# nubot-nudt/RDMNet

Measured on AMD Instinct MI355X. Metric: scan-pairs/sec (whole node), higher is better.
Workload: dtype f32

## Files before the change

### rdmnet_amd/csrc/engine.hip

```cpp
#include <algorithm>
#include <cmath>
#include <cstring>
#include <atomic>
#include <chrono>
#include <functional>
#include <map>
#include <memory>
#include <string>
#include <vector>

#include "../../include/rdmnet_hip.h"
#include <ctime>

#include "common.h"
#include "internal.h"
#include "lockstep.h"

namespace {

using namespace rdm;

struct Mat {
  float* p = nullptr;
  int64_t rows = 0, cols = 0, ld = 0;
  Mat cols_from(int64_t c0, int64_t n) const { return Mat{p + c0, rows, n, ld}; }
  Mat rows_from(int64_t r0, int64_t n) const { return Mat{p + r0 * ld, n, cols, ld}; }
};

struct HostParam {
  std::vector<int64_t> shape;
  std::vector<float> data;
};

struct Linear {
  float* b = nullptr;
  float* wt = nullptr;
  float* bias = nullptr;
  float* packed = nullptr;
  int64_t in = 0, out = 0, kpad = 0, ldb = 0;
};

inline int64_t pad4(int64_t n) { return (n + 3) / 4 * 4; }

struct ParamSet {
  std::map<std::string, Linear> lin;
  std::map<std::string, float*> vec;
  std::vector<void*> owned;
  int device = -1;
  ParamSet() = default;
  ParamSet(const ParamSet&) = delete;
  ParamSet& operator=(const ParamSet&) = delete;
  ~ParamSet() {
    for (void* p : owned) (void)hipFree(p);
  }
};

struct Level {
  float* pts = nullptr;
  int64_t n = 0;
  int64_t* lengths = nullptr;
  int64_t n_ref = 0;
};
struct Table {
  int64_t* idx = nullptr;
  bool i32 = false;
  int64_t rows = 0, width = 0;
  int64_t ld = 0;
// ... 9 lines not shown
struct PairPyramid {
  Level lv[5];
  Table nb[5], sub[4], up[4];
  Grid grids[5];
  int32_t* flags = nullptr;
  int calls = 0;
};

}

struct rdm_engine {
  rdm_engine_config cfg;
  int device = -1;
  std::map<std::string, HostParam> host;
  std::shared_ptr<ParamSet> params = std::make_shared<ParamSet>();
  char* arena = nullptr;
  size_t arena_cap = 0, arena_off = 0;
  bool arena_exhausted = false, arena_fixed = false;
  void* pinned = nullptr;
  void* pinned_dev = nullptr;
  int64_t host_corr_cap = 0;
  int wait_sleep_us = 0;
  bool finalized = false;
  std::map<std::string, rdm_tensor_view> taps;
  bool keep_taps = false;
  bool collate_only = false;
  std::vector<double> topk_fracs;
  bool has_fm = false;
  rdm_fine_matching_options fm{1, 0, 1, 0, 0.f, 0};
  int pairs_in_flight = 1;
  int overlap_mode = 1;
  hipStream_t side = nullptr;
  std::map<hipStream_t, bool> side_ok;
  std::vector<PairPyramid> batch;
  std::vector<int64_t> batch_n_ref, batch_n_src;
  size_t arena_base = 0;
  bool profile = false;
  bool profile_shapes_only = false;
  std::vector<hipEvent_t> events;
  std::vector<rdm_kpconv_profile> prof;
  int prof_layers = 0;
  struct GtInputs {
    bool valid = false;
    const float* nodes[2] = {nullptr, nullptr};
    int64_t m[2] = {0, 0};
    const float* pf[2] = {nullptr, nullptr};
    int64_t nf[2] = {0, 0};
    const int64_t* knn[2] = {nullptr, nullptr};
    const uint8_t* km[2] = {nullptr, nullptr};
    const uint8_t* nm[2] = {nullptr, nullptr};
    int k = 0;
  } gt;

  template <typename T>
  T* alloc(size_t count) {
    size_t bytes = align_up(count * sizeof(T) + 16);
    if (arena_off + bytes > arena_cap) return nullptr;
    T* r = reinterpret_cast<T*>(arena + arena_off);
    arena_off += bytes;
    return r;
  }
  Mat mat(int64_t rows, int64_t cols) {
    Mat m;
    m.rows = rows; m.cols = cols; m.ld = pad4(cols);
    m.p = alloc<float>(static_cast<size_t>(rows > 0 ? rows : 1) * m.ld);
    return m;
  }
};

namespace {

#define ENG_CHECK(...)             \
  do {                             \
    int _rc = (__VA_ARGS__);       \
    if (_rc != 0) return _rc;      \
  } while (0)
#define ENG_ALLOC(ptr)                                             \
  do {                                                             \
    if ((ptr) == nullptr) {                                        \
      set_error("rdm_engine: activation arena exhausted (%zu B)", e->arena_cap); \
      e->arena_exhausted = true;                                   \
      return RDM_ERR_WORKSPACE;                                    \
    }                                                              \
  } while (0)

struct Run {
  rdm_engine* e;
  hipStream_t st;
  void* ws;
  size_t ws_bytes;
  int groups;
};

void tap(Run& r, const char* name, const void* p, int64_t rows, int64_t cols, int64_t ld, int dtype) {
  if (!r.e->keep_taps) return;
  rdm_tensor_view v;
  v.data = const_cast<void*>(p); v.rows = rows; v.cols = cols; v.ld = ld; v.dtype = dtype;
  r.e->taps[name] = v;
}
void tap(Run& r, const char* name, const Mat& m) { tap(r, name, m.p, m.rows, m.cols, m.ld, 0); }

const Linear* lin_param(Run& r, const std::string& name) {
  auto it = r.e->params->lin.find(name);
  if (it != r.e->params->lin.end()) return &it->second;
  set_error("rdm_engine: missing parameter %s", name.c_str());
  return nullptr;
}

float* vecp(Run& r, const std::string& name) {
  auto it = r.e->params->vec.find(name);
  return it == r.e->params->vec.end() ? nullptr : it->second;
}

int norm_params(Run& r, const std::string& prefix, float** g, float** b) {
  *g = vecp(r, prefix + ".weight");
  *b = vecp(r, prefix + ".bias");
  if (*g && *b) return RDM_OK;
  set_error("rdm_engine: missing parameter %s.*", prefix.c_str());
  return RDM_ERR_ARG;
}

int linear(Run& r, const std::string& name, const Mat& x, Mat& y, int act = 0, bool alloc_out = true) {
  lockstep_align();
  rdm_engine* e = r.e;
  const Linear* Lp = lin_param(r, name);
  if (!Lp) return RDM_ERR_ARG;
  const Linear& L = *Lp;
  if (alloc_out) {
    y = e->mat(x.rows, L.out);
    ENG_ALLOC(y.p);
  }
  return rdm_gemm(x.p, x.ld, 0, L.b, L.ldb, 0, 0, y.p, y.ld, 0, x.rows, L.out, L.kpad, 1, L.bias, nullptr, act, r.ws,
                  r.ws_bytes, r.st);
}

int linear_pair(Run& r, const std::string& name0, const Mat& x0, Mat& y0, const std::string& name1, const Mat& x1, Mat& y1) {
  lockstep_align();
  rdm_engine* e = r.e;
  const Linear* P0 = lin_param(r, name0);
  const Linear* P1 = P0 ? lin_param(r, name1) : nullptr;
  if (!P0 || !P1) return RDM_ERR_ARG;
  const Linear &L0 = *P0, &L1 = *P1;
  y0 = e->mat(x0.rows, L0.out);
  y1 = e->mat(x1.rows, L1.out);
  ENG_ALLOC(y0.p); ENG_ALLOC(y1.p);
  return gemm_pair(x0.p, x0.ld, L0.b, L0.ldb, y0.p, y0.ld, x0.rows, L0.out, L0.kpad, L0.bias, x1.p, x1.ld, L1.b, L1.ldb, y1.p,
                   y1.ld, x1.rows, L1.out, L1.kpad, L1.bias, r.ws, r.ws_bytes, r.st);
}

int group_norm(Run& r, const std::string& name, const Mat& x, Mat& y, int act, const Mat* res, uint8_t* positive) {
  lockstep_align();
  rdm_engine* e = r.e;
  y = e->mat(x.rows, x.cols);
  ENG_ALLOC(y.p);
  float *g, *b;
  ENG_CHECK(norm_params(r, name + ".norm", &g, &b));
  return rdm_group_norm(x.p, x.rows, x.cols, x.ld, r.groups, g, b, 1e-5f, res ? res->p : nullptr, res ? res->ld : 0, act,
                        y.p, y.ld, positive, r.ws, r.ws_bytes, r.st);
}

int unary(Run& r, const std::string& name, const Mat& x, Mat& y, int act, const Mat* res, uint8_t* positive) {
  lockstep_align();
  rdm_engine* e = r.e;
  const Linear* Lp = lin_param(r, name + ".mlp");
  if (!Lp) return RDM_ERR_ARG;
  const Linear& L = *Lp;
  Mat t = e->mat(x.rows, L.out);
  y = e->mat(x.rows, L.out);
  ENG_ALLOC(t.p); ENG_ALLOC(y.p);
  float *g, *b;
  ENG_CHECK(norm_params(r, name + ".norm.norm", &g, &b));
  return rdm_linear_group_norm(x.p, x.ld, L.b, L.ldb, L.bias, nullptr, x.rows, L.out, L.kpad, r.groups, g, b, 1e-5f,
                               res ? res->p : nullptr, res ? res->ld : 0, act, t.p, t.ld, y.p, y.ld, positive, r.ws,
                               r.ws_bytes, r.st);
}

int decoder_stage(Run& r, const std::string& lin_name, const std::string* norm_name, const Mat& coarse, const int64_t* up_idx,
                  int64_t up_ld, const Mat& skip, int64_t m, Mat& y) {
  lockstep_align();
  rdm_engine* e = r.e;
  const Linear* Lp = lin_param(r, lin_name);
  if (!Lp) return RDM_ERR_ARG;
  const Linear& L = *Lp;
  RDM_REQUIRE(coarse.cols + skip.cols == L.in, "rdm_engine: %s expects %lld input columns", lin_name.c_str(), (long long)L.in);
  Mat t = e->mat(m, L.out);
  ENG_ALLOC(t.p);
  float *g = nullptr, *b = nullptr;
  if (norm_name) {
    y = e->mat(m, L.out);
    ENG_ALLOC(y.p);
    ENG_CHECK(norm_params(r, *norm_name, &g, &b));
  } else {
    y = t;
  }
  const size_t need = rdm_decoder_stage_workspace_bytes(m, L.out, L.in);
  void* ws = r.ws;
  size_t ws_bytes = r.ws_bytes;
  if (need > ws_bytes) {
    ws = e->alloc<char>(need);
    ENG_ALLOC(ws);
    ws_bytes = need;
  }
  return rdm_decoder_stage(coarse.p, coarse.rows, coarse.cols, coarse.ld, up_idx, up_ld, skip.p, skip.cols, skip.ld, m, L.b, L.ldb,
                           L.bias, L.out, r.groups, g, b, 1e-5f, 2, t.p, t.ld, norm_name ? y.p : nullptr, norm_name ? y.ld : 0, ws,
                           ws_bytes, r.st);
}

int layer_norm(Run& r, const std::string& name, const Mat& x, const Mat* res, int act, Mat& y, bool alloc_out = true) {
  lockstep_align();
  rdm_engine* e = r.e;
  if (alloc_out) {
    y = e->mat(x.rows, x.cols);
    ENG_ALLOC(y.p);
  }
  return rdm_layer_norm(x.p, x.rows, x.cols, x.ld, res ? res->p : nullptr, res ? res->ld : 0, vecp(r, name + ".weight"),
                        vecp(r, name + ".bias"), 1e-5f, act, y.p, y.ld, r.st);
}

int layer_event(rdm_engine* e, int k, hipStream_t st) {
  if (e->profile_shapes_only) return RDM_OK;
  if (lockstep_active()) {
    lockstep_event(e->events[k], st);
    return RDM_OK;
  }
  RDM_HIP_CHECK(hipEventRecord(e->events[k], st));
  return RDM_OK;
}

int kpconv(Run& r, const std::string& name, const Mat& x, const uint8_t* x_pos, const Level& q, const Level& s,
           const Table& t, float sigma, const std::string& norm_name, Mat& y, const float* order,
           const Mat* pool_src = nullptr, Mat* pool_out = nullptr) {
  lockstep_align();
  rdm_engine* e = r.e;
  const Linear* Wp = lin_param(r, name + ".weights");
  if (!Wp) return RDM_ERR_ARG;
  const Linear& W = *Wp;
  const int64_t cin = x.cols, kdim = cin == 1 ? 16 : 15 * cin;
  const int i32 = t.i32 ? 1 : 0;
  const int li = e->prof_layers;
  const bool prof = e->profile && (e->profile_shapes_only ? li < 16 : 3 * li + 2 < static_cast<int>(e->events.size()));
  auto end_profile = [&](int fused) -> int {
    ENG_CHECK(layer_event(e, 3 * li + 2, r.st));
    rdm_kpconv_profile p;
    p.m = q.n; p.h = t.width; p.c_in = cin; p.c_out = W.out; p.pooled_channels = pool_src ? pool_src->cols : 0;
    p.gather_ms = p.total_ms = 0.f;
    p.fused = fused; p.reserved = 0;
    e->prof.push_back(p);
    e->prof_layers++;
    return RDM_OK;
  };
  if (W.packed && rdm_kpconv_fused_enabled()) {
    float *gam, *bet;
    ENG_CHECK(norm_params(r, norm_name + ".norm", &gam, &bet));
    Mat conv = e->mat(q.n, W.out);
    y = e->mat(q.n, W.out);
    ENG_ALLOC(conv.p); ENG_ALLOC(y.p);
    RDM_REQUIRE(rdm_kpconv_fused_workspace_bytes(q.n, cin, W.out) <= r.ws_bytes, "rdm_engine: scratch too small");
    if (prof) ENG_CHECK(layer_event(e, 3 * li, r.st));
    const int nblk = static_cast<int>(rdm_kpconv_fused_partial_rows(q.n, cin));
    double* gn_partial = static_cast<double*>(r.ws);
    const size_t stat_bytes = align_up(static_cast<size_t>(nblk) * 2 * W.out * sizeof(double));
    ENG_CHECK(kpconv_fused_impl(q.pts, q.n, s.pts, s.n, x.p, cin, x.ld, x_pos, t.idx, t.width, t.stride(), t.flags,
                                vecp(r, name + ".kernel_points"), sigma, W.packed, W.bias, W.out, conv.p, conv.ld, gn_partial, order, 0,
                                i32, r.st));
    if (prof) ENG_CHECK(layer_event(e, 3 * li + 1, r.st));
    ENG_CHECK(group_norm_finish(gn_partial, nblk, conv.p, q.n, W.out, conv.ld, r.groups, gam, bet, 1e-5f, nullptr, 0, 2, y.p, y.ld,
                                nullptr, static_cast<char*>(r.ws) + stat_bytes, r.ws_bytes - stat_bytes, r.st));
    if (pool_src) {
      *pool_out = e->mat(q.n, pool_src->cols);
      ENG_ALLOC(pool_out->p);
      ENG_CHECK(gather_max_ordered(pool_src->p, pool_src->rows, pool_src->cols, pool_src->ld, t.idx, q.n, t.width, t.stride(),
                                   t.flags, pool_out->p, pool_out->ld, order, i32, r.st));
    }
    if (prof) ENG_CHECK(end_profile(1));
    return RDM_OK;
  }
  Mat wf = e->mat(q.n, kdim);
  ENG_ALLOC(wf.p);
  float* nn = e->alloc<float>(q.n > 0 ? q.n : 1);
  ENG_ALLOC(nn);
  if (prof) ENG_CHECK(layer_event(e, 3 * li, r.st));
  ENG_CHECK(kpconv_gather_impl(q.pts, q.n, s.pts, s.n, x.p, cin, x.ld, x_pos, t.idx, t.width, t.stride(), t.flags,
                               vecp(r, name + ".kernel_points"), sigma, wf.p, wf.ld, nn, order, i32, r.st));
  if (prof) ENG_CHECK(layer_event(e, 3 * li + 1, r.st));
  Mat conv = e->mat(q.n, W.out);
  ENG_ALLOC(conv.p);
  const size_t gemm_ws = rdm_gemm_workspace_bytes(q.n, W.out, 1);
  const size_t stat_bytes = align_up(static_cast<size_t>(gemm_stats_max_blocks(q.n)) * 2 * W.out * sizeof(double));
  RDM_REQUIRE(gemm_ws + stat_bytes + rdm_group_norm_workspace_bytes(q.n, W.out) <= r.ws_bytes, "rdm_engine: scratch too small");
  double* gn_partial = reinterpret_cast<double*>(static_cast<char*>(r.ws) + gemm_ws);
  int gn_blocks = 0;
  ENG_CHECK(gemm_with_stats(wf.p, wf.ld, W.b, W.ldb, conv.p, conv.ld, q.n, W.out, W.kpad, W.bias, nn, r.ws, gemm_ws,
                            gn_partial, &gn_blocks, r.st));
  if (pool_src) {
    *pool_out = e->mat(q.n, pool_src->cols);
    ENG_ALLOC(pool_out->p);
    ENG_CHECK(gather_max_ordered(pool_src->p, pool_src->rows, pool_src->cols, pool_src->ld, t.idx, q.n, t.width, t.stride(),
                                   t.flags, pool_out->p, pool_out->ld, order, i32, r.st));
  }
  if (prof) ENG_CHECK(end_profile(0));
  y = e->mat(q.n, W.out);
  ENG_ALLOC(y.p);
  float *gam, *bet;
  ENG_CHECK(norm_params(r, norm_name + ".norm", &gam, &bet));
  return group_norm_finish(gn_partial, gn_blocks, conv.p, q.n, W.out, conv.ld, r.groups, gam, bet, 1e-5f, nullptr, 0, 2, y.p,
                           y.ld, nullptr, static_cast<char*>(r.ws) + gemm_ws + stat_bytes, r.ws_bytes - gemm_ws - stat_bytes,
                           r.st);
}

int linear_ln(Run& r, const std::string& lin, const std::string& norm, const Mat& x, const Mat& res, Mat& y, bool alloc_out) {
  lockstep_align();
  rdm_engine* e = r.e;
  const Linear* Lp = lin_param(r, lin);
  if (!Lp) return RDM_ERR_ARG;
  const Linear& L = *Lp;
  if (L.wt && L.out == 128) {
    if (alloc_out) {
      y = e->mat(x.rows, L.out);
      ENG_ALLOC(y.p);
    }
    return rdm_linear_layer_norm(x.p, x.ld, L.wt, L.kpad, L.bias, x.rows, L.out, L.kpad, res.p, res.ld, vecp(r, norm + ".weight"),
                                 vecp(r, norm + ".bias"), 1e-5f, 0, y.p, y.ld, r.st);
  }
  Mat h;
  ENG_CHECK(linear(r, lin, x, h));
  return layer_norm(r, norm, h, &res, 0, y, alloc_out);
}

int attention_tail(Run& r, const std::string& p, const Mat& hid, const Mat& x, Mat out) {
  lockstep_align();
  rdm_engine* e = r.e;
  auto lo = e->params->lin.find(p + ".attention.linear"), l1 = e->params->lin.find(p + ".output.expand"), l2 = e->params->lin.find(p + ".output.squeeze");
  if (lo != e->params->lin.end() && l1 != e->params->lin.end() && l2 != e->params->lin.end() && lo->second.wt && l1->second.wt && l2->second.wt &&
      lo->second.out == 128 && lo->second.kpad == 128 && l1->second.out == 256 && l1->second.kpad == 128 &&
      l2->second.out == 128 && l2->second.kpad == 256) {
    const Linear &Lo = lo->second, &L1 = l1->second, &L2 = l2->second;
    auto pk = e->params->vec.find(p + ".__tail_packed");
    static const bool unpacked = ::rdm::dev_knob("RDM_TAIL_UNPACKED") != nullptr;
    if (pk != e->params->vec.end() && !unpacked)
      return rdm_attention_tail_packed(hid.p, hid.ld, x.p, x.ld, hid.rows, 128, pk->second, Lo.bias, vecp(r, p + ".attention.norm.weight"),
                                       vecp(r, p + ".attention.norm.bias"), L1.bias, L2.bias, vecp(r, p + ".output.norm.weight"),
                                       vecp(r, p + ".output.norm.bias"), 1e-5f, out.p, out.ld, r.st);
    return rdm_attention_tail(hid.p, hid.ld, x.p, x.ld, hid.rows, 128, Lo.wt, Lo.kpad, Lo.bias, vecp(r, p + ".attention.norm.weight"),
                              vecp(r, p + ".attention.norm.bias"), L1.wt, L1.kpad, L1.bias, L2.wt, L2.kpad, L2.bias,
                              vecp(r, p + ".output.norm.weight"), vecp(r, p + ".output.norm.bias"), 1e-5f, out.p, out.ld, r.st);
  }
  Mat y, z1;
  ENG_CHECK(linear_ln(r, p + ".attention.linear", p + ".attention.norm", hid, x, y, true));
  ENG_CHECK(linear(r, p + ".output.expand", y, z1, 1));
  return linear_ln(r, p + ".output.squeeze", p + ".output.norm", z1, y, out, false);
}

int thdroformer(Run& r, const std::string& name, const Mat& pts4, const Mat& x, int64_t n0, int num_layers, Mat out,
                const std::function<int()>* after_two = nullptr, const std::vector<double>* topk = nullptr) {
  rdm_engine* e = r.e;
  const int heads = e->cfg.num_heads;
  const int64_t N = x.rows, n1 = N - n0;
  Mat emb, f;
  ENG_CHECK(linear(r, name + ".embedding.proj", pts4, emb));
  ENG_CHECK(linear(r, name + ".in_proj", x, f));
// ... 179 lines not shown
  if (e->side_ok.size() >= 64) e->side_ok.clear();
  if (e->side && runs_beside(st, e->side)) {
    *usable = e->side_ok[st] = true;
    return RDM_OK;
  }
  bool have_user = false;
  for (const auto& kv : e->side_ok) have_user |= kv.second;
  if (have_user) {
    *usable = e->side_ok[st] = false;
    return RDM_OK;
  }
  std::vector<hipStream_t> rejected;
  if (e->side) rejected.push_back(e->side);
  e->side = nullptr;
  for (int attempt = 0; attempt < 6 && !e->side; ++attempt) {
    hipStream_t cand = nullptr;
    RDM_HIP_CHECK(hipStreamCreateWithFlags(&cand, hipStreamNonBlocking));
    if (runs_beside(st, cand)) e->side = cand;
    else rejected.push_back(cand);
  }
  for (hipStream_t r : rejected) (void)hipStreamDestroy(r);
  *usable = e->side_ok[st] = e->side != nullptr;
  return RDM_OK;
}
struct SideGuard {
  rdm_engine* e;
  int pending = 0;
  ~SideGuard() {
    if (pending > 0 && e->side) (void)hipStreamSynchronize(e->side);
  }
};

int d2h(Run& r, const void* dev, size_t bytes, void* host_dst) {
  copy_words(dev, r.e->pinned_dev, static_cast<int>((bytes + 3) / 4), r.st);
  ENG_CHECK(wait_stream(r));
  std::memcpy(host_dst, r.e->pinned, bytes);
  return RDM_OK;
}

}

extern "C" int rdm_engine_create(const rdm_engine_config* cfg, rdm_engine** out) {
  RDM_REQUIRE(cfg && out, "rdm_engine_create: null pointer");
  RDM_REQUIRE(cfg->num_stages == 5 && cfg->kernel_size == 15, "rdm_engine_create: only 5 stages / 15 kernel points");
  int device = -1;
  RDM_HIP_CHECK(hipGetDevice(&device));
  rdm_engine* e = new rdm_engine();
  e->cfg = *cfg;
  e->device = device;
  e->params->device = device;
  e->arena_cap = cfg->arena_bytes ? cfg->arena_bytes : (size_t(3) << 30);
  e->arena_fixed = cfg->arena_bytes != 0;
  hipError_t err = hipMalloc(reinterpret_cast<void**>(&e->arena), e->arena_cap);
  if (err != hipSuccess) {
    set_error("rdm_engine_create: hipMalloc(%zu) failed: %s", e->arena_cap, hipGetErrorString(err));
    delete e;
    return RDM_ERR_HIP;
  }
  e->host_corr_cap = static_cast<int64_t>(std::max(cfg->num_correspondences, 1)) * 2 * std::max(cfg->points_in_patch, 1);
  err = hipHostMalloc(&e->pinned, 4096 + static_cast<size_t>(e->host_corr_cap) * 7 * sizeof(float), hipHostMallocMapped);
  if (err == hipSuccess) err = hipHostGetDevicePointer(&e->pinned_dev, e->pinned, 0);
  if (err != hipSuccess) {
    set_error("rdm_engine_create: hipHostMalloc failed: %s", hipGetErrorString(err));
    (void)hipFree(e->arena);
    delete e;
    return RDM_ERR_HIP;
  }
  *out = e;
  return RDM_OK;
}

extern "C" void rdm_engine_destroy(rdm_engine* e) {
  if (!e) return;
  e->params.reset();
  for (auto& ev : e->events) (void)hipEventDestroy(ev);
  if (e->side) {
    (void)hipStreamSynchronize(e->side);
    (void)hipStreamDestroy(e->side);
  }
  if (e->arena) (void)hipFree(e->arena);
  if (e->pinned) (void)hipHostFree(e->pinned);
  delete e;
}

extern "C" int rdm_engine_set_param(rdm_engine* e, const char* name, const float* data_host, const int64_t* shape_host,
                                    int ndim) {
  RDM_REQUIRE(e && name && data_host && ndim >= 0 && ndim <= 4, "rdm_engine_set_param: bad arguments");
  HostParam p;
  int64_t n = 1;
  for (int i = 0; i < ndim; ++i) {
    p.shape.push_back(shape_host[i]);
    n *= shape_host[i];
  }
  p.data.assign(data_host, data_host + n);
  e->host[name] = std::move(p);
  e->finalized = false;
  return RDM_OK;
}

namespace {
int upload(rdm_engine* e, const std::vector<float>& h, float** dev) {
  void* p = nullptr;
  RDM_HIP_CHECK(hipMalloc(&p, (h.size() + 4) * sizeof(float)));
  RDM_HIP_CHECK(hipMemcpy(p, h.data(), h.size() * sizeof(float), hipMemcpyHostToDevice));
  e->params->owned.push_back(p);
  *dev = static_cast<float*>(p);
// ... 96 lines not shown
        continue;
      float* d = nullptr;
      RDM_HIP_CHECK(hipMalloc(reinterpret_cast<void**>(&d), rdm_attention_tail_packed_floats() * sizeof(float)));
      e->params->owned.push_back(d);
      ENG_CHECK(rdm_attention_tail_pack_weights(lo->second.wt, lo->second.kpad, l1->second.wt, l1->second.kpad, l2->second.wt, l2->second.kpad, d, nullptr));
      e->params->vec[p + ".__tail_packed"] = d;
    }
    RDM_HIP_CHECK(hipDeviceSynchronize());
  }
  e->finalized = true;
  return RDM_OK;
}

extern "C" int rdm_engine_share_params(rdm_engine* e, const rdm_engine* src) {
  RDM_REQUIRE(e && src && e != src, "rdm_engine_share_params: bad arguments");
  RDM_REQUIRE(src->finalized, "rdm_engine_share_params: the source engine is not finalized");
  RDM_REQUIRE(e->device == src->device && src->params->device == src->device,
              "rdm_engine_share_params: the engines live on different devices (%d vs %d)", e->device, src->device);
  const rdm_engine_config &a = e->cfg, &b = src->cfg;
  RDM_REQUIRE(a.num_stages == b.num_stages && a.kernel_size == b.kernel_size && a.group_norm == b.group_norm &&
                  a.out_dim == b.out_dim && a.num_heads == b.num_heads && a.num_layers == b.num_layers &&
                  a.num_layers2 == b.num_layers2 && a.vote_mlp_layers == b.vote_mlp_layers &&
                  a.points_in_patch == b.points_in_patch,
              "rdm_engine_share_params: the engines were created with different model shapes");
  e->host.clear();
  e->params = src->params;
  e->finalized = true;
  return RDM_OK;
}

extern "C" int rdm_engine_enable_profile(rdm_engine* e, int enable) {
  RDM_REQUIRE(e, "rdm_engine_enable_profile: null engine");
  RDM_REQUIRE(enable >= 0 && enable <= 2, "rdm_engine_enable_profile: 0 (off), 1 (events) or 2 (layer shapes only)");
  e->profile = enable != 0;
  e->profile_shapes_only = enable == 2;
  if (enable == 1 && e->events.empty()) {
    e->events.resize(3 * 16);
    for (auto& ev : e->events) RDM_HIP_CHECK(hipEventCreate(&ev));
  }
  return RDM_OK;
}

extern "C" int rdm_engine_reserve(rdm_engine* e, size_t bytes) {
  RDM_REQUIRE(e && bytes >= (size_t(1) << 20), "rdm_engine_reserve: at least 1 MiB");
  RDM_HIP_CHECK(hipDeviceSynchronize());
  e->batch.clear();
  e->arena_base = 0;
  e->gt.valid = false;
  RDM_HIP_CHECK(hipFree(e->arena));
  e->arena = nullptr;
  e->arena_cap = bytes;
  e->arena_fixed = false;
  const hipError_t err = hipMalloc(reinterpret_cast<void**>(&e->arena), e->arena_cap);
  if (err != hipSuccess) {
    e->arena_cap = 0;
    set_error("rdm_engine_reserve: hipMalloc(%zu) failed: %s", bytes, hipGetErrorString(err));
    return RDM_ERR_HIP;
  }
  return RDM_OK;
}

extern "C" int rdm_engine_set_wait(rdm_engine* e, int sleep_us) {
  RDM_REQUIRE(e && sleep_us >= 0, "rdm_engine_set_wait: bad arguments");
  e->wait_sleep_us = sleep_us;
  return RDM_OK;
}

extern "C" int rdm_engine_set_pairs_in_flight(rdm_engine* e, int n) {
  RDM_REQUIRE(e && n >= 1, "rdm_engine_set_pairs_in_flight: bad arguments");
  e->pairs_in_flight = n;
  return RDM_OK;
}

extern "C" int rdm_engine_set_fine_matching(rdm_engine* e, const rdm_fine_matching_options* o) {
  RDM_REQUIRE(e, "rdm_engine_set_fine_matching: null engine");
  if (!o) {
    e->has_fm = false;
    return RDM_OK;
  }
  const int K = std::max(e->cfg.points_in_patch, 1);
  RDM_REQUIRE(o->topk >= 1 && o->topk <= K + (o->use_dustbin ? 1 : 0), "rdm_engine_set_fine_matching: topk = %d is outside [1, %d]",
              o->topk, K + (o->use_dustbin ? 1 : 0));
  RDM_REQUIRE(o->confidence_threshold >= 0.f, "rdm_engine_set_fine_matching: confidence_threshold = %g is not >= 0",
              static_cast<double>(o->confidence_threshold));
  RDM_REQUIRE(o->correspondence_limit >= 0, "rdm_engine_set_fine_matching: correspondence_limit = %d (0 = none, or >= 1)",
              o->correspondence_limit);
  const int64_t cap = rdm_lgr_options_capacity(std::max(e->cfg.num_correspondences, 1), K, o);
  if (cap > e->host_corr_cap) {
    int device = -1;
    RDM_HIP_CHECK(hipGetDevice(&device));
    RDM_REQUIRE(device == e->device, "rdm_engine_set_fine_matching: the engine belongs to device %d, current is %d", e->device, device);
    void* pinned = nullptr;
    void* pinned_dev = nullptr;
    RDM_HIP_CHECK(hipHostMalloc(&pinned, 4096 + static_cast<size_t>(cap) * 7 * sizeof(float), hipHostMallocMapped));
    const hipError_t err = hipHostGetDevicePointer(&pinned_dev, pinned, 0);
    if (err != hipSuccess) {
      (void)hipHostFree(pinned);
      set_error("rdm_engine_set_fine_matching: hipHostGetDevicePointer failed: %s", hipGetErrorString(err));
      return RDM_ERR_HIP;
    }
    RDM_HIP_CHECK(hipDeviceSynchronize());
    if (e->pinned) (void)hipHostFree(e->pinned);
    e->pinned = pinned;
    e->pinned_dev = pinned_dev;
    e->host_corr_cap = cap;
  }
// ... 93 lines not shown
    if (!(nb0_done && i == 0)) ENG_CHECK(search(e, sq, lv[i], py.grids[i], radius, c.neighbor_limits[i], !full, row(), py.nb[i]));
    if (i < 4) ENG_CHECK(search(e, sq, lv[i + 1], py.grids[i], radius, c.neighbor_limits[i], !full, row(), py.sub[i]));
    if (i > 0 && (full || i > 1))
      ENG_CHECK(search(e, sq, lv[i - 1], py.grids[i], radius, full ? c.neighbor_limits[i] : 1, false, row(), py.up[i - 1]));
  }
  return RDM_OK;
}

int build_level_grids(rdm_engine* e, PairPyramid* pys, int n, int first, int last, hipStream_t st) {
  const float* gp[8];
  int64_t gn[8];
  const int64_t* gl[8];
  float gr[8];
  void* gw[8];
  size_t gb[8];
  int k = 0;
  auto launch = [&]() -> int {
    RDM_DUP_LOOP("rnbuild")
    ENG_CHECK(radius_grid_build_multi(k, gp, gn, gl, 2, gr, gw, gb, st));
    k = 0;
    return RDM_OK;
  };
  for (int p = 0; p < n; ++p) {
    float rad = e->cfg.init_radius;
    for (int i = 0; i < last; ++i, rad *= 2.f) {
      if (i < first) continue;
      const Level& l = pys[p].lv[i];
      Grid& g = pys[p].grids[i];
      g.n_s = l.n;
      g.bytes = rdm_radius_grid_workspace_bytes(l.n);
      g.ws = e->alloc<char>(g.bytes);
      ENG_ALLOC(g.ws);
      gp[k] = l.pts; gn[k] = l.n; gl[k] = l.lengths; gr[k] = rad; gw[k] = g.ws; gb[k] = g.bytes;
      if (++k == 8) ENG_CHECK(launch());
    }
  }
  return k > 0 ? launch() : RDM_OK;
}

}

static int engine_run_once(rdm_engine* e, const float* ref_points, int64_t n_ref, const float* src_points, int64_t n_src,
                           const rdm_data_dict* dd, rdm_engine_result* res, void* stream, const PairPyramid* pre = nullptr);

static bool may_grow(const rdm_engine* e, int rc) {
  return rc == RDM_ERR_WORKSPACE && e->arena_exhausted && !e->arena_fixed && e->arena_cap < (size_t(96) << 30);
}
static int grow_arena(rdm_engine* e, void* stream, const char* who) {
  RDM_HIP_CHECK(hipStreamSynchronize(static_cast<hipStream_t>(stream)));
  RDM_HIP_CHECK(hipFree(e->arena));
  e->arena = nullptr;
  e->arena_cap *= 2;
  const hipError_t err = hipMalloc(reinterpret_cast<void**>(&e->arena), e->arena_cap);
  if (err != hipSuccess) {
    e->arena_cap = 0;
    set_error("%s: growing the activation arena failed: %s", who, hipGetErrorString(err));
    return RDM_ERR_HIP;
  }
  return RDM_OK;
}
static int engine_run_growing(rdm_engine* e, const float* ref_points, int64_t n_ref, const float* src_points, int64_t n_src,
                              const rdm_data_dict* dd, rdm_engine_result* res, void* stream) {
  PadGuard pad_guard(e->pairs_in_flight >= 3 ? 20480u : 0u);
  for (;;) {
    e->arena_exhausted = false;
    const int rc = engine_run_once(e, ref_points, n_ref, src_points, n_src, dd, res, stream);
    if (!may_grow(e, rc)) return rc;
    ENG_CHECK(grow_arena(e, stream, "rdm_engine_run"));
  }
}

extern "C" int rdm_engine_run(rdm_engine* e, const float* ref_points, int64_t n_ref, const float* src_points,
                              int64_t n_src, rdm_engine_result* res, void* stream) {
  RDM_REQUIRE(e && ref_points && src_points && res, "rdm_engine_run: null pointer");
  RDM_REQUIRE(e->finalized, "rdm_engine_run: call rdm_engine_finalize first");
  RDM_REQUIRE(n_ref > 0 && n_src > 0, "rdm_engine_run: empty cloud");
  return engine_run_growing(e, ref_points, n_ref, src_points, n_src, nullptr, res, stream);
}

static int collate_batch_once(rdm_engine* e, int B, const float* const* refs, const int64_t* n_refs, const float* const* srcs,
                              const int64_t* n_srcs, hipStream_t st) {
  const rdm_engine_config& c = e->cfg;
  e->arena_off = 0;
  e->arena_base = 0;
  e->gt.valid = false;
  e->batch.clear();
  e->taps.clear();
  Run r;
  r.e = e; r.st = st; r.groups = c.group_norm;
  int64_t n_tot = 0;
  for (int p = 0; p < B; ++p) n_tot += n_refs[p] + n_srcs[p];
  const int nc = 2 * B;
  r.ws_bytes = std::max<size_t>(rdm_grid_subsample_workspace_bytes(n_tot, nc), size_t(16) << 20);
  r.ws = e->alloc<char>(r.ws_bytes);
  ENG_ALLOC(r.ws);
  float* pts[5];
  int64_t* len[5];
  pts[0] = e->alloc<float>(3 * n_tot);
  len[0] = e->alloc<int64_t>(nc);
  ENG_ALLOC(pts[0]); ENG_ALLOC(len[0]);
  {
    int64_t base = 0;
    for (int p = 0; p < B; ++p) {
      ENG_CHECK(launch1d<concat_points_kernel_body, concat_points_kernel>("concat_points", 3 * (n_refs[p] + n_srcs[p]), st, refs[p], n_refs[p], srcs[p], n_srcs[p],
                         pts[0] + 3 * base, len[0] + 2 * p));
      base += n_refs[p] + n_srcs[p];
// ... 716 lines not shown
  const int64_t cap = n0;
  for (int i = 1; i < 5; ++i) {
    voxel *= 2.f;
    lv[i].pts = e->alloc<float>(3 * cap);
    lv[i].lengths = all_len + 2 * (i - 1);
    ENG_ALLOC(lv[i].pts);
    RDM_DUP_LOOP("gs")
    ENG_CHECK(grid_subsample_mode(i == 1 ? pts0 : lv[i - 1].pts, cap, i == 1 ? len0 : lv[i - 1].lengths, 2, voxel, lv[i].pts,
                                  lv[i].lengths, r.ws, r.ws_bytes, r.st, i <= gs_multi_levels() ? 2 : 1));
    if (i == 1 && overlap_l0) {
      ENG_CHECK(launch1d<concat_points_kernel_body, concat_points_kernel>("concat_points", 3 * n0, rs.st, ref_points, n_ref, src_points, n_src, lv[0].pts,
                         lv[0].lengths));
      ENG_CHECK(build_level_grids(e, &py, 1, 0, 1, rs.st));
      SearchQueue side_queue(rs.st);
      ENG_CHECK(search(e, side_queue, lv[0], py.grids[0], c.init_radius, c.neighbor_limits[0], !full, py.flags + 2 * py.calls++,
                       py.nb[0]));
      ENG_CHECK(side_queue.flush());
      ENG_CHECK(encoder_input(rs, nullptr, n0, enc));
      ENG_CHECK(encoder_blocks(rs, py, 0, 2, enc));
    }
  }
  int64_t host_len[8];
  ENG_CHECK(d2h(r, all_len, sizeof(host_len), host_len));
  if (overlap_l0) {
    ENG_CHECK(wait_on(e, e->side));
    side_guard.pending--;
  }
  for (int i = 1; i < 5; ++i) {
    lv[i].n_ref = host_len[2 * (i - 1)];
    lv[i].n = host_len[2 * (i - 1)] + host_len[2 * (i - 1) + 1];
  }
  ENG_CHECK(build_level_grids(e, &py, 1, overlap_l0 ? 1 : 0, 5, r.st));
  SearchQueue sq(r.st);
  ENG_CHECK(search_pyramid(e, py, full, overlap_l0, sq));
  return sq.flush();
}

void tap_pyramid(Run& r, const PairPyramid& py) {
  for (int i = 0; i < 5; ++i) {
    const Level& l = py.lv[i];
    tap(r, ("lengths" + std::to_string(i)).c_str(), l.lengths, 1, 2, 2, 1);
    tap(r, ("points" + std::to_string(i)).c_str(), l.pts, l.n, 3, 3, 0);
    tap(r, ("neighbors" + std::to_string(i)).c_str(), py.nb[i].idx, py.nb[i].rows, py.nb[i].width, py.nb[i].stride(), 1);
    if (i < 4) {
      tap(r, ("subsampling" + std::to_string(i)).c_str(), py.sub[i].idx, py.sub[i].rows, py.sub[i].width, py.sub[i].stride(), 1);
      tap(r, ("upsampling" + std::to_string(i)).c_str(), py.up[i].idx, py.up[i].rows, py.up[i].width, py.up[i].stride(), 1);
    }
  }
  tap(r, "search_flags", py.flags, 32, 2, 2, 3);
}

}

static int engine_run_once(rdm_engine* e, const float* ref_points, int64_t n_ref, const float* src_points, int64_t n_src,
                           const rdm_data_dict* dd, rdm_engine_result* res, void* stream, const PairPyramid* pre) {
  const rdm_engine_config& c = e->cfg;
  e->arena_off = pre ? e->arena_base : 0;
  e->gt.valid = false;
  if (!pre) {
    e->batch.clear();
    e->arena_base = 0;
  }
  e->taps.clear();
  e->prof.clear();
  e->prof_layers = 0;
  Run r;
  r.e = e; r.st = static_cast<hipStream_t>(stream); r.groups = c.group_norm;
  const int64_t n0 = n_ref + n_src;
  bool overlap = !pre && !lockstep_active() && !e->collate_only && r.st != nullptr && (e->overlap_mode == 2 || (e->overlap_mode == 1 && e->pairs_in_flight == 1));
  if (overlap) ENG_CHECK(ensure_side(e, r.st, &overlap));
  SideGuard side_guard{e};
  r.ws_bytes = pre ? size_t(96) << 20
                   : std::max<size_t>(rdm_grid_subsample_workspace_bytes(n0, 2),
                                      std::max<size_t>(rdm_radius_neighbors_workspace_bytes(n0, n0, 2), size_t(96) << 20));
  r.ws = e->alloc<char>(r.ws_bytes);
  ENG_ALLOC(r.ws);
  std::memset(res, 0, sizeof(*res));

  PairPyramid py;
  Encoder enc;
  if (pre) py = *pre;
  else if (dd) ENG_CHECK(pyramid_from_data_dict(r, *dd, py));
  else ENG_CHECK(collate_pair(r, overlap, side_guard, ref_points, n_ref, src_points, n_src, py, enc));
  for (int i = 0; i < 5; ++i) {
    res->level_sizes[i] = py.lv[i].n;
    res->level_ref_sizes[i] = py.lv[i].n_ref;
  }
  tap_pyramid(r, py);
  if (e->collate_only) {
    res->arena_used = e->arena_off;
    return RDM_OK;
  }

  {
    size_t need = r.ws_bytes;
    for (int l = 0; l < c.num_stages; ++l)
      need = std::max(need, rdm_linear_group_norm_workspace_bytes(py.lv[l].n, int64_t(128) << l));
    if (need > r.ws_bytes) {
      r.ws_bytes = need;
      r.ws = e->alloc<char>(r.ws_bytes);
      ENG_ALLOC(r.ws);
    }
  }

  if (enc.blocks == 0) ENG_CHECK(encoder_input(r, dd, n0, enc));
  ENG_CHECK(encoder_blocks(r, py, enc.blocks, 14, enc));
  tap(r, "feats_c_enc", enc.feats[4]);
// ... 175 lines not shown
```

### rdmnet_amd/csrc/gemm.hip

```cpp
#include "../../include/rdmnet_hip.h"
#include <cmath>
#include <cstdlib>
#include <type_traits>

#include "common.h"
#include "internal.h"
#include "lockstep.h"

namespace {

using namespace rdm;

typedef float f32x16 __attribute__((ext_vector_type(16)));
typedef float f32x4_t __attribute__((ext_vector_type(4)));

struct GemmArgs {
  const float* A;
  const float* B;
  float* C;
  const float* bias;
  const float* rowdiv;
  int M, N, K;
  int lda, ldb, ldc;
  long long sa, sb, sc;
  int act;
  int splits;
  float* part;
  double* stats;
  const float* A2;
  const int64_t* aidx;
  int lda2, ldi, c1, n_coarse;
  const int64_t* bidx;
  int n_b;
  int xcd_tiles;
#ifdef RDM_GEMM_TIMING
  unsigned long long* clk;
#endif
};
#ifdef RDM_GEMM_TIMING
#define GEMM_STAMP(k) do { if (blockIdx.x == 0 && blockIdx.y == 0 && blockIdx.z == 0 && threadIdx.x == 0) g.clk[k] = __builtin_amdgcn_s_memtime(); } while (0)
#else
#define GEMM_STAMP(k) do { } while (0)
#endif
#ifdef RDM_GEMM_TIMING
#define GEMM_WIDE_STAMP(k) do { if (blockIdx.x == 0 && blockIdx.y == 0 && blockIdx.z == 0 && threadIdx.x == 0 && (k) < 392) g.clk[k] = __builtin_amdgcn_s_memtime(); } while (0)
#else
#define GEMM_WIDE_STAMP(k) do { } while (0)
#endif

__device__ __forceinline__ float apply_act(float v, int act) {
  if (act == 1) return v > 0.f ? v : 0.f;
  if (act == 2) return v > 0.f ? v : 0.1f * v;
  return v;
}

template <int BM, int BN, int WM, int WN, int BK, bool TRANS_B, int PF, bool CAT = false>
__device__ __forceinline__ void gemm_kernel_body(const dim3 blockIdx, const dim3 gridDim, GemmArgs g) {
  (void)blockIdx; (void)gridDim;
  constexpr int TM = BM / WM, TN = BN / WN, FM = TM / 32, FN = TN / 32;
  static_assert(WM * WN == 4 && TM % 32 == 0 && TN % 32 == 0, "bad tile");
  constexpr int LDA_S = BM + 1, LDB_S = TRANS_B ? BN + 1 : BN + 4;
  constexpr int CR = BM < 64 ? BM : 64;
  constexpr int LDC_S = BN + 4;
  constexpr int TPR = BN / 4;
  constexpr int RPI = 256 / TPR;
  constexpr int kBytesAB = (2 * BK * LDA_S + 2 * BK * LDB_S) * 4, kBytesC = CR * LDC_S * 4, kBytesStat = RPI * BN * 2 * 8;
  constexpr int kBytes = kBytesAB > kBytesC ? (kBytesAB > kBytesStat ? kBytesAB : kBytesStat) : (kBytesC > kBytesStat ? kBytesC : kBytesStat);
  static_assert((2 * BK * LDA_S * 4) % 16 == 0 && CR % RPI == 0, "tile layout");
  __shared__ __attribute__((aligned(16))) char smem[kBytes];
  float (*As)[BK][LDA_S] = reinterpret_cast<float (*)[BK][LDA_S]>(smem);
  float (*Bs)[BK][LDB_S] = reinterpret_cast<float (*)[BK][LDB_S]>(smem + 2 * BK * LDA_S * 4);
  float (*Cs)[LDC_S] = reinterpret_cast<float (*)[LDC_S]>(smem);
  double (*stat_red)[1][2] = reinterpret_cast<double (*)[1][2]>(smem);

  const int tid = threadIdx.x, lane = tid & 63, wave = tid >> 6;
  const int wm = wave / WN, wn = wave % WN;
  int tile_x = blockIdx.x, tile_y = blockIdx.y;
  if (g.xcd_tiles) {
    const int nblk = gridDim.x * gridDim.y, lin = blockIdx.y * gridDim.x + blockIdx.x;
    const int q = nblk / 8, rr = nblk % 8, xcd = lin % 8, within = lin / 8;
    const int logical = (xcd < rr ? xcd * (q + 1) : rr * (q + 1) + (xcd - rr) * q) + within;
    tile_x = logical % gridDim.x;
    tile_y = logical / gridDim.x;
  }
  const int m0 = tile_y * BM, n0 = tile_x * BN;
  GEMM_STAMP(0);
  const int batch = blockIdx.z / g.splits, split = blockIdx.z % g.splits;
  const float* A = g.A + batch * g.sa;
  const float* B = g.B + batch * g.sb;

  const int ktiles = (g.K + BK - 1) / BK;
  const int per = (ktiles + g.splits - 1) / g.splits;
  const int kt0 = split * per, kt1 = min(ktiles, kt0 + per);

  constexpr int A_N4 = BM * BK / 4;
  constexpr int A_V = (A_N4 + 255) / 256;
  constexpr int KC4 = BK / 4;
  constexpr int B_N4 = BK * BN / 4;
  constexpr int B_V = (B_N4 + 255) / 256;
  static_assert(PF == 1 || PF == 2, "one or two register stages");
  float4 ra0[A_V], rb0[B_V], ra1[PF == 2 ? A_V : 1], rb1[PF == 2 ? B_V : 1];
  long long cat_row[CAT ? A_V : 1], cat_brow[CAT && TRANS_B ? B_V : 1];
  if constexpr (CAT && !TRANS_B) {
#pragma unroll
    for (int i = 0; i < A_V; ++i) {
      const int row = (tid + i * 256) / (BK / 4);
      const long long id = g.aidx[static_cast<long long>(min(m0 + row, g.M - 1)) * g.ldi];
      cat_row[i] = (id >= 0 && id < g.n_coarse) ? id : -1;
    }
  }
  if constexpr (CAT && TRANS_B) {
    A = g.A;
    B = g.B;
    int any_a = 0, any_b = 0;
#pragma unroll
    for (int i = 0; i < A_V; ++i) {
      const int row = (tid + i * 256) / (BK / 4);
      const long long id = (m0 + row < g.M && (A_N4 % 256 == 0 || tid + i * 256 < A_N4)) ? g.aidx[static_cast<long long>(batch) * g.M + m0 + row] : -1;
      cat_row[i] = (id >= 0 && id < g.n_coarse) ? id : -1;
      any_a |= cat_row[i] >= 0;
    }
// ... 197 lines not shown
        const float4 t = *reinterpret_cast<const float4*>(&Cs[lrow][c4]);
        float v[4] = {t.x, t.y, t.z, t.w};
        if (has_rd) {
          const float rd = rdv[pass * (CR / RPI) + it];
#pragma unroll
          for (int e = 0; e < 4; ++e) v[e] = v[e] / rd;
        }
        if (!partial) {
#pragma unroll
          for (int e = 0; e < 4; ++e) {
            const float u = v[e] + bv[e];
            const float neg = act == 2 ? 0.1f * u : 0.f;
            v[e] = (act != 0 && !(u > 0.f)) ? neg : u;
          }
        }
        float* dst = C + static_cast<long long>(row) * ldc + gcol;
        if (vec_ok && gcol + 3 < g.N) {
          *reinterpret_cast<float4*>(dst) = make_float4(v[0], v[1], v[2], v[3]);
        } else {
#pragma unroll
          for (int e = 0; e < 4; ++e)
            if (gcol + e < g.N) dst[e] = v[e];
        }
        if (stats) {
#pragma unroll
          for (int e = 0; e < 4; ++e) {
            cs[e] += v[e];
            css[e] += static_cast<double>(v[e]) * v[e];
          }
        }
      }
    }
    GEMM_STAMP(5);
    lds_barrier();
  }
  if (stats) {
#pragma unroll
    for (int e = 0; e < 4; ++e) {
      stat_red[rsub * BN + c4 + e][0][0] = cs[e];
      stat_red[rsub * BN + c4 + e][0][1] = css[e];
    }
    lds_barrier();
    for (int cl = tid; cl < BN; cl += 256) {
      const int col = n0 + cl;
      if (col >= g.N) continue;
      double a = 0.0, b = 0.0;
#pragma unroll
      for (int w = 0; w < RPI; ++w) {
        a += stat_red[w * BN + cl][0][0];
        b += stat_red[w * BN + cl][0][1];
      }
      g.stats[(static_cast<long long>(tile_y) * 2 + 0) * g.N + col] = a;
      g.stats[(static_cast<long long>(tile_y) * 2 + 1) * g.N + col] = b;
    }
  }
  GEMM_STAMP(3);
}
template <int BM, int BN, int WM, int WN, int BK, bool TRANS_B, int PF, bool CAT = false>
__global__ __launch_bounds__(256, (BM * BN <= 64 * 64 ? 4 : 1)) void gemm_kernel(GemmArgs g) { gemm_kernel_body<BM, BN, WM, WN, BK, TRANS_B, PF, CAT>(blockIdx, gridDim, g); }


template <bool CAT, bool MI16 = false>
__device__ __forceinline__ void gemm_wide_body(const dim3 blockIdx, const dim3 gridDim, GemmArgs g) {
  (void)gridDim;
  constexpr int BM = 128, BN = 128, BK = 32;
  constexpr int IMG = 8 * BM * 4;
  constexpr int CR = 64, LDC_S = BN + 4, TPR = BN / 4, RPI = 256 / TPR;
  static_assert(BM == BN && RPI == 8 && CR * LDC_S * 4 <= 4 * IMG * 4 && 16 * BN * 2 * 8 <= 4 * IMG * 4, "wide tile layout");
  __shared__ __attribute__((aligned(16))) char smem[4 * IMG * 4];
  float* As = reinterpret_cast<float*>(smem);
  float* Bs = As + 2 * IMG;
  float (*Cs)[LDC_S] = reinterpret_cast<float (*)[LDC_S]>(smem);
  double (*stat_red)[BN][2] = reinterpret_cast<double (*)[BN][2]>(smem);

  const int tid = threadIdx.x, lane = tid & 63, wave = tid >> 6;
  const int wm = wave >> 1, wn = wave & 1;
  constexpr int NF = MI16 ? 4 : 2;
  constexpr int FR = MI16 ? 16 : 32;
  constexpr int KG = MI16 ? 16 : 8;
  constexpr int NG = BK / KG;
  constexpr int KL = MI16 ? 4 : 2;
  const int lk = MI16 ? lane >> 4 : lane >> 5, li = MI16 ? lane & 15 : lane & 31;
  const int m0 = blockIdx.y * BM, n0 = blockIdx.x * BN;
  const int batch = blockIdx.z / g.splits, split = blockIdx.z % g.splits;
  const float* A = g.A + (CAT ? 0 : batch * g.sa);
  const float* B = g.B + batch * g.sb;
  const int ktiles = (g.K + BK - 1) / BK;
  const int per = (ktiles + g.splits - 1) / g.splits;
  const int kt0 = split * per, kt1 = min(ktiles, kt0 + per);
  GEMM_WIDE_STAMP(0);

  const int a_q = tid & 7, a_row = tid >> 3;
  const int b_p = tid >> 5, b_n4 = (tid & 31) * 4;
  const int b_k = MI16 ? 16 * (b_p >> 2) + (b_p & 3) : 8 * (b_p >> 1) + (b_p & 1);
  float4 ra[4], rb[4];
  const float* a_ptr[4];
  long long cat_row[CAT ? 4 : 1];
#pragma unroll
  for (int i = 0; i < 4; ++i) {
    const int row = min(m0 + a_row + 32 * i, g.M - 1);
    if constexpr (CAT) {
      const long long id = g.aidx[static_cast<long long>(row) * g.ldi];
      cat_row[i] = (id >= 0 && id < g.n_coarse) ? id : -1;
      a_ptr[i] = A + max(cat_row[i], 0ll) * g.lda;
    } else {
      a_ptr[i] = A + static_cast<long long>(row) * g.lda;
// ... 206 lines not shown
        float v[4] = {t.x, t.y, t.z, t.w};
        if (has_rd) {
#pragma unroll
          for (int e = 0; e < 4; ++e) v[e] = v[e] / rdv[it];
        }
        if (!partial) {
#pragma unroll
          for (int e = 0; e < 4; ++e) {
            const float u = v[e] + bv[e];
            const float neg = act == 2 ? 0.1f * u : 0.f;
            v[e] = (act != 0 && !(u > 0.f)) ? neg : u;
          }
        }
        float* dst = C + static_cast<long long>(row) * ldc + gcol;
        if (vec_ok && gcol + 3 < g.N) {
          *reinterpret_cast<float4*>(dst) = make_float4(v[0], v[1], v[2], v[3]);
        } else {
#pragma unroll
          for (int e = 0; e < 4; ++e)
            if (gcol + e < g.N) dst[e] = v[e];
        }
        if (stats) {
#pragma unroll
          for (int e = 0; e < 4; ++e) {
            cs[it & 1][e] += v[e];
            css[it & 1][e] += static_cast<double>(v[e]) * v[e];
          }
        }
      }
    }
    lds_barrier();
    if (stats) {
#pragma unroll
      for (int par = 0; par < 2; ++par)
#pragma unroll
        for (int e = 0; e < 4; ++e) {
          stat_red[par * RPI + rsub][c4 + e][0] = cs[par][e];
          stat_red[par * RPI + rsub][c4 + e][1] = css[par][e];
        }
      lds_barrier();
      if (tid < BN && n0 + tid < g.N) {
        double a = 0.0, b = 0.0;
#pragma unroll
        for (int w = 0; w < 16; ++w) {
          a += stat_red[w][tid][0];
          b += stat_red[w][tid][1];
        }
        const long long blk = static_cast<long long>(blockIdx.y) * 2 + pass;
        g.stats[(blk * 2 + 0) * g.N + n0 + tid] = a;
        g.stats[(blk * 2 + 1) * g.N + n0 + tid] = b;
      }
      lds_barrier();
    }
  }
  GEMM_WIDE_STAMP(3);
}
template <bool CAT, bool MI16 = false>
__global__ __launch_bounds__(256, 2) void gemm_wide_kernel(GemmArgs g) { gemm_wide_body<CAT, MI16>(blockIdx, gridDim, g); }

__device__ __forceinline__ void gemm_small_body(const dim3 blockIdx, const GemmArgs& g, float (*red)[32][33]) {
  const int tid = threadIdx.x, lane = tid & 63, wave = tid >> 6;
  const int li = lane & 31, lk = lane >> 5;
  const int m0 = blockIdx.y * 32, n0 = blockIdx.x * 32;
  const int kq = g.K / 4;
  const int kbeg = wave * kq;
  const int row = min(m0 + li, g.M - 1);
  const int col = n0 + li;
  const bool col_ok = col < g.ldb;
  const float* arow = g.A + static_cast<long long>(row) * g.lda;
  f32x16 acc;
#pragma unroll
  for (int r = 0; r < 16; ++r) acc[r] = 0.f;
  for (int c = 0; c < kq; c += 32) {
    float a[16], b[16];
    const int kb = kbeg + c + lk * 16;
#pragma unroll
    for (int q = 0; q < 4; ++q) {
      float4 v = make_float4(0.f, 0.f, 0.f, 0.f);
      if (c + lk * 16 + 4 * q < kq) v = *reinterpret_cast<const float4*>(arow + kb + 4 * q);
      a[4 * q] = v.x; a[4 * q + 1] = v.y; a[4 * q + 2] = v.z; a[4 * q + 3] = v.w;
    }
#pragma unroll
    for (int t = 0; t < 16; ++t)
      b[t] = (col_ok && c + lk * 16 + t < kq) ? g.B[static_cast<long long>(kb + t) * g.ldb + col] : 0.f;
#pragma unroll
    for (int t = 0; t < 16; ++t) acc = __builtin_amdgcn_mfma_f32_32x32x2f32(a[t], b[t], acc, 0, 0, 0);
  }
#pragma unroll
  for (int r = 0; r < 16; ++r) red[wave][(r & 3) + 8 * (r >> 2) + 4 * lk][li] = acc[r];
  __syncthreads();
#pragma unroll
  for (int q = 0; q < 4; ++q) {
    const int e = tid + 256 * q, rr = e >> 5, cc = e & 31;
    const int orow = m0 + rr, ocol = n0 + cc;
    if (orow < g.M && ocol < g.N) {
      float v = ((red[0][rr][cc] + red[1][rr][cc]) + red[2][rr][cc]) + red[3][rr][cc];
      if (g.bias) v += g.bias[ocol];
      g.C[static_cast<long long>(orow) * g.ldc + ocol] = apply_act(v, g.act);
    }
  }
}

__device__ __forceinline__ void gemm_small_entry(const dim3 blockIdx, const dim3 gridDim, GemmArgs g) {
  (void)gridDim;
  __shared__ float red[4][32][33];
  gemm_small_body(blockIdx, g, red);
// ... 231 lines not shown
  layer_norm(o, 2, g2, be2);
  TAIL_STAMP(7);
#pragma unroll
  for (int r = 0; r < 4; ++r) {
    const int row = m0 + 4 * kb + r;
    if (row < a.M) a.out[static_cast<long long>(row) * a.ldo + c] = o[r];
  }
}
template <bool PACKED>
__global__ __launch_bounds__(512) void attention_tail128_kernel(TailArgs a) { attention_tail128_body<PACKED>(blockIdx, gridDim, a); }

__global__ void attention_tail_pack_kernel(const float* wo, int ldwo, const float* w1, int ldw1, const float* w2, int ldw2, float4* out) {
  const int e = blockIdx.x * blockDim.x + threadIdx.x;
  if (e >= 20480) return;
  const int lane = e & 63, i = lane & 15, kb = lane >> 4;
  const float* src;
  if (e < 4096) {
    const int w = e >> 9, s = (e >> 6) & 7;
    src = wo + static_cast<long long>(16 * w + i) * ldwo + 16 * s + 4 * kb;
  } else if (e < 12288) {
    const int t = e - 4096, w = t >> 10, h = (t >> 9) & 1, s = (t >> 6) & 7;
    src = w1 + static_cast<long long>(32 * w + 16 * h + i) * ldw1 + 16 * s + 4 * kb;
  } else {
    const int t = e - 12288, w = t >> 10, s = (t >> 6) & 15;
    src = w2 + static_cast<long long>(16 * w + i) * ldw2 + 16 * s + 4 * kb;
  }
  out[e] = *reinterpret_cast<const float4*>(src);
}

__device__ __forceinline__ void splitk_reduce_kernel_body(const dim3 blockIdx, const dim3 gridDim, GemmArgs g, int batches) {
  (void)blockIdx; (void)gridDim;
  const long long total = static_cast<long long>(batches) * g.M * g.N;
  for (long long i = blockIdx.x * static_cast<long long>(blockDim.x) + threadIdx.x; i < total;
       i += static_cast<long long>(gridDim.x) * blockDim.x) {
    const int n = static_cast<int>(i % g.N);
    const int m = static_cast<int>((i / g.N) % g.M);
    const int b = static_cast<int>(i / (static_cast<long long>(g.M) * g.N));
    const float* p = g.part + (static_cast<long long>(b) * g.splits) * g.M * g.N +
                     static_cast<long long>(m) * g.N + n;
    float v = 0.f;
    for (int s = 0; s < g.splits; ++s) v += p[static_cast<long long>(s) * g.M * g.N];
    if (g.rowdiv) v = v / g.rowdiv[m];
    if (g.bias) v += g.bias[n];
    g.C[b * g.sc + static_cast<long long>(m) * g.ldc + n] = apply_act(v, g.act);
  }
}
__global__ void splitk_reduce_kernel(GemmArgs g, int batches) { splitk_reduce_kernel_body(blockIdx, gridDim, g, batches); }


constexpr int kStatRowsPerLane = 8;
inline int stat_rows_per_block(long long n) { return kStatRowsPerLane * (256 / static_cast<int>(n < 256 ? n : 256)); }
__device__ __forceinline__ void splitk_reduce_stats_kernel_body(const dim3 blockIdx, const dim3 gridDim, GemmArgs g, double* stats) {
  (void)blockIdx; (void)gridDim;
  __shared__ double red[2][256];
  const int cw = g.N < 256 ? g.N : 256;
  const int lanes = 256 / cw;
  const int r0 = blockIdx.x * (kStatRowsPerLane * lanes);
  const int r1 = min(g.M, r0 + kStatRowsPerLane * lanes);
  const int col_in = threadIdx.x % cw, rl = threadIdx.x / cw;
  const int col = blockIdx.y * 256 + col_in;
  double s = 0.0, ss = 0.0;
  if (rl < lanes && col < g.N) {
    const float bv = g.bias ? g.bias[col] : 0.f;
    const long long plane = static_cast<long long>(g.M) * g.N;
    float acc[kStatRowsPerLane];
    const float* p[kStatRowsPerLane];
#pragma unroll
    for (int u = 0; u < kStatRowsPerLane; ++u) {
      const int r = min(r0 + rl + u * lanes, g.M - 1);
      p[u] = g.part + static_cast<long long>(r) * g.N + col;
      acc[u] = 0.f;
    }
    for (int k = 0; k < g.splits; ++k) {
#pragma unroll
      for (int u = 0; u < kStatRowsPerLane; ++u) acc[u] += p[u][k * plane];
    }
#pragma unroll
    for (int u = 0; u < kStatRowsPerLane; ++u) {
      const int r = r0 + rl + u * lanes;
      if (r >= r1) break;
      float v = acc[u];
      if (g.rowdiv) v = v / g.rowdiv[r];
      v = apply_act(v + bv, g.act);
      g.C[static_cast<long long>(r) * g.ldc + col] = v;
      const double d = v;
      s += d;
      ss += d * d;
    }
  }
  red[0][threadIdx.x] = s;
  red[1][threadIdx.x] = ss;
  __syncthreads();
  if (threadIdx.x < cw && col < g.N) {
    double a = 0.0, b = 0.0;
    for (int k = 0; k < lanes; ++k) {
      a += red[0][k * cw + threadIdx.x];
      b += red[1][k * cw + threadIdx.x];
    }
    stats[(static_cast<long long>(blockIdx.x) * 2 + 0) * g.N + col] = a;
    stats[(static_cast<long long>(blockIdx.x) * 2 + 1) * g.N + col] = b;
  }
}
__global__ __launch_bounds__(256) void splitk_reduce_stats_kernel(GemmArgs g, double* stats) { splitk_reduce_stats_kernel_body(blockIdx, gridDim, g, stats); }


thread_local unsigned g_lds_pad = 0;

template <int BM, int BN, int WM, int WN, int BK, int PF = 1>
void launch(const GemmArgs& g, int batches, bool trans_b, hipStream_t st) {
  dim3 grid(ceil_div(g.N, BN), ceil_div(g.M, BM), batches * g.splits);
  static const int pad_env = [] { const char* v = ::rdm::dev_knob("RDM_GEMM_LDS_PAD"); return v ? atoi(v) : -1; }();
  const unsigned pad = pad_env >= 0 ? static_cast<unsigned>(pad_env) : g_lds_pad;
  if constexpr (BM == 64 && BN == 64 && BK == 32 && PF == 2) {
    if (g.aidx && g.bidx) {
      ::rdm::launch<gemm_kernel_body<BM, BN, WM, WN, BK, true, PF, true>, gemm_kernel<BM, BN, WM, WN, BK, true, PF, true>, 256, (BM * BN <= 64 * 64 ? 4 : 1)>(grid, pad, st, g);
      return;
    }
    if (g.aidx) {
      ::rdm::launch<gemm_kernel_body<BM, BN, WM, WN, BK, false, PF, true>, gemm_kernel<BM, BN, WM, WN, BK, false, PF, true>, 256, (BM * BN <= 64 * 64 ? 4 : 1)>(grid, pad, st, g);
      return;
    }
  }
  if (trans_b)
    ::rdm::launch<gemm_kernel_body<BM, BN, WM, WN, BK, true, PF>, gemm_kernel<BM, BN, WM, WN, BK, true, PF>, 256, (BM * BN <= 64 * 64 ? 4 : 1)>(grid, pad, st, g);
  else
    ::rdm::launch<gemm_kernel_body<BM, BN, WM, WN, BK, false, PF>, gemm_kernel<BM, BN, WM, WN, BK, false, PF>, 256, (BM * BN <= 64 * 64 ? 4 : 1)>(grid, pad, st, g);
}

void launch_wide(const GemmArgs& g, int batches, hipStream_t st, bool mi16_form) {
  dim3 grid(ceil_div(g.N, 128), ceil_div(g.M, 128), batches * g.splits);
  static const bool mi16 = ::rdm::dev_knob("RDM_GEMM_WIDE_MI16") != nullptr;
  if (mi16 || mi16_form) {
    if (g.aidx) ::rdm::launch<gemm_wide_body<true, true>, gemm_wide_kernel<true, true>, 256, 2>(grid, 0, st, g);
    else ::rdm::launch<gemm_wide_body<false, true>, gemm_wide_kernel<false, true>, 256, 2>(grid, 0, st, g);
    return;
  }
  if (g.aidx) ::rdm::launch<gemm_wide_body<true>, gemm_wide_kernel<true>, 256, 2>(grid, 0, st, g);
  else ::rdm::launch<gemm_wide_body<false>, gemm_wide_kernel<false>, 256, 2>(grid, 0, st, g);
}

}

void rdm::gemm_set_lds_pad(unsigned bytes) { g_lds_pad = bytes; }

extern "C" size_t rdm_gemm_workspace_bytes(int64_t m, int64_t n, int batches) {
  const size_t by_shape = static_cast<size_t>(m) * static_cast<size_t>(n) * 16;
  const size_t by_tiles = static_cast<size_t>(1024) * 128 * 128;
  return align_up(std::min(by_shape, by_tiles) * sizeof(float) * static_cast<size_t>(batches > 0 ? batches : 1));
}

namespace {

thread_local int g_last_plan[4] = {0, 0, 0, 0};

int gemm_dispatch(GemmArgs g, int batches, bool trans_b, void* ws, size_t ws_bytes, int* stat_blocks, hipStream_t st, int form = 0) {
  const long long m = g.M, n = g.N, k = g.K;
  const char* tune_env = ::rdm::dev_knob("RDM_GEMM_TUNE");
  if (batches == 1 && !trans_b && !g.rowdiv && !g.stats && !g.aidx && m <= 1536 && k % 16 == 0 && k >= 64 && k <= 1024 &&
      m * n <= 1536 * 512 && !(tune_env && tune_env[0] != '0')) {
    if (stat_blocks) *stat_blocks = 0;
    g_last_plan[0] = 32; g_last_plan[1] = 32; g_last_plan[2] = static_cast<int>(k / 4); g_last_plan[3] = 4;
    RDM_DUP_LOOP("gemmsmall")
    ::rdm::launch<gemm_small_entry, gemm_small_kernel, 256>(dim3(ceil_div<long long>(n, 32), ceil_div<long long>(m, 32)), 0, st, g);
    return launch_status("gemm_small_kernel");
  }
  enum Tile { T128, T64, T128x32 };
  struct Cand { Tile tile; int bm, bn; double fixed_us, lat_k64_us, mfma_k64_us; int resident; double alpha; };
  static const Cand cands[3] = {{T128, 128, 128, 4.0, 2.6, 3.4, 3, 0.0}, {T64, 64, 64, 1.5, 2.2, 0.86, 4, 0.2},
                                {T128x32, 128, 32, 3.0, 1.3, 0.86, 3, 0.0}};
  static const int split_set[8] = {1, 2, 3, 4, 6, 8, 12, 16};
  static const long long model_cus = [] {
    const char* v = ::rdm::dev_knob("RDM_GEMM_CUS");
    const long long n = v ? atoll(v) : 256;
    return n >= 8 && n <= 256 ? n : 256ll;
  }();
  Tile tile = T64;
  int best_s = 1;
  {
    double best = 1e30;
    const size_t ws_cap = ws ? ws_bytes : 0;
    for (const Cand& c : cands) {
      if (g.aidx && c.tile != T64) continue;
      if (c.tile == T128x32 && n > 64) continue;
      if (c.tile != T128x32 && n <= 32) continue;
      if (c.tile == T128 && n < 128) continue;
      const long long tiles = ceil_div<long long>(m, c.bm) * ceil_div<long long>(n, c.bn) * batches;
      const int max_s = k >= 256 ? static_cast<int>(std::min<long long>(16, k / 128)) : 1;
      for (int sp : split_set) {
        if (sp > max_s) break;
        if (sp > 1 && static_cast<size_t>(m) * n * sp * batches * sizeof(float) > ws_cap) break;
        const long long blocks = tiles * sp;
        const double k_per = static_cast<double>(k) / sp / 64.0;
        const long long per_round = model_cus * c.resident;
        const long long full = blocks / per_round, rem = blocks % per_round;
        auto per_k64 = [&](double r) { return std::max(c.lat_k64_us * (1.0 + c.alpha * (r - 1.0)), c.mfma_k64_us * r); };
        double t = full * (c.fixed_us + k_per * per_k64(c.resident));
        if (rem) t += c.fixed_us + k_per * per_k64(static_cast<double>(ceil_div<long long>(rem, model_cus)));
        if (sp > 1) t += 3.0 + static_cast<double>(m) * n * sp * 8.0 / 1.5e6;
        if (t < best) {
          best = t;
          tile = c.tile;
          best_s = sp;
        }
      }
    }
  }
  int force_splits = 0, exp_tile = 0;
  if (const char* tune = ::rdm::dev_knob("RDM_GEMM_TUNE")) {
    int t = 0, sp = 0;
    if (sscanf(tune, "%d,%d", &t, &sp) >= 1) {
      if (t == 1) tile = T128;
      else if (t == 2) tile = T64;
      else if (t == 3) tile = T128x32;
      else if (t >= 4 && t <= 7) exp_tile = t;
      force_splits = sp;
      if (t >= 1 && t <= 7 && sp == 0) best_s = 1;
    }
  }
  static const int big_min_m = [] { const char* v = ::rdm::dev_knob("RDM_GEMM_BIG"); return v ? atoi(v) : 0; }();
  static const int big_tile = [] { const char* v = ::rdm::dev_knob("RDM_GEMM_BIG"); const char* c = v ? strchr(v, ',') : nullptr; return c ? atoi(c + 1) : 6; }();
  static const bool big_split = ::rdm::dev_knob("RDM_GEMM_BIG_SPLIT") != nullptr;
  if (big_min_m > 0 && exp_tile == 0 && m >= big_min_m && n >= 128 && (best_s == 1 || big_split) && force_splits == 0 && batches == 1)
    exp_tile = big_tile;
  static const bool xcd_env = ::rdm::dev_knob("RDM_GEMM_XCD") != nullptr;
  g.xcd_tiles = (xcd_env && ceil_div<long long>(n, 64) > 1 && ceil_div<long long>(m, 64) * ceil_div<long long>(n, 64) >= 64) ? 1 : 0;
  if (g.aidx) {
    tile = T64;
    exp_tile = 0;
    if (g.bidx) best_s = 1, force_splits = 0;
  }
  static const int wide_min_m = [] { const char* v = ::rdm::dev_knob("RDM_GEMM_WIDE_MIN_M"); return v ? atoi(v) : 256; }();
  static const int wide_min_n = [] { const char* v = ::rdm::dev_knob("RDM_GEMM_WIDE_MIN_N"); return v ? atoi(v) : 128; }();
  static const bool wide_knob = ::rdm::dev_knob("RDM_GEMM_WIDE") != nullptr;
  const bool wide_off = !wide_knob && form == 0;
  static const bool wide_force = ::rdm::dev_knob("RDM_GEMM_WIDE_FORCE") != nullptr;
  if (wide_force && !trans_b && !g.bidx && exp_tile == 0) tile = T64;
  const bool wide = !wide_off && tile == T64 && exp_tile == 0 && !trans_b && !g.bidx && (form != 0 || (m >= wide_min_m && n >= wide_min_n));
  int bm = tile == T64 ? 64 : 128, bn = tile == T128 ? 128 : (tile == T64 ? 64 : 32);
  if (wide) { bm = 128; bn = 128; }
  if (exp_tile == 4) { bm = 128; bn = 64; }
  if (exp_tile == 5) { bm = 64; bn = 128; }
  if (exp_tile == 6) { bm = 128; bn = 128; }
  if (exp_tile == 7) { bm = 256; bn = 64; }
  {
    int sp = force_splits > 0 ? force_splits : best_s;
    const size_t need = static_cast<size_t>(m) * n * sp * batches * sizeof(float);
    if (sp > 1 && ws && ws_bytes >= need) {
      g.splits = sp;
      g.part = static_cast<float*>(ws);
    }
  }
  double* reduce_stats = nullptr;
  if (g.splits > 1) {
    if (batches == 1 && g.N % 4 == 0) reduce_stats = g.stats;
    g.stats = nullptr;
  }
  if (stat_blocks)
    *stat_blocks = g.stats ? static_cast<int>(ceil_div<long long>(m, wide ? 64 : bm))
                           : (reduce_stats ? static_cast<int>(ceil_div<long long>(m, stat_rows_per_block(n))) : 0);
  g_last_plan[0] = bm; g_last_plan[1] = bn; g_last_plan[3] = g.splits;
  g_last_plan[2] = wide ? 32 : (tile == T128 ? 16 : ((tile == T64 ? (k >= 48 || g.aidx) : k >= 32) ? 32 : 16));
  RDM_DUP_LOOP("gemm") {
  if (wide) launch_wide(g, batches, st, form == 2);
  else
#ifdef RDM_DEV_KNOBS
  if (exp_tile == 4) launch<128, 64, 2, 2, 32, 2>(g, batches, trans_b, st);
  else if (exp_tile == 5) launch<64, 128, 2, 2, 32, 2>(g, batches, trans_b, st);
  else if (exp_tile == 6) launch<128, 128, 2, 2, 32, 2>(g, batches, trans_b, st);
  else if (exp_tile == 7) launch<256, 64, 4, 1, 32, 2>(g, batches, trans_b, st);
  else
#endif
  switch (tile) {
    case T128: launch<128, 128, 2, 2, 16>(g, batches, trans_b, st); break;
    case T64:
      static const bool bk16 = ::rdm::dev_knob("RDM_GEMM_BK16") != nullptr;
      if ((k >= 48 && !bk16) || g.aidx) launch<64, 64, 2, 2, 32, 2>(g, batches, trans_b, st);
      else launch<64, 64, 2, 2, 16>(g, batches, trans_b, st);
      break;
    case T128x32:
      if (k >= 32) launch<128, 32, 4, 1, 32, 2>(g, batches, trans_b, st);
      else launch<128, 32, 4, 1, 16>(g, batches, trans_b, st);
      break;
  }
  }
  if (int e = launch_status("gemm_kernel")) return e;
  if (g.splits > 1 && reduce_stats) {
    RDM_DUP_LOOP("splitk")
    ::rdm::launch<splitk_reduce_stats_kernel_body, splitk_reduce_stats_kernel, 256>(dim3(ceil_div<long long>(m, stat_rows_per_block(n)), ceil_div<long long>(n, 256)), 0, st, g, reduce_stats);
    return launch_status("splitk_reduce_stats_kernel");
  }
  if (g.splits > 1) {
    const long long total = static_cast<long long>(batches) * m * n;
    const int blocks = static_cast<int>(std::min<long long>(ceil_div<long long>(total, 256), 2048));
    ::rdm::launch<splitk_reduce_kernel_body, splitk_reduce_kernel, 256>(dim3(blocks), 0, st, g, batches);
    return launch_status("splitk_reduce_kernel");
  }
  return RDM_OK;
}

}

int rdm::gemm_with_stats(const float* a, int64_t lda, const float* b, int64_t ldb, float* c, int64_t ldc, int64_t m,
                         int64_t n, int64_t k, const float* bias, const float* rowdiv, void* ws, size_t ws_bytes,
                         double* gn_partial, int* gn_blocks, void* stream, int form) {
  GemmArgs g;
  g.A = a; g.B = b; g.C = c; g.bias = bias; g.rowdiv = rowdiv;
  g.M = static_cast<int>(m); g.N = static_cast<int>(n); g.K = static_cast<int>(k);
  g.lda = static_cast<int>(lda); g.ldb = static_cast<int>(ldb); g.ldc = static_cast<int>(ldc);
  g.sa = g.sb = g.sc = 0;
  g.act = 0; g.splits = 1; g.part = nullptr; g.stats = gn_partial;
  g.A2 = nullptr; g.aidx = nullptr; g.lda2 = g.ldi = g.c1 = g.n_coarse = 0; g.bidx = nullptr; g.n_b = 0;
  return gemm_dispatch(g, 1, false, ws, ws_bytes, gn_blocks, static_cast<hipStream_t>(stream), form);
}

int rdm::gemm_concat_with_stats(const float* coarse, int64_t ld1, int64_t c1, int64_t n_coarse, const int64_t* idx, int64_t ldi,
                                const float* skip, int64_t ld2, int64_t c2, const float* b, int64_t ldb, float* c, int64_t ldc,
                                int64_t m, int64_t n, const float* bias, int act, void* ws, size_t ws_bytes, double* gn_partial,
                                int* gn_blocks, void* stream, int form) {
  if (c1 % 32 != 0 || c2 % 4 != 0 || c2 < 4 || ld1 % 4 != 0 || ld2 % 4 != 0 || ldb % 4 != 0 || m <= 0 ||
      ((reinterpret_cast<uintptr_t>(coarse) | reinterpret_cast<uintptr_t>(skip) | reinterpret_cast<uintptr_t>(b)) & 15) != 0)
    return 1;
  GemmArgs g;
  g.A = coarse; g.B = b; g.C = c; g.bias = bias; g.rowdiv = nullptr;
  g.M = static_cast<int>(m); g.N = static_cast<int>(n); g.K = static_cast<int>(c1 + c2);
  g.lda = static_cast<int>(ld1); g.ldb = static_cast<int>(ldb); g.ldc = static_cast<int>(ldc);
  g.sa = g.sb = g.sc = 0;
  g.act = act; g.splits = 1; g.part = nullptr; g.stats = gn_partial;
  g.A2 = skip; g.aidx = idx; g.lda2 = static_cast<int>(ld2); g.ldi = static_cast<int>(ldi); g.c1 = static_cast<int>(c1);
  g.n_coarse = static_cast<int>(n_coarse);
  g.bidx = nullptr; g.n_b = 0;
  return gemm_dispatch(g, 1, false, ws, ws_bytes, gn_blocks, static_cast<hipStream_t>(stream), form);
}

namespace {
bool small_kernel_ok(long long m, long long n, long long k) {
  return m <= 1536 && k % 16 == 0 && k >= 64 && k <= 1024 && m * n <= 1536 * 512 && !::rdm::dev_knob("RDM_GEMM_TUNE");
}
}

int rdm::gemm_pair(const float* a0, int64_t lda0, const float* b0, int64_t ldb0, float* c0, int64_t ldc0, int64_t m0, int64_t n0,
                   int64_t k0, const float* bias0, const float* a1, int64_t lda1, const float* b1, int64_t ldb1, float* c1,
                   int64_t ldc1, int64_t m1, int64_t n1, int64_t k1, const float* bias1, void* ws, size_t ws_bytes, void* stream) {
  if (m0 > 0 && m1 > 0 && small_kernel_ok(m0, n0, k0) && small_kernel_ok(m1, n1, k1) && lda0 % 4 == 0 && lda1 % 4 == 0 &&
      ldb0 % 4 == 0 && ldb1 % 4 == 0 && ((reinterpret_cast<uintptr_t>(a0) | reinterpret_cast<uintptr_t>(a1)) & 15) == 0) {
    GemmArgs g[2];
    const float* A[2] = {a0, a1}; const float* B[2] = {b0, b1}; float* C[2] = {c0, c1}; const float* bias[2] = {bias0, bias1};
    const int64_t M[2] = {m0, m1}, N[2] = {n0, n1}, K[2] = {k0, k1}, LA[2] = {lda0, lda1}, LB[2] = {ldb0, ldb1}, LC[2] = {ldc0, ldc1};
    for (int i = 0; i < 2; ++i) {
      g[i].A = A[i]; g[i].B = B[i]; g[i].C = C[i]; g[i].bias = bias[i]; g[i].rowdiv = nullptr;
      g[i].M = static_cast<int>(M[i]); g[i].N = static_cast<int>(N[i]); g[i].K = static_cast<int>(K[i]);
      g[i].lda = static_cast<int>(LA[i]); g[i].ldb = static_cast<int>(LB[i]); g[i].ldc = static_cast<int>(LC[i]);
      g[i].sa = g[i].sb = g[i].sc = 0; g[i].act = 0; g[i].splits = 1; g[i].part = nullptr; g[i].stats = nullptr;
      g[i].A2 = nullptr; g[i].aidx = nullptr; g[i].lda2 = g[i].ldi = g[i].c1 = g[i].n_coarse = 0; g[i].bidx = nullptr; g[i].n_b = 0;
    }
    const long long gx = ceil_div<long long>(std::max(n0, n1), 32), gy = ceil_div<long long>(std::max(m0, m1), 32);
    ::rdm::launch<gemm_small_pair_entry, gemm_small_pair_kernel, 256>(dim3(gx, gy, 2), 0, static_cast<hipStream_t>(stream), g[0], g[1]);
    return launch_status("gemm_small_pair_kernel");
  }
  if (m0 > 0)
    if (int e = rdm_gemm(a0, lda0, 0, b0, ldb0, 0, 0, c0, ldc0, 0, m0, n0, k0, 1, bias0, nullptr, 0, ws, ws_bytes, stream)) return e;
  if (m1 > 0) return rdm_gemm(a1, lda1, 0, b1, ldb1, 0, 0, c1, ldc1, 0, m1, n1, k1, 1, bias1, nullptr, 0, ws, ws_bytes, stream);
  return RDM_OK;
}

extern "C" int rdm_gemm_last_plan(int* out4_host) {
  using namespace rdm;
  RDM_REQUIRE(out4_host, "rdm_gemm_last_plan: null pointer");
  for (int i = 0; i < 4; ++i) out4_host[i] = g_last_plan[i];
  return RDM_OK;
}

extern "C" int rdm_gemm(const float* a, int64_t lda, int64_t stride_a, const float* b, int64_t ldb,
                        int64_t stride_b, int trans_b, float* c, int64_t ldc, int64_t stride_c,
                        int64_t m, int64_t n, int64_t k, int batches, const float* bias,
                        const float* rowdiv, int act, void* ws, size_t ws_bytes, void* stream) {
  return rdm_gemm_form(a, lda, stride_a, b, ldb, stride_b, trans_b, c, ldc, stride_c, m, n, k, batches, bias, rowdiv, act, ws, ws_bytes, 0, stream);
}

extern "C" int rdm_gemm_form(const float* a, int64_t lda, int64_t stride_a, const float* b, int64_t ldb,
                             int64_t stride_b, int trans_b, float* c, int64_t ldc, int64_t stride_c,
                             int64_t m, int64_t n, int64_t k, int batches, const float* bias,
                             const float* rowdiv, int act, void* ws, size_t ws_bytes, int form, void* stream) {
  using namespace rdm;
  RDM_REQUIRE(form >= 0 && form <= 2, "rdm_gemm_form: unknown form %d", form);
  RDM_REQUIRE(a && b && c, "rdm_gemm: null pointer");
  RDM_REQUIRE(m >= 0 && n >= 0 && k >= 0 && batches >= 1, "rdm_gemm: bad sizes");
  if (m == 0 || n == 0) return RDM_OK;
  RDM_REQUIRE(k % 4 == 0 && lda % 4 == 0 && ldb % 4 == 0,
              "rdm_gemm: K (%lld), lda (%lld), ldb (%lld) must be multiples of 4 (pad with zeros)",
              (long long)k, (long long)lda, (long long)ldb);
  RDM_REQUIRE((reinterpret_cast<uintptr_t>(a) & 15) == 0 && (reinterpret_cast<uintptr_t>(b) & 15) == 0,
              "rdm_gemm: A and B must be 16-byte aligned");
  RDM_REQUIRE(act >= 0 && act <= 2, "rdm_gemm: unknown activation %d", act);
  GemmArgs g;
  g.A = a; g.B = b; g.C = c; g.bias = bias; g.rowdiv = rowdiv;
  g.M = static_cast<int>(m); g.N = static_cast<int>(n); g.K = static_cast<int>(k);
  g.lda = static_cast<int>(lda); g.ldb = static_cast<int>(ldb); g.ldc = static_cast<int>(ldc);
  g.sa = stride_a; g.sb = stride_b; g.sc = stride_c;
  g.act = act; g.splits = 1; g.part = nullptr; g.stats = nullptr;
  g.A2 = nullptr; g.aidx = nullptr; g.lda2 = g.ldi = g.c1 = g.n_coarse = 0; g.bidx = nullptr; g.n_b = 0;
  return gemm_dispatch(g, batches, trans_b != 0, ws, ws_bytes, nullptr, static_cast<hipStream_t>(stream), form);
}

extern "C" size_t rdm_linear_group_norm_workspace_bytes(int64_t m, int64_t n) {
  return rdm_gemm_workspace_bytes(m, n, 1) + rdm::align_up(static_cast<size_t>(rdm::gemm_stats_max_blocks(m)) * 2 * n * sizeof(double)) +
         rdm_group_norm_workspace_bytes(m, n) + 1024;
}

extern "C" int rdm_linear_group_norm(const float* x, int64_t ldx, const float* w, int64_t ldw, const float* bias,
                                     const float* rowdiv, int64_t m, int64_t n, int64_t k, int groups,
                                     const float* gamma, const float* beta, float eps, const float* residual,
                                     int64_t ldr, int act, float* lin_out, int64_t ld_lin, float* y, int64_t ldy,
                                     uint8_t* positive, void* ws, size_t ws_bytes, void* stream) {
  return rdm_linear_group_norm_form(x, ldx, w, ldw, bias, rowdiv, m, n, k, groups, gamma, beta, eps, residual, ldr, act, lin_out, ld_lin, y, ldy,
                                    positive, ws, ws_bytes, 0, stream);
}

extern "C" int rdm_linear_group_norm_form(const float* x, int64_t ldx, const float* w, int64_t ldw, const float* bias,
                                          const float* rowdiv, int64_t m, int64_t n, int64_t k, int groups,
                                          const float* gamma, const float* beta, float eps, const float* residual,
                                          int64_t ldr, int act, float* lin_out, int64_t ld_lin, float* y, int64_t ldy,
                                          uint8_t* positive, void* ws, size_t ws_bytes, int form, void* stream) {
  using namespace rdm;
  RDM_REQUIRE(form >= 0 && form <= 2, "rdm_linear_group_norm_form: unknown form %d", form);
  RDM_REQUIRE(x && w && gamma && beta && lin_out && y, "rdm_linear_group_norm: null pointer");
  RDM_REQUIRE(k % 4 == 0 && ldx % 4 == 0 && ldw % 4 == 0, "rdm_linear_group_norm: K, ldx, ldw must be multiples of 4");
  if (m == 0) return RDM_OK;
  Arena ar(ws, ws_bytes);
  const size_t gemm_ws = rdm_gemm_workspace_bytes(m, n, 1);
  char* gws = ar.take<char>(gemm_ws);
  double* partial = ar.take<double>(static_cast<size_t>(gemm_stats_max_blocks(m)) * 2 * n);
  const size_t gn_ws = rdm_group_norm_workspace_bytes(m, n);
  char* nws = ar.take<char>(gn_ws);
  if (!ar.ok) {
    set_error("rdm_linear_group_norm: workspace too small (%zu < %zu)", ws_bytes, ar.off);
    return RDM_ERR_WORKSPACE;
  }
  int nblk = 0;
  if (int e = gemm_with_stats(x, ldx, w, ldw, lin_out, ld_lin, m, n, k, bias, rowdiv, gws, gemm_ws, partial, &nblk, stream, form))
    return e;
  return group_norm_finish(partial, nblk, lin_out, m, n, ld_lin, groups, gamma, beta, eps, residual, ldr, act, y, ldy,
                           positive, nws, gn_ws, stream);
}

extern "C" int rdm_patch_scores(const float* ref_feats, int64_t ld_ref, int64_t n_ref, const int64_t* ref_idx,
                                const float* src_feats, int64_t ld_src, int64_t n_src, const int64_t* src_idx, int64_t batch,
                                int64_t side, int64_t d, const float* rowdiv, float* scores, void* stream) {
  using namespace rdm;
  RDM_REQUIRE(ref_feats && src_feats && ref_idx && src_idx && scores, "rdm_patch_scores: null pointer");
  RDM_REQUIRE(batch >= 0 && side > 0 && d > 0 && d % 4 == 0 && ld_ref % 4 == 0 && ld_src % 4 == 0 && n_ref > 0 && n_src > 0,
              "rdm_patch_scores: bad sizes");
  RDM_REQUIRE(((reinterpret_cast<uintptr_t>(ref_feats) | reinterpret_cast<uintptr_t>(src_feats)) & 15) == 0,
              "rdm_patch_scores: features must be 16-byte aligned");
  if (batch == 0) return RDM_OK;
  GemmArgs g;
  g.A = ref_feats; g.B = src_feats; g.C = scores; g.bias = nullptr; g.rowdiv = rowdiv;
  g.M = static_cast<int>(side); g.N = static_cast<int>(side); g.K = static_cast<int>(d);
  g.lda = static_cast<int>(ld_ref); g.ldb = static_cast<int>(ld_src); g.ldc = static_cast<int>(side);
  g.sa = g.sb = 0; g.sc = side * side;
  g.act = 0; g.splits = 1; g.part = nullptr; g.stats = nullptr;
  g.A2 = nullptr; g.aidx = ref_idx; g.lda2 = g.ldi = g.c1 = 0; g.n_coarse = static_cast<int>(n_ref);
  g.bidx = src_idx; g.n_b = static_cast<int>(n_src);
  return gemm_dispatch(g, static_cast<int>(batch), true, nullptr, 0, nullptr, static_cast<hipStream_t>(stream));
}

extern "C" size_t rdm_decoder_stage_workspace_bytes(int64_t m, int64_t n, int64_t k) {
  return rdm_linear_group_norm_workspace_bytes(m, n) + rdm::align_up(static_cast<size_t>(m > 0 ? m : 1) * ((k + 3) / 4 * 4) * sizeof(float));
}

extern "C" int rdm_decoder_stage(const float* coarse, int64_t n_coarse, int64_t c1, int64_t ld1, const int64_t* idx, int64_t ldi,
                                 const float* skip, int64_t c2, int64_t ld2, int64_t m, const float* w, int64_t ldw,
                                 const float* bias, int64_t n, int groups, const float* gamma, const float* beta, float eps,
                                 int act, float* lin_out, int64_t ld_lin, float* y, int64_t ldy, void* ws, size_t ws_bytes,
                                 void* stream) {
  return rdm_decoder_stage_form(coarse, n_coarse, c1, ld1, idx, ldi, skip, c2, ld2, m, w, ldw, bias, n, groups, gamma, beta, eps, act, lin_out, ld_lin,
                                y, ldy, ws, ws_bytes, 0, stream);
}

extern "C" int rdm_decoder_stage_form(const float* coarse, int64_t n_coarse, int64_t c1, int64_t ld1, const int64_t* idx, int64_t ldi,
                                      const float* skip, int64_t c2, int64_t ld2, int64_t m, const float* w, int64_t ldw,
                                      const float* bias, int64_t n, int groups, const float* gamma, const float* beta, float eps,
                                      int act, float* lin_out, int64_t ld_lin, float* y, int64_t ldy, void* ws, size_t ws_bytes,
                                      int form, void* stream) {
  using namespace rdm;
  RDM_REQUIRE(form >= 0 && form <= 2, "rdm_decoder_stage_form: unknown form %d", form);
  RDM_REQUIRE(coarse && idx && skip && w && lin_out && (!gamma || (beta && y)), "rdm_decoder_stage: null pointer");
  RDM_REQUIRE(c1 > 0 && c2 > 0 && n > 0 && m >= 0 && ldw % 4 == 0, "rdm_decoder_stage: bad sizes");
  if (m == 0) return RDM_OK;
  const int64_t k = c1 + c2, kpad = (k + 3) / 4 * 4;
  static const bool no_virtual = ::rdm::dev_knob("RDM_NO_VIRTUAL_CONCAT") != nullptr;
  Arena ar(ws, ws_bytes);
  const size_t gemm_ws = rdm_gemm_workspace_bytes(m, n, 1);
  char* gws = ar.take<char>(gemm_ws);
  double* partial = ar.take<double>(static_cast<size_t>(gemm_stats_max_blocks(m)) * 2 * n);
  const size_t gn_ws = rdm_group_norm_workspace_bytes(m, n);
  char* nws = ar.take<char>(gn_ws);
  float* cat = ar.take<float>(static_cast<size_t>(m) * kpad);
  if (!ar.ok) {
    set_error("rdm_decoder_stage: workspace too small (%zu < %zu)", ws_bytes, ar.off);
    return RDM_ERR_WORKSPACE;
  }
  int nblk = 0;
  int rc = 1;
  if (!no_virtual && k == kpad)
    rc = gemm_concat_with_stats(coarse, ld1, c1, n_coarse, idx, ldi, skip, ld2, c2, w, ldw, lin_out, ld_lin, m, n, bias, 0, gws,
                                gemm_ws, gamma ? partial : nullptr, &nblk, stream, form);
  if (rc == 1) {
    if (int e = rdm_upsample_concat(coarse, n_coarse, c1, ld1, idx, ldi, skip, c2, ld2, m, cat, kpad, stream)) return e;
    rc = gemm_with_stats(cat, kpad, w, ldw, lin_out, ld_lin, m, n, kpad, bias, nullptr, gws, gemm_ws, gamma ? partial : nullptr,
                         &nblk, stream, form);
  }
  if (rc != 0 || !gamma) return rc;
  return group_norm_finish(partial, nblk, lin_out, m, n, ld_lin, groups, gamma, beta, eps, nullptr, 0, act, y, ldy, nullptr, nws,
                           gn_ws, stream);
}

extern "C" int rdm_linear_layer_norm(const float* x, int64_t ldx, const float* w, int64_t ldw, const float* bias, int64_t m,
                                     int64_t n, int64_t k, const float* residual, int64_t ldr, const float* gamma,
                                     const float* beta, float eps, int act, float* y, int64_t ldy, void* stream) {
  using namespace rdm;
  RDM_REQUIRE(x && w && gamma && beta && y, "rdm_linear_layer_norm: null pointer");
  RDM_REQUIRE(n == 128 && k >= 16 && k % 16 == 0 && m >= 0 && ldx % 4 == 0 && ldw >= k && ldw % 4 == 0 && act >= 0 && act <= 1,
              "rdm_linear_layer_norm: supports n = 128, k multiple of 16 (n=%lld k=%lld)", (long long)n, (long long)k);
  RDM_REQUIRE((reinterpret_cast<uintptr_t>(x) & 15) == 0 && (reinterpret_cast<uintptr_t>(w) & 15) == 0,
              "rdm_linear_layer_norm: x and w must be 16-byte aligned");
  if (m == 0) return RDM_OK;
  LinLnArgs a;
  a.A = x; a.B = w; a.bias = bias; a.res = residual; a.gamma = gamma; a.beta = beta; a.out = y;
  a.M = static_cast<int>(m); a.K = static_cast<int>(k); a.lda = static_cast<int>(ldx); a.ldb = static_cast<int>(ldw);
  a.ldr = static_cast<int>(ldr); a.ldo = static_cast<int>(ldy); a.act = act; a.eps = eps;
  ::rdm::launch<linear_ln128_body, linear_ln128_kernel, 256>(dim3(static_cast<unsigned>(ceil_div<int64_t>(m, 16))), 0, static_cast<hipStream_t>(stream), a);
  return launch_status("linear_ln128_kernel");
}

extern "C" int rdm_attention_tail(const float* hidden, int64_t ld_hidden, const float* x, int64_t ldx, int64_t m, int64_t d,
                                       const float* wo, int64_t ld_wo, const float* bo, const float* gamma1, const float* beta1,
                                       const float* w1, int64_t ld_w1, const float* b1, const float* w2, int64_t ld_w2,
                                       const float* b2, const float* gamma2, const float* beta2, float eps, float* out,
                                       int64_t ld_out, void* stream) {
  using namespace rdm;
  RDM_REQUIRE(hidden && x && wo && w1 && w2 && gamma1 && beta1 && gamma2 && beta2 && out, "rdm_attention_tail: null pointer");
  RDM_REQUIRE(d == 128 && m >= 0, "rdm_attention_tail: supports d = 128 with a 256-wide FFN (d=%lld)", (long long)d);
  RDM_REQUIRE(ld_hidden % 4 == 0 && ld_wo % 4 == 0 && ld_w1 % 4 == 0 && ld_w2 % 4 == 0 && ld_wo >= 128 && ld_w1 >= 128 &&
                  ld_w2 >= 256 && ld_hidden >= 128 && ldx >= 128 && ld_out >= 128,
              "rdm_attention_tail: bad leading dimensions");
  RDM_REQUIRE(((reinterpret_cast<uintptr_t>(hidden) | reinterpret_cast<uintptr_t>(wo) | reinterpret_cast<uintptr_t>(w1) |
                reinterpret_cast<uintptr_t>(w2)) & 15) == 0,
              "rdm_attention_tail: hidden and the weights must be 16-byte aligned");
  if (m == 0) return RDM_OK;
  TailArgs a;
  a.hid = hidden; a.x = x; a.wo = wo; a.bo = bo; a.g1 = gamma1; a.be1 = beta1; a.w1 = w1; a.b1 = b1; a.w2 = w2; a.b2 = b2;
  a.g2 = gamma2; a.be2 = beta2; a.out = out; a.M = static_cast<int>(m); a.ldh = static_cast<int>(ld_hidden);
  a.ldx = static_cast<int>(ldx); a.ldo = static_cast<int>(ld_out); a.ldwo = static_cast<int>(ld_wo);
  a.ldw1 = static_cast<int>(ld_w1); a.ldw2 = static_cast<int>(ld_w2); a.eps = eps;
  a.packed = nullptr;
  RDM_DUP_LOOP("tail")
  ::rdm::launch<attention_tail128_body<false>, attention_tail128_kernel<false>, 512>(dim3(static_cast<unsigned>(ceil_div<int64_t>(m, 16))), 0, static_cast<hipStream_t>(stream), a);
  return launch_status("attention_tail128_kernel");
}

extern "C" size_t rdm_attention_tail_packed_floats(void) { return 81920; }

extern "C" int rdm_attention_tail_pack_weights(const float* wo, int64_t ld_wo, const float* w1, int64_t ld_w1, const float* w2,
                                               int64_t ld_w2, float* packed, void* stream) {
  using namespace rdm;
  RDM_REQUIRE(wo && w1 && w2 && packed, "rdm_attention_tail_pack_weights: null pointer");
  RDM_REQUIRE(ld_wo % 4 == 0 && ld_w1 % 4 == 0 && ld_w2 % 4 == 0 && ld_wo >= 128 && ld_w1 >= 128 && ld_w2 >= 256,
// ... 30 lines not shown
```

### rdmnet_amd/csrc/internal.h

```cpp
#pragma once
#include <cstddef>
#include <cstdint>

namespace rdm {

int gemm_with_stats(const float* a, int64_t lda, const float* b, int64_t ldb, float* c, int64_t ldc, int64_t m,
                    int64_t n, int64_t k, const float* bias, const float* rowdiv, void* ws, size_t ws_bytes,
                    double* gn_partial, int* gn_blocks, void* stream, int form = 0);

void gemm_set_lds_pad(unsigned bytes);
int gemm_concat_with_stats(const float* coarse, int64_t ld1, int64_t c1, int64_t n_coarse, const int64_t* idx, int64_t ldi,
                           const float* skip, int64_t ld2, int64_t c2, const float* b, int64_t ldb, float* c, int64_t ldc,
                           int64_t m, int64_t n, const float* bias, int act, void* ws, size_t ws_bytes, double* gn_partial,
                           int* gn_blocks, void* stream, int form = 0);

int gemm_pair(const float* a0, int64_t lda0, const float* b0, int64_t ldb0, float* c0, int64_t ldc0, int64_t m0, int64_t n0,
              int64_t k0, const float* bias0, const float* a1, int64_t lda1, const float* b1, int64_t ldb1, float* c1,
              int64_t ldc1, int64_t m1, int64_t n1, int64_t k1, const float* bias1, void* ws, size_t ws_bytes, void* stream);

inline int64_t gemm_stats_max_blocks(int64_t m) { return (m + 7) / 8 + 1; }

int grid_subsample_mode(const float* points, int64_t n_points, const int64_t* lengths, int batch, float voxel_size,
                        float* out_points, int64_t* out_lengths, void* ws, size_t ws_bytes, void* stream, int mode);

int group_norm_finish(const double* partial, int nblk, const float* x, int64_t n, int64_t c, int64_t ldx, int groups,
                      const float* gamma, const float* beta, float eps, const float* residual, int64_t ldr, int act,
                      float* y, int64_t ldy, uint8_t* positive, void* ws, size_t ws_bytes, void* stream, int form = 0);

int gather_rows_multi(int n, const void* const* x, const int64_t* n_src, const int64_t* words, const int64_t* ldx,
                      const int64_t* const* idx, const int64_t* m, void* const* y, const int64_t* ldy, void* stream);

int radius_grid_build_multi(int n, const float* const* s_points, const int64_t* n_s, const int64_t* const* s_lengths, int batch,
                            const float* radius, void* const* grid_ws, const size_t* grid_ws_bytes, void* stream);

int radius_grid_build_trivial(const float* s_points, int64_t n_s, const int64_t* s_lengths, int batch, void* grid_ws,
                              size_t grid_ws_bytes, void* stream);

int compact_indices_pair(const uint8_t* keep, int64_t n_ref, int64_t n, int32_t* order, int32_t* counts,
                         const int32_t* mirror_src, int32_t* mirror_dst, int mirror_words, void* stream);

int gather_max_ordered(const float* x, int64_t n_s, int64_t c, int64_t ldx, const int64_t* idx, int64_t m, int64_t h, int64_t ldi,
                       const int32_t* width, float* y, int64_t ldy, const float* order_records, int i32, void* stream);
int kpconv_gather_impl(const float* q_points, int64_t m, const float* s_points, int64_t n_s, const float* s_feats, int64_t c,
                       int64_t ldf, const uint8_t* s_positive, const int64_t* idx, int64_t h, int64_t ldi, const int32_t* width,
                       const float* kernel_points, float sigma, float* wf, int64_t ldw, float* nn, const float* order_records,
                       int i32, void* stream, int form = 0);
bool kpconv_tile_gather_applies(int64_t c, int64_t h, bool has_order);
int kpconv_tile_gather(const float* q_points, int64_t m, const float* s_points, int64_t n_s, const float* s_feats, int64_t c,
                       int64_t ldf, const uint8_t* s_positive, const int64_t* idx, int64_t h, int64_t ldi, const int32_t* width,
                       const float* kernel_points, float sigma, float* wf, int64_t ldw, float* nn, const float* order_records,
                       int i32, void* stream);
int kpconv_fused_impl(const float* q_points, int64_t m, const float* s_points, int64_t n_s, const float* s_feats, int64_t c,
                      int64_t ldf, const uint8_t* s_positive, const int64_t* idx, int64_t h, int64_t ldi, const int32_t* width,
                      const float* kernel_points, float sigma, const float* w_packed, const float* bias, int64_t c_out, float* out,
                      int64_t ldo, double* gn_partial, const float* order_records, int form, int i32, void* stream);

size_t radius_redo_queue_bytes();
void radius_redo_queue_reset(void* queue);
int radius_grid_query_deferred(void* grid_ws, size_t grid_ws_bytes, int64_t n_s, const float* q_points, int64_t n_q,
                               const int64_t* q_lengths, int batch, float radius, int width, int64_t* out_idx,
                               int32_t* out_counts, int32_t* out_max, int32_t* status, unsigned char* redo_flags, void* queue,
                               int i32, void* stream);
int radius_redo_flush(void* queue, void* stream);

}
```

### rdmnet_amd/csrc/kpconv_fused.hip

```cpp
#include <atomic>
#include <cstdlib>

#include "../../include/rdmnet_hip.h"
#include "common.h"
#include "internal.h"
#include "lockstep.h"

namespace {

using namespace rdm;

typedef float f32x4 __attribute__((ext_vector_type(4)));

constexpr int kKP = 15;
constexpr int kMaxH = 128;

__device__ __forceinline__ float kp_influence(float dx, float dy, float dz, float inv_sigma) {
#pragma clang fp contract(off)
  const float xx = dx * dx, zz = dz * dz;
  const float d2 = __builtin_fmaf(dy, dy, xx) + zz;
  return fmaxf(0.f, __builtin_fmaf(-inv_sigma, __builtin_amdgcn_sqrtf(d2), 1.f));
}

struct FusedArgs {
  const float* q_points;
  const float* s_points;
  const float* s_feats;
  const unsigned char* s_pos;
  const int64_t* idx;
  int i32;
  const float* kp;
  const int32_t* width;
  const float* w;
  const float* bias;
  float* out;
  double* stats;
  int M, Ns, H;
  int ldf, ldi, ldo;
  float sigma;
  int ctot;
  float* nn;
};

typedef float f32x2 __attribute__((ext_vector_type(2)));
__device__ __forceinline__ f32x2 kp_influence2(f32x2 dx, f32x2 dy, f32x2 dz, float inv_sigma) {
#pragma clang fp contract(off)
  const f32x2 xx = dx * dx, zz = dz * dz;
  const f32x2 d2 = __builtin_elementwise_fma(dy, dy, xx) + zz;
  const f32x2 sq = {__builtin_amdgcn_sqrtf(d2.x), __builtin_amdgcn_sqrtf(d2.y)};
  const f32x2 ninv = {-inv_sigma, -inv_sigma}, one = {1.f, 1.f};
  const f32x2 w = __builtin_elementwise_fma(ninv, sq, one);
  return f32x2{fmaxf(0.f, w.x), fmaxf(0.f, w.y)};
}

template <int C, int QB, int NW, int ITERS>
__device__ __forceinline__ void kpconv_fused_kernel_body(const dim3 blockIdx, const dim3 gridDim, FusedArgs a) {
  (void)blockIdx; (void)gridDim;
  constexpr int VEC = C / 16;
  constexpr int NT = C / 16;
  constexpr int RT = QB / 16;
  constexpr int TILES = NT * RT;
  constexpr int KS = NW / TILES;
  constexpr int K16 = kKP * C / 16;
  constexpr int LDW = kKP * C + 4;
  constexpr int QPW = QB / NW;
  constexpr int PF = 4;
  static_assert(TILES * KS == NW && QPW * NW == QB && (KS - 1) * TILES * 1024 <= NW * kMaxH * 16, "wavefront roles");
  extern __shared__ __attribute__((aligned(16))) float smem[];
  float* WF = smem;
  float4* nb_all = reinterpret_cast<float4*>(smem + QB * LDW);
  float* nn_s = smem + QB * LDW + NW * kMaxH * 4;
  const int wave = threadIdx.x >> 6, lane = threadIdx.x & 63;
  const int g = lane >> 4, j = lane & 15;
  float4* nb = nb_all + wave * kMaxH;
  const float kx = j < kKP ? a.kp[3 * j] : 0.f, ky = j < kKP ? a.kp[3 * j + 1] : 0.f, kz = j < kKP ? a.kp[3 * j + 2] : 0.f;
  const float inv_sigma = 1.0f / a.sigma;
  int H = a.H;
  if (a.width) H = min(H, *a.width);
  const int tw = wave % TILES, kh = wave / TILES, rt = tw / NT, ct = tw % NT;
  const float bias_v = a.bias[16 * ct + j];
  double st_s = 0.0, st_ss = 0.0;

  for (int it = 0; it < ITERS; ++it) {
    const int q0 = (blockIdx.x * ITERS + it) * QB;
    if (q0 >= a.M) break;
    for (int qq = 0; qq < QPW; ++qq) {
      const int ql = wave * QPW + qq, m = q0 + ql;
      if (m >= a.M) break;
      const float qx = a.q_points[3 * m], qy = a.q_points[3 * m + 1], qz = a.q_points[3 * m + 2];
      int positives = 0;
      f32x4 acc[VEC];
#pragma unroll
      for (int t = 0; t < VEC; ++t) acc[t] = f32x4{0.f, 0.f, 0.f, 0.f};
      for (int hc = 0; hc < H; hc += kMaxH) {
// ... 76 lines not shown
      const float4* wp = reinterpret_cast<const float4*>(a.w) + static_cast<int64_t>(ct) * 64 + lane;
      const int s_begin = kh * K16 / KS, s_end = (kh + 1) * K16 / KS;
#pragma unroll 4
      for (int s = s_begin; s < s_end; ++s) {
        const float4 bv = wp[static_cast<int64_t>(s) * NT * 64];
        const float4 av = *reinterpret_cast<const float4*>(arow + 16 * s);
        o0 = __builtin_amdgcn_mfma_f32_16x16x4f32(av.x, bv.x, o0, 0, 0, 0);
        o1 = __builtin_amdgcn_mfma_f32_16x16x4f32(av.y, bv.y, o1, 0, 0, 0);
        o0 = __builtin_amdgcn_mfma_f32_16x16x4f32(av.z, bv.z, o0, 0, 0, 0);
        o1 = __builtin_amdgcn_mfma_f32_16x16x4f32(av.w, bv.w, o1, 0, 0, 0);
      }
    }
    f32x4 o = o0 + o1;
    f32x4* red = reinterpret_cast<f32x4*>(nb_all);
    if (kh > 0) red[((kh - 1) * TILES + tw) * 64 + lane] = o;
    __syncthreads();
    if (kh == 0) {
#pragma unroll
      for (int k = 1; k < KS; ++k) o = o + red[((k - 1) * TILES + tw) * 64 + lane];
#pragma unroll
      for (int r = 0; r < 4; ++r) {
        const int ql = 16 * rt + 4 * g + r, m = q0 + ql;
        if (m < a.M) {
          float v = o[r] / nn_s[ql];
          v += bias_v;
          a.out[static_cast<int64_t>(m) * a.ldo + 16 * ct + j] = v;
          st_s += static_cast<double>(v);
          st_ss += static_cast<double>(v) * static_cast<double>(v);
        }
      }
    }
    __syncthreads();
  }
  if (a.stats) {
    st_s = (st_s + __shfl_xor(st_s, 16, 64)) + (__shfl_xor(st_s, 32, 64) + __shfl_xor(st_s, 48, 64));
    st_ss = (st_ss + __shfl_xor(st_ss, 16, 64)) + (__shfl_xor(st_ss, 32, 64) + __shfl_xor(st_ss, 48, 64));
    double* ex = reinterpret_cast<double*>(smem);
    if (kh == 0 && g == 0) {
      ex[(tw * 16 + j) * 2 + 0] = st_s;
      ex[(tw * 16 + j) * 2 + 1] = st_ss;
    }
    __syncthreads();
    if (threadIdx.x < C) {
      const int c = threadIdx.x, cti = c / 16, cj = c % 16;
      double s = 0.0, ss = 0.0;
#pragma unroll
      for (int r = 0; r < RT; ++r) {
        s += ex[((r * NT + cti) * 16 + cj) * 2 + 0];
        ss += ex[((r * NT + cti) * 16 + cj) * 2 + 1];
      }
      a.stats[(static_cast<int64_t>(blockIdx.x) * 2 + 0) * C + c] = s;
      a.stats[(static_cast<int64_t>(blockIdx.x) * 2 + 1) * C + c] = ss;
    }
  }
}
template <int C, int QB, int NW, int ITERS>
__global__ __launch_bounds__(64 * NW) void kpconv_fused_kernel(FusedArgs a) { kpconv_fused_kernel_body<C, QB, NW, ITERS>(blockIdx, gridDim, a); }


#ifdef RDM_TILE_TIMING
__device__ long long* rdm_tile_clk;
#define TILE_T0() long long tl_t = __builtin_amdgcn_s_memtime(); int tl_k = 0; const long long tl_rt0 = wall_clock64()
#define TILE_PHASE() do { const long long now = __builtin_amdgcn_s_memtime(); if (threadIdx.x == 0 && rdm_tile_clk) rdm_tile_clk[tl_blk * 8 + tl_k] = now - tl_t; tl_t = now; ++tl_k; } while (0)
__device__ long long* rdm_tile_wclk;
#define TILE_W(slot, val) do { if ((threadIdx.x & 63) == 0 && rdm_tile_wclk) rdm_tile_wclk[(tl_blk * 16 + (threadIdx.x >> 6)) * 8 + (slot)] = (val); } while (0)
#define TILE_NOW() __builtin_amdgcn_s_memtime()
#ifdef RDM_TILE_TRIP_STAMPS
#define TRIP_DECL() long long ts_a = 0, ts_b = 0, ts_c = 0, ts_d = 0, ts_t = 0
#define TRIP_BEGIN() ts_t = TILE_NOW()
#define TRIP_LDS(acc_) do { asm volatile("s_waitcnt lgkmcnt(0)" ::: "memory"); const long long n_ = TILE_NOW(); acc_ += n_ - ts_t; ts_t = n_; } while (0)
#define TRIP_REG(acc_, v_) do { asm volatile("" ::"v"(v_)); asm volatile("s_nop 0" ::: "memory"); const long long n_ = TILE_NOW(); acc_ += n_ - ts_t; ts_t = n_; } while (0)
#define TRIP_END() do { TILE_W(4, ts_a); TILE_W(5, ts_b); TILE_W(6, ts_c); TILE_W(7, ts_d); } while (0)
#endif
#else
#define TILE_T0() do { } while (0)
#define TILE_PHASE() do { } while (0)
#define TILE_W(slot, val) do { } while (0)
#define TILE_NOW() 0ll
#endif
#ifndef RDM_TILE_TRIP_STAMPS
#define TRIP_DECL() do { } while (0)
#define TRIP_BEGIN() do { } while (0)
#define TRIP_LDS(acc_) do { } while (0)
#define TRIP_REG(acc_, v_) do { } while (0)
#define TRIP_END() do { } while (0)
#endif
constexpr int kTileQB = 16;
constexpr int kTileHash = 1024;
constexpr int kTileProbes = 16;

template <int C> struct TileCfg;
#ifndef RDM_TILE32_NW
#define RDM_TILE32_NW 8
#define RDM_TILE32_CAP 240
#endif
template <> struct TileCfg<32> { static constexpr int NW = RDM_TILE32_NW, CAP = RDM_TILE32_CAP; };
template <> struct TileCfg<64> { static constexpr int NW = 8, CAP = 240; };

template <int C>
struct TileLds {
  static constexpr int CAP = TileCfg<C>::CAP;
  static constexpr int LDW = kKP * C + 4;
  static constexpr int R0 = kTileQB * LDW > (CAP + 1) * C ? kTileQB * LDW : (CAP + 1) * C;
  static constexpr size_t off_pts = static_cast<size_t>(R0) * 4;
  static constexpr size_t off_hkey = off_pts + static_cast<size_t>(CAP + 1) * 16;
  static constexpr size_t off_hval = off_hkey + kTileHash * 4;
// ... 308 lines not shown
    if (lane == 0) nn_s[ql] = static_cast<float>(positives[qq] > 1 ? positives[qq] : 1);
  }
  __syncthreads();

  const int ct = wave % TILES, khg = wave / TILES;
  const float bias_v = a.bias[16 * ct + j];
  f32x4* red = reinterpret_cast<f32x4*>(smem_raw + L::off_pts);
  f32x4 o = {0.f, 0.f, 0.f, 0.f};
#pragma unroll
  for (int sub = 0; sub < SPW; ++sub) {
    const int kh = khg * SPW + sub;
    f32x4 o0 = {0.f, 0.f, 0.f, 0.f}, o1 = {0.f, 0.f, 0.f, 0.f};
    const float* arow = R0 + j * LDW + 4 * g;
    const float4* wp = reinterpret_cast<const float4*>(a.w) + static_cast<int64_t>(ct) * 64 + lane;
    const int s_begin = kh * K16 / KS, s_end = (kh + 1) * K16 / KS;
#pragma unroll 4
    for (int s = s_begin; s < s_end; ++s) {
      const float4 bv = wp[static_cast<int64_t>(s) * NT * 64];
      const float4 av = *reinterpret_cast<const float4*>(arow + 16 * s);
      o0 = __builtin_amdgcn_mfma_f32_16x16x4f32(av.x, bv.x, o0, 0, 0, 0);
      o1 = __builtin_amdgcn_mfma_f32_16x16x4f32(av.y, bv.y, o1, 0, 0, 0);
      o0 = __builtin_amdgcn_mfma_f32_16x16x4f32(av.z, bv.z, o0, 0, 0, 0);
      o1 = __builtin_amdgcn_mfma_f32_16x16x4f32(av.w, bv.w, o1, 0, 0, 0);
    }
    const f32x4 os = o0 + o1;
    if (kh == 0) o = os;
    else red[((kh - 1) * TILES + ct) * 64 + lane] = os;
  }
  __syncthreads();
  TILE_PHASE();
  double st_s = 0.0, st_ss = 0.0;
  if (khg == 0) {
#pragma unroll
    for (int k = 1; k < KS; ++k) o = o + red[((k - 1) * TILES + ct) * 64 + lane];
#pragma unroll
    for (int r = 0; r < 4; ++r) {
      const int ql = 4 * g + r, m = mrow[ql];
      if (m >= 0) {
        float v = o[r] / nn_s[ql];
        v += bias_v;
        a.out[static_cast<int64_t>(m) * a.ldo + 16 * ct + j] = v;
        st_s += static_cast<double>(v);
        st_ss += static_cast<double>(v) * static_cast<double>(v);
      }
    }
  }
  if (a.stats) {
    st_s = (st_s + __shfl_xor(st_s, 16, 64)) + (__shfl_xor(st_s, 32, 64) + __shfl_xor(st_s, 48, 64));
    st_ss = (st_ss + __shfl_xor(st_ss, 16, 64)) + (__shfl_xor(st_ss, 32, 64) + __shfl_xor(st_ss, 48, 64));
    if (khg == 0 && g == 0) {
      a.stats[(static_cast<int64_t>(blk) * 2 + 0) * C + 16 * ct + j] = st_s;
      a.stats[(static_cast<int64_t>(blk) * 2 + 1) * C + 16 * ct + j] = st_ss;
    }
  }
  TILE_PHASE();
#ifdef RDM_TILE_TIMING
  if (threadIdx.x == 0 && rdm_tile_clk) rdm_tile_clk[tl_blk * 8 + 7] = n_slots + ((wall_clock64() - tl_rt0) << 16);
#endif
}
template <int C, bool GATHER = false>
__global__ __launch_bounds__(64 * TileCfg<C>::NW, (C == 32 && TileCfg<C>::NW == 8 ? 3 : 2) * TileCfg<C>::NW / 4) void kpconv_tile_kernel(FusedArgs a, const float4* __restrict__ order, int xcd_ranges) { kpconv_tile_kernel_body<C, GATHER>(blockIdx, gridDim, a, order, xcd_ranges); }


constexpr int kC1Out = 64, kC1Waves = 16, kC1Qpw = 4;
__device__ __forceinline__ void kpconv_fused_c1_kernel_body(const dim3 blockIdx, const dim3 gridDim, FusedArgs a) {
  (void)blockIdx; (void)gridDim;
  __shared__ float4 nb_all[kC1Waves][kMaxH];
  __shared__ double ex[kC1Waves][kC1Out][2];
  const int wave = threadIdx.x >> 6, lane = threadIdx.x & 63;
  const int g = lane >> 4, j = lane & 15;
  float4* nb = nb_all[wave];
  const float kx = j < kKP ? a.kp[3 * j] : 0.f, ky = j < kKP ? a.kp[3 * j + 1] : 0.f, kz = j < kKP ? a.kp[3 * j + 2] : 0.f;
  const float inv_sigma = 1.0f / a.sigma;
  int H = a.H;
  if (a.width) H = min(H, *a.width);
  float wcol[kKP];
#pragma unroll
  for (int k = 0; k < kKP; ++k) wcol[k] = a.w[k * kC1Out + lane];
  const float bias_v = a.bias[lane];
  double st_s = 0.0, st_ss = 0.0;
  const int m0 = (blockIdx.x * kC1Waves + wave) * kC1Qpw;
  for (int qq = 0; qq < kC1Qpw; ++qq) {
    const int m = m0 + qq;
    if (m >= a.M) break;
    const float qx = a.q_points[3 * m], qy = a.q_points[3 * m + 1], qz = a.q_points[3 * m + 2];
    int positives = 0;
    float acc = 0.f;
    for (int hc = 0; hc < H; hc += kMaxH) {
      const int Hc = min(H - hc, kMaxH);
      int Hq = 0;
      for (int hb = 0; hb < Hc; hb += 64) {
        const int h = hb + lane;
        const int64_t id = h < Hc ? ld_index(a.idx, static_cast<int64_t>(m) * a.ldi + hc + h, a.i32) : -1;
        const unsigned long long rm = __builtin_amdgcn_ballot_w64(id >= 0 && id < a.Ns);
        if (rm) Hq = hb + 64 - __builtin_clzll(rm);
        float4 v = make_float4(0.f, 0.f, 0.f, 0.f);
        if (id >= 0 && id < a.Ns) {
          v.x = a.s_points[3 * id] - qx;
          v.y = a.s_points[3 * id + 1] - qy;
          v.z = a.s_points[3 * id + 2] - qz;
          v.w = a.s_feats[id * a.ldf];
          positives += a.s_pos[id];
        }
        if (h < Hc) nb[h] = v;
      }
      __builtin_amdgcn_fence(__ATOMIC_SEQ_CST, "wavefront");
      __builtin_amdgcn_wave_barrier();
      for (int h = g; h < Hq; h += 4) {
        const float4 v = nb[h];
        const float dx = v.x - kx, dy = v.y - ky, dz = v.z - kz;
        const float d2 = (dx * dx + dy * dy) + dz * dz;
        acc += fmaxf(0.f, 1.f - __builtin_amdgcn_sqrtf(d2) * inv_sigma) * v.w;
      }
      __builtin_amdgcn_fence(__ATOMIC_SEQ_CST, "wavefront");
      __builtin_amdgcn_wave_barrier();
    }
    positives = wave_sum_i(positives);
    acc += __shfl_xor(acc, 16, 64);
    acc += __shfl_xor(acc, 32, 64);
    float o = 0.f;
#pragma unroll
    for (int k = 0; k < kKP; ++k)
      o = fmaf(__builtin_bit_cast(float, __builtin_amdgcn_readlane(__builtin_bit_cast(int, acc), k)), wcol[k], o);
    float v = o / static_cast<float>(positives > 1 ? positives : 1);
    v += bias_v;
    a.out[static_cast<int64_t>(m) * a.ldo + lane] = v;
    st_s += static_cast<double>(v);
    st_ss += static_cast<double>(v) * static_cast<double>(v);
  }
  if (a.stats) {
    ex[wave][lane][0] = st_s;
    ex[wave][lane][1] = st_ss;
    __syncthreads();
    if (wave == 0) {
      double s = 0.0, ss = 0.0;
#pragma unroll
      for (int w = 0; w < kC1Waves; ++w) {
        s += ex[w][lane][0];
        ss += ex[w][lane][1];
      }
      a.stats[(static_cast<int64_t>(blockIdx.x) * 2 + 0) * kC1Out + lane] = s;
      a.stats[(static_cast<int64_t>(blockIdx.x) * 2 + 1) * kC1Out + lane] = ss;
    }
  }
}
__global__ __launch_bounds__(64 * kC1Waves) void kpconv_fused_c1_kernel(FusedArgs a) { kpconv_fused_c1_kernel_body(blockIdx, gridDim, a); }


template <int C, int QB, int NW>
constexpr size_t fused_lds_bytes() { return sizeof(float) * (static_cast<size_t>(QB) * (kKP * C + 4) + NW * kMaxH * 4 + QB); }

constexpr int kQb32 = 16, kNw32 = 16, kIters32 = 1, kQb64 = 16, kNw64 = 8, kIters64 = 1;

}

extern "C" int rdm_kpconv_fused_enabled(void) {
  static const bool on = [] {
    const char* v = ::rdm::dev_knob("RDM_FUSED_KPCONV");
    return !(v != nullptr && v[0] == '0');
  }();
  return on ? 1 : 0;
}

extern "C" int rdm_kpconv_fused_supported(int64_t c_in, int64_t c_out) {
  return (c_in == 1 && c_out == kC1Out) || (c_in == 32 && c_out == 32) || (c_in == 64 && c_out == 64);
}

namespace {
bool use_tile(int64_t c_in, int64_t h, int64_t m, int64_t n_s, bool has_order, int form = 0) {
  static const bool on = [] {
    const char* v = ::rdm::dev_knob("RDM_KPCONV_TILE");
    return !(v != nullptr && v[0] == '0');
  }();
  if (!((c_in == 32 || c_in == 64) && h <= kMaxH)) return false;
  if (form != 0) return form >= 2;
  return on && has_order && (c_in == 32 || 2 * m > n_s);
}
int64_t rows_per_block(int64_t c_in) {
  static_assert(kTileQB == kQb32 * kIters32 && kTileQB == kQb64 * kIters64, "one partial-row count for both forms");
  return c_in == 1 ? kC1Waves * kC1Qpw : kTileQB;
}
}

bool rdm::kpconv_tile_gather_applies(int64_t c, int64_t h, bool has_order) {
  return has_order && c >= 128 && c % 64 == 0 && h <= kMaxH;
}
int rdm::kpconv_tile_gather(const float* q_points, int64_t m, const float* s_points, int64_t n_s, const float* s_feats, int64_t c,
                            int64_t ldf, const uint8_t* s_positive, const int64_t* idx, int64_t h, int64_t ldi, const int32_t* width,
                            const float* kernel_points, float sigma, float* wf, int64_t ldw, float* nn, const float* order_records,
                            int i32, void* stream) {
  using namespace rdm;
  RDM_REQUIRE(kpconv_tile_gather_applies(c, h, order_records != nullptr), "kpconv_tile_gather: unsupported shape");
  RDM_REQUIRE(ldf % 4 == 0 && ldw % 4 == 0 && (reinterpret_cast<uintptr_t>(s_feats) & 15) == 0 && (reinterpret_cast<uintptr_t>(wf) & 15) == 0,
              "kpconv_tile_gather: features / WF must be 16-byte aligned with row strides that are multiples of 4");
  if (m == 0) return RDM_OK;
  FusedArgs a{};
// ... 8 lines not shown
  RDM_DUP_LOOP("gather")
  ::rdm::launch<kpconv_tile_kernel_body<64, true>, kpconv_tile_kernel<64, true>, 64 * TileCfg<64>::NW, 2 * TileCfg<64>::NW / 4>(grid, TileLds<64>::bytes, static_cast<hipStream_t>(stream), a,
                     reinterpret_cast<const float4*>(order_records), 1);
  return launch_status("kpconv_tile_kernel<64, gather>");
}

extern "C" int64_t rdm_kpconv_fused_partial_rows(int64_t m, int64_t c_in) {
  return m <= 0 ? 0 : rdm::ceil_div<int64_t>(m, rows_per_block(c_in));
}

extern "C" size_t rdm_kpconv_packed_floats(int64_t c_in, int64_t c_out) {
  return c_in == 1 ? static_cast<size_t>(16) * c_out : static_cast<size_t>(kKP) * c_in * c_out;
}

extern "C" int rdm_kpconv_pack_weights(const float* w, int64_t c_in, int64_t c_out, float* packed) {
  using namespace rdm;
  RDM_REQUIRE(w && packed && rdm_kpconv_fused_supported(c_in, c_out), "rdm_kpconv_pack_weights: unsupported (%lld -> %lld)",
              (long long)c_in, (long long)c_out);
  if (c_in == 1) {
    for (int64_t k = 0; k < 16; ++k)
      for (int64_t c = 0; c < c_out; ++c) packed[k * c_out + c] = k < kKP ? w[k * c_out + c] : 0.f;
    return RDM_OK;
  }
  const int64_t nt = c_out / 16, k16 = kKP * c_in / 16;
  for (int64_t s = 0; s < k16; ++s)
    for (int64_t t = 0; t < nt; ++t)
      for (int64_t lane = 0; lane < 64; ++lane)
        for (int64_t e = 0; e < 4; ++e)
          packed[((s * nt + t) * 64 + lane) * 4 + e] = w[(16 * s + 4 * (lane >> 4) + e) * c_out + 16 * t + (lane & 15)];
  return RDM_OK;
}

extern "C" int rdm_kpconv_fused(const float* q_points, int64_t m, const float* s_points, int64_t n_s, const float* s_feats,
                                int64_t c, int64_t ldf, const uint8_t* s_positive, const int64_t* idx, int64_t h,
                                int64_t ldi, const int32_t* width, const float* kernel_points, float sigma,
                                const float* w_packed, const float* bias, int64_t c_out, float* out, int64_t ldo,
                                double* gn_partial, const float* order_records, void* stream) {
  return rdm_kpconv_fused_form(q_points, m, s_points, n_s, s_feats, c, ldf, s_positive, idx, h, ldi, width, kernel_points, sigma,
                               w_packed, bias, c_out, out, ldo, gn_partial, order_records, 0, stream);
}

extern "C" int rdm_kpconv_fused_form(const float* q_points, int64_t m, const float* s_points, int64_t n_s, const float* s_feats,
                                     int64_t c, int64_t ldf, const uint8_t* s_positive, const int64_t* idx, int64_t h,
                                     int64_t ldi, const int32_t* width, const float* kernel_points, float sigma,
                                     const float* w_packed, const float* bias, int64_t c_out, float* out, int64_t ldo,
                                     double* gn_partial, const float* order_records, int form, void* stream) {
  return rdm::kpconv_fused_impl(q_points, m, s_points, n_s, s_feats, c, ldf, s_positive, idx, h, ldi, width, kernel_points, sigma,
                                w_packed, bias, c_out, out, ldo, gn_partial, order_records, form, 0, stream);
}

int rdm::kpconv_fused_impl(const float* q_points, int64_t m, const float* s_points, int64_t n_s, const float* s_feats, int64_t c,
                           int64_t ldf, const uint8_t* s_positive, const int64_t* idx, int64_t h, int64_t ldi, const int32_t* width,
                           const float* kernel_points, float sigma, const float* w_packed, const float* bias, int64_t c_out,
                           float* out, int64_t ldo, double* gn_partial, const float* order_records, int form, int i32, void* stream) {
  using namespace rdm;
  RDM_REQUIRE(form >= 0 && form <= 3, "rdm_kpconv_fused_form: form must be 0, 1 or 2 (3: lab variant of 2 without the XCD ranges)");
  RDM_REQUIRE(q_points && s_points && s_feats && s_positive && idx && kernel_points && w_packed && bias && out,
              "rdm_kpconv_fused: null pointer");
  RDM_REQUIRE(rdm_kpconv_fused_supported(c, c_out), "rdm_kpconv_fused: unsupported channel counts %lld -> %lld", (long long)c,
              (long long)c_out);
  RDM_REQUIRE(m >= 0 && n_s > 0 && h > 0 && ldo >= c_out, "rdm_kpconv_fused: bad sizes (h=%lld)", (long long)h);
  RDM_REQUIRE(c == 1 || (ldf % 4 == 0 && (reinterpret_cast<uintptr_t>(s_feats) & 15) == 0 &&
                         (reinterpret_cast<uintptr_t>(w_packed) & 15) == 0),
              "rdm_kpconv_fused: features / packed weights must be 16-byte aligned with a row stride that is a multiple of 4");
  if (m == 0) return RDM_OK;
  FusedArgs a;
  a.q_points = q_points; a.s_points = s_points; a.s_feats = s_feats; a.s_pos = s_positive; a.idx = idx; a.i32 = i32 ? 1 : 0;
  a.kp = kernel_points;
  a.width = width; a.w = w_packed; a.bias = bias; a.out = out; a.stats = gn_partial;
  a.M = static_cast<int>(m); a.Ns = static_cast<int>(n_s); a.H = static_cast<int>(h);
  a.ldf = static_cast<int>(ldf); a.ldi = static_cast<int>(ldi); a.ldo = static_cast<int>(ldo); a.sigma = sigma;
  hipStream_t st = static_cast<hipStream_t>(stream);
  const unsigned blocks = static_cast<unsigned>(rdm_kpconv_fused_partial_rows(m, c));
  RDM_DUP_LOOP("fused") {
  if (c == 1) {
    ::rdm::launch<kpconv_fused_c1_kernel_body, kpconv_fused_c1_kernel, 64 * kC1Waves>(dim3(blocks), 0, st, a);
    continue;
  }
  if (use_tile(c, h, m, n_s, order_records != nullptr, form)) {
    static std::atomic<uint64_t> tattr32{0}, tattr64{0};
    const float4* order = reinterpret_cast<const float4*>(order_records);
    const int xcd_ranges = form == 3 ? 0 : 1;
    if (c == 32) {
      RDM_HIP_CHECK(set_max_dynamic_lds(reinterpret_cast<const void*>(kpconv_tile_kernel<32>), static_cast<int>(TileLds<32>::bytes), tattr32));
      ::rdm::launch<kpconv_tile_kernel_body<32>, kpconv_tile_kernel<32>, 64 * TileCfg<32>::NW, (TileCfg<32>::NW == 8 ? 3 : 2) * TileCfg<32>::NW / 4>(dim3(blocks), TileLds<32>::bytes, st, a, order, xcd_ranges);
    } else {
      RDM_HIP_CHECK(set_max_dynamic_lds(reinterpret_cast<const void*>(kpconv_tile_kernel<64>), static_cast<int>(TileLds<64>::bytes), tattr64));
      ::rdm::launch<kpconv_tile_kernel_body<64>, kpconv_tile_kernel<64>, 64 * TileCfg<64>::NW, 2 * TileCfg<64>::NW / 4>(dim3(blocks), TileLds<64>::bytes, st, a, order, xcd_ranges);
    }
    continue;
  }
  static std::atomic<uint64_t> attr32{0}, attr64{0};
  RDM_HIP_CHECK(set_max_dynamic_lds(reinterpret_cast<const void*>(kpconv_fused_kernel<32, kQb32, kNw32, kIters32>),
                                    static_cast<int>(fused_lds_bytes<32, kQb32, kNw32>()), attr32));
  RDM_HIP_CHECK(set_max_dynamic_lds(reinterpret_cast<const void*>(kpconv_fused_kernel<64, kQb64, kNw64, kIters64>),
                                    static_cast<int>(fused_lds_bytes<64, kQb64, kNw64>()), attr64));
  const size_t lds32 = fused_lds_bytes<32, kQb32, kNw32>(), lds64 = fused_lds_bytes<64, kQb64, kNw64>();
  if (c == 32)
    ::rdm::launch<kpconv_fused_kernel_body<32, kQb32, kNw32, kIters32>, kpconv_fused_kernel<32, kQb32, kNw32, kIters32>, 64 * kNw32>(dim3(blocks), lds32, st, a);
  else
    ::rdm::launch<kpconv_fused_kernel_body<64, kQb64, kNw64, kIters64>, kpconv_fused_kernel<64, kQb64, kNw64, kIters64>, 64 * kNw64>(dim3(blocks), lds64, st, a);
  }
  return launch_status("kpconv_fused_kernel");
}

extern "C" size_t rdm_kpconv_fused_workspace_bytes(int64_t m, int64_t c_in, int64_t c_out) {
  const size_t nblk = static_cast<size_t>(rdm_kpconv_fused_partial_rows(m > 0 ? m : 1, c_in));
  return rdm::align_up(nblk * 2 * c_out * sizeof(double)) + rdm_group_norm_workspace_bytes(m, c_out) + 256;
}

extern "C" int rdm_kpconv_fused_group_norm(const float* q_points, int64_t m, const float* s_points, int64_t n_s,
                                           const float* s_feats, int64_t c, int64_t ldf, const uint8_t* s_positive,
                                           const int64_t* idx, int64_t h, int64_t ldi, const int32_t* width,
                                           const float* kernel_points, float sigma, const float* w_packed, const float* bias,
                                           int64_t c_out, int groups, const float* gamma, const float* beta, float eps, int act,
                                           float* conv_out, int64_t ld_conv, float* y, int64_t ldy, void* ws, size_t ws_bytes,
                                           const float* order_records, void* stream) {
  using namespace rdm;
  RDM_REQUIRE(gamma && beta && conv_out && y, "rdm_kpconv_fused_group_norm: null pointer");
  if (m == 0) return RDM_OK;
  Arena ar(ws, ws_bytes);
  const int nblk = static_cast<int>(rdm_kpconv_fused_partial_rows(m, c));
  double* partial = ar.take<double>(static_cast<size_t>(nblk) * 2 * c_out);
  const size_t gn_ws = rdm_group_norm_workspace_bytes(m, c_out);
  char* nws = ar.take<char>(gn_ws);
  if (!ar.ok) {
    set_error("rdm_kpconv_fused_group_norm: workspace too small (%zu < %zu)", ws_bytes, ar.off);
    return RDM_ERR_WORKSPACE;
  }
  if (int e = rdm_kpconv_fused(q_points, m, s_points, n_s, s_feats, c, ldf, s_positive, idx, h, ldi, width, kernel_points, sigma,
                               w_packed, bias, c_out, conv_out, ld_conv, partial, order_records, stream))
    return e;
  return group_norm_finish(partial, nblk, conv_out, m, c_out, ld_conv, groups, gamma, beta, eps, nullptr, 0, act, y, ldy, nullptr,
                           nws, gn_ws, stream);
}

#ifdef RDM_TILE_TIMING
extern "C" int rdm_dbg_tile_timing(long long* buffer) {
  RDM_HIP_CHECK(hipMemcpyToSymbol(HIP_SYMBOL(rdm_tile_clk), &buffer, sizeof(buffer)));
  return rdm::RDM_OK;
}
extern "C" int rdm_dbg_tile_wave_timing(long long* buffer) {
  RDM_HIP_CHECK(hipMemcpyToSymbol(HIP_SYMBOL(rdm_tile_wclk), &buffer, sizeof(buffer)));
  return rdm::RDM_OK;
}
#endif
```

### rdmnet_amd/csrc/norm.hip

```cpp
#include "../../include/rdmnet_hip.h"
#include "common.h"
#include "internal.h"
#include "lockstep.h"

namespace {

using namespace rdm;

constexpr int kGnRowsPerBlock = 64;

__device__ __forceinline__ void gn_partial_kernel_body(const dim3 blockIdx, const dim3 gridDim, const float* x, int n, int c, int ld,
                                                         double* partial) {
  (void)blockIdx; (void)gridDim;
  __shared__ double red[2][256];
  const int r0 = blockIdx.x * kGnRowsPerBlock;
  const int r1 = min(n, r0 + kGnRowsPerBlock);
  const int cw = c < 256 ? c : 256;
  const int lanes = 256 / cw;
  const int col_in = threadIdx.x % cw, rl = threadIdx.x / cw;
  const int col = blockIdx.y * 256 + col_in;
  double s = 0.0, ss = 0.0;
  if (rl < lanes && col < c)
    for (int r = r0 + rl; r < r1; r += lanes) {
      const double v = x[static_cast<int64_t>(r) * ld + col];
      s += v;
      ss += v * v;
    }
  red[0][threadIdx.x] = s;
  red[1][threadIdx.x] = ss;
  __syncthreads();
  if (threadIdx.x < cw && col < c) {
    double a = 0.0, b = 0.0;
    for (int k = 0; k < lanes; ++k) {
      a += red[0][k * cw + threadIdx.x];
      b += red[1][k * cw + threadIdx.x];
    }
    partial[(static_cast<int64_t>(blockIdx.x) * 2 + 0) * c + col] = a;
    partial[(static_cast<int64_t>(blockIdx.x) * 2 + 1) * c + col] = b;
  }
}
__global__ __launch_bounds__(256) void gn_partial_kernel(const float* x, int n, int c, int ld,
                                                         double* partial) { gn_partial_kernel_body(blockIdx, gridDim, x, n, c, ld, partial); }


template <int COLS>
struct GnFinalizeLds {
  double sh[2][1024 / COLS][COLS];
};
template <int COLS>
__device__ __forceinline__ float2 gn_scale_shift(GnFinalizeLds<COLS>& L, int col0, const double* partial, int nblk, int n, int c,
                                                 int groups, const float* gamma, const float* beta, float eps) {
  constexpr int LANES = 1024 / COLS;
  const int ci = threadIdx.x % COLS, lane = threadIdx.x / COLS;
  const int col = col0 + ci;
  double s = 0.0, ss = 0.0;
  if (col < c)
    for (int b0 = lane; b0 < nblk; b0 += 4 * LANES) {
      double p0[4], p1[4];
#pragma unroll
      for (int u = 0; u < 4; ++u) {
        const int b = b0 + LANES * u;
        p0[u] = b < nblk ? partial[(static_cast<int64_t>(b) * 2 + 0) * c + col] : 0.0;
        p1[u] = b < nblk ? partial[(static_cast<int64_t>(b) * 2 + 1) * c + col] : 0.0;
      }
#pragma unroll
      for (int u = 0; u < 4; ++u) {
        s += p0[u];
        ss += p1[u];
      }
    }
  L.sh[0][lane][ci] = s;
  L.sh[1][lane][ci] = ss;
  __syncthreads();
  if (lane == 0) {
    double a = 0.0, b = 0.0;
    for (int k = 0; k < LANES; ++k) {
      a += L.sh[0][k][ci];
      b += L.sh[1][k][ci];
    }
    L.sh[0][0][ci] = a;
    L.sh[1][0][ci] = b;
  }
  __syncthreads();
  float2 out = make_float2(0.f, 0.f);
  if (lane == 0 && col < c) {
    const int cpg = c / groups;
    const int g0 = (ci / cpg) * cpg;
    double gs = 0.0, gss = 0.0;
    for (int k = 0; k < cpg; ++k) {
      gs += L.sh[0][0][g0 + k];
      gss += L.sh[1][0][g0 + k];
    }
    const double cnt = static_cast<double>(n) * cpg;
    const double mean = gs / cnt;
    double var = gss / cnt - mean * mean;
    if (var < 0.0) var = 0.0;
    const double rstd = 1.0 / sqrt(var + static_cast<double>(eps));
    const double gsc = rstd * static_cast<double>(gamma[col]);
    out.x = static_cast<float>(gsc);
    out.y = static_cast<float>(static_cast<double>(beta[col]) - mean * gsc);
  }
  return out;
}
template <int COLS>
__device__ __forceinline__ void gn_finalize_kernel_body(const dim3 blockIdx, const dim3 gridDim, const double* partial, int nblk, int n,
                                                            int c, int groups, const float* gamma,
                                                            const float* beta, float eps, float* scale,
                                                            float* shift) {
  (void)blockIdx; (void)gridDim;
  __shared__ GnFinalizeLds<COLS> L;
  const float2 v = gn_scale_shift<COLS>(L, blockIdx.x * COLS, partial, nblk, n, c, groups, gamma, beta, eps);
  const int col = blockIdx.x * COLS + threadIdx.x % COLS;
  if (threadIdx.x / COLS == 0 && col < c) {
    scale[col] = v.x;
    shift[col] = v.y;
  }
}
template <int COLS>
__global__ __launch_bounds__(1024) void gn_finalize_kernel(const double* partial, int nblk, int n,
                                                            int c, int groups, const float* gamma,
                                                            const float* beta, float eps, float* scale,
                                                            float* shift) { gn_finalize_kernel_body<COLS>(blockIdx, gridDim, partial, nblk, n, c, groups, gamma, beta, eps, scale, shift); }


constexpr int kGnFusedRows = 256;
__device__ __forceinline__ void gn_finalize_apply_kernel_body(const dim3 blockIdx, const dim3 gridDim, const double* partial, int nblk, const float* x, int n, int c, int ldx,
                                                                  int groups, const float* gamma, const float* beta, float eps,
                                                                  const float* res, int ldr, int act, float* y, int ldy) {
  (void)blockIdx; (void)gridDim;
  __shared__ GnFinalizeLds<64> L;
  __shared__ float sc_l[64], sh_l[64];
  const int col0 = blockIdx.x * 64;
  const float2 v = gn_scale_shift<64>(L, col0, partial, nblk, n, c, groups, gamma, beta, eps);
  if (threadIdx.x < 64) {
    sc_l[threadIdx.x] = v.x;
    sh_l[threadIdx.x] = v.y;
  }
  __syncthreads();
  const int q = threadIdx.x & 15, rl = threadIdx.x >> 4;
  const int col = col0 + 4 * q;
  if (col >= c) return;
  const float4 sc = *reinterpret_cast<const float4*>(sc_l + 4 * q), sh = *reinterpret_cast<const float4*>(sh_l + 4 * q);
  const int r1 = min(n, (static_cast<int>(blockIdx.y) + 1) * kGnFusedRows);
  for (int row = blockIdx.y * kGnFusedRows + rl; row < r1; row += 64) {
    const float4 xv = *reinterpret_cast<const float4*>(x + static_cast<int64_t>(row) * ldx + col);
    float o[4] = {__builtin_fmaf(xv.x, sc.x, sh.x), __builtin_fmaf(xv.y, sc.y, sh.y), __builtin_fmaf(xv.z, sc.z, sh.z),
                  __builtin_fmaf(xv.w, sc.w, sh.w)};
    if (res) {
      const float4 rv = *reinterpret_cast<const float4*>(res + static_cast<int64_t>(row) * ldr + col);
      o[0] += rv.x; o[1] += rv.y; o[2] += rv.z; o[3] += rv.w;
    }
#pragma unroll
    for (int k = 0; k < 4; ++k) {
      if (act == 2) o[k] = o[k] > 0.f ? o[k] : 0.1f * o[k];
      else if (act == 1) o[k] = o[k] > 0.f ? o[k] : 0.f;
    }
    *reinterpret_cast<float4*>(y + static_cast<int64_t>(row) * ldy + col) = make_float4(o[0], o[1], o[2], o[3]);
  }
}
__global__ __launch_bounds__(1024) void gn_finalize_apply_kernel(const double* partial, int nblk, const float* x, int n, int c, int ldx,
                                                                  int groups, const float* gamma, const float* beta, float eps,
                                                                  const float* res, int ldr, int act, float* y, int ldy) { gn_finalize_apply_kernel_body(blockIdx, gridDim, partial, nblk, x, n, c, ldx, groups, gamma, beta, eps, res, ldr, act, y, ldy); }


__device__ __forceinline__ void gn_apply_kernel_body(const dim3 blockIdx, const dim3 gridDim, const float* x, int n, int c, int ldx,
                                                       const float* scale, const float* shift,
                                                       const float* res, int ldr, int act, float* y,
                                                       int ldy, unsigned char* positive) {
  (void)blockIdx; (void)gridDim;
  const int row = blockIdx.x * 4 + (threadIdx.x >> 6);
  if (row >= n) return;
  const int lane = threadIdx.x & 63;
  float rs = 0.f;
  for (int col = lane; col < c; col += 64) {
    float v = x[static_cast<int64_t>(row) * ldx + col] * scale[col] + shift[col];
    if (res) v += res[static_cast<int64_t>(row) * ldr + col];
    if (act == 2) v = v > 0.f ? v : 0.1f * v;
    else if (act == 1) v = v > 0.f ? v : 0.f;
    y[static_cast<int64_t>(row) * ldy + col] = v;
    rs += v;
  }
  if (positive) {
    rs = wave_sum(rs);
    if (lane == 0) positive[row] = rs > 0.f ? 1 : 0;
  }
}
// ... 224 lines not shown
}
__global__ void gather_rows_multi_kernel(GatherBatch b) { gather_rows_multi_kernel_body(blockIdx, gridDim, b); }


}

int rdm::gather_rows_multi(int n, const void* const* x, const int64_t* n_src, const int64_t* words, const int64_t* ldx,
                           const int64_t* const* idx, const int64_t* m, void* const* y, const int64_t* ldy, void* stream) {
  RDM_REQUIRE(n >= 1 && n <= 4, "gather_rows_multi: 1..4 gathers");
  GatherBatch b;
  b.n = n;
  b.first_block[0] = 0;
  int64_t max_words = 0;
  for (int k = 0; k < n; ++k) max_words = std::max(max_words, words[k]);
  const int threads = max_words >= 256 ? 256 : (max_words >= 128 ? 128 : 64);
  for (int k = 0; k < n; ++k) {
    RDM_REQUIRE(x[k] && idx[k] && y[k] && words[k] > 0 && m[k] >= 0, "gather_rows_multi: bad arguments");
    int lanes = 1;
    while (lanes < words[k] && lanes < threads) lanes <<= 1;
    b.item[k] = GatherItem{static_cast<const uint32_t*>(x[k]), static_cast<int>(n_src[k]), static_cast<int>(words[k]),
                           static_cast<int>(ldx[k]), idx[k], static_cast<uint32_t*>(y[k]), static_cast<int>(ldy[k]),
                           static_cast<int>(m[k]), lanes};
    b.first_block[k + 1] = b.first_block[k] + static_cast<int>(ceil_div<int64_t>(m[k], threads / lanes));
  }
  if (b.first_block[n] == 0) return RDM_OK;
  const dim3 grid(static_cast<unsigned>(b.first_block[n]));
  hipStream_t st = static_cast<hipStream_t>(stream);
  if (threads == 256) ::rdm::launch<gather_rows_multi_kernel_body, gather_rows_multi_kernel, 256>(grid, 0, st, b);
  else if (threads == 128) ::rdm::launch<gather_rows_multi_kernel_body, gather_rows_multi_kernel, 128>(grid, 0, st, b);
  else ::rdm::launch<gather_rows_multi_kernel_body, gather_rows_multi_kernel, 64>(grid, 0, st, b);
  return launch_status("gather_rows_multi_kernel");
}

extern "C" int rdm_gather_rows(const void* x, int64_t n_src, int64_t words, int64_t ldx, const int64_t* idx,
                               int64_t m, void* y, int64_t ldy, void* stream) {
  using namespace rdm;
  RDM_REQUIRE(x && idx && y && words > 0, "rdm_gather_rows: bad arguments");
  if (m == 0) return RDM_OK;
  const int threads = words >= 256 ? 256 : (words >= 128 ? 128 : 64);
  if (threads == 256) ::rdm::launch<gather_rows_kernel_body, gather_rows_kernel, 256>(dim3(static_cast<unsigned>(m)), 0, static_cast<hipStream_t>(stream), static_cast<const uint32_t*>(x), static_cast<int>(n_src),
                     static_cast<int>(words), static_cast<int>(ldx), idx, static_cast<int>(m),
                     static_cast<uint32_t*>(y), static_cast<int>(ldy));
  else if (threads == 128) ::rdm::launch<gather_rows_kernel_body, gather_rows_kernel, 128>(dim3(static_cast<unsigned>(m)), 0, static_cast<hipStream_t>(stream), static_cast<const uint32_t*>(x), static_cast<int>(n_src),
                     static_cast<int>(words), static_cast<int>(ldx), idx, static_cast<int>(m),
                     static_cast<uint32_t*>(y), static_cast<int>(ldy));
  else ::rdm::launch<gather_rows_kernel_body, gather_rows_kernel, 64>(dim3(static_cast<unsigned>(m)), 0, static_cast<hipStream_t>(stream), static_cast<const uint32_t*>(x), static_cast<int>(n_src),
                     static_cast<int>(words), static_cast<int>(ldx), idx, static_cast<int>(m),
                     static_cast<uint32_t*>(y), static_cast<int>(ldy));
  return launch_status("gather_rows_kernel");
}

extern "C" size_t rdm_group_norm_workspace_bytes(int64_t n, int64_t c) {
  const size_t nblk = static_cast<size_t>(rdm::ceil_div<int64_t>(n > 0 ? n : 1, kGnRowsPerBlock));
  return rdm::align_up(nblk * 2 * c * sizeof(double)) + rdm::align_up(2 * c * sizeof(float));
}

int rdm::group_norm_finish(const double* partial_in, int nblk, const float* x, int64_t n, int64_t c, int64_t ldx,
                           int groups, const float* gamma, const float* beta, float eps, const float* residual,
                           int64_t ldr, int act, float* y, int64_t ldy, uint8_t* positive, void* ws, size_t ws_bytes,
                           void* stream, int form) {
  Arena ar(ws, ws_bytes);
  const int own_blk = static_cast<int>(ceil_div<int64_t>(n, kGnRowsPerBlock));
  double* partial = ar.take<double>(static_cast<size_t>(own_blk) * 2 * c);
  float* ss = ar.take<float>(2 * c);
  if (!ar.ok) {
    set_error("rdm_group_norm: workspace too small (%zu < %zu)", ws_bytes, ar.off);
    return RDM_ERR_WORKSPACE;
  }
  hipStream_t st = static_cast<hipStream_t>(stream);
  const double* use = partial_in;
  if (nblk <= 0) {
    ::rdm::launch<gn_partial_kernel_body, gn_partial_kernel, 256>(dim3(own_blk, ceil_div<int64_t>(c, 256)), 0, st, x,
                       static_cast<int>(n), static_cast<int>(c), static_cast<int>(ldx), partial);
    use = partial;
    nblk = own_blk;
  }
  const bool vec_ok = c % 4 == 0 && ldx % 4 == 0 && ldy % 4 == 0 && (!residual || ldr % 4 == 0) &&
                      (reinterpret_cast<uintptr_t>(x) & 15) == 0 && (reinterpret_cast<uintptr_t>(y) & 15) == 0 &&
                      (!residual || (reinterpret_cast<uintptr_t>(residual) & 15) == 0);
  static const bool fin64 = ::rdm::dev_knob("RDM_GN_FINALIZE_64") != nullptr;
  const bool narrow = !fin64 && nblk >= 128 && c / groups <= 16 && 16 % (c / groups) == 0;
  if (form != 1 && !narrow && !positive && vec_ok && c % 64 == 0 && n <= 4096) {
    RDM_DUP_LOOP("gnfin")
    ::rdm::launch<gn_finalize_apply_kernel_body, gn_finalize_apply_kernel, 1024>(dim3(static_cast<unsigned>(c / 64), static_cast<unsigned>(ceil_div<int64_t>(n, kGnFusedRows))), 0, st, use, nblk, x, static_cast<int>(n), static_cast<int>(c), static_cast<int>(ldx), groups, gamma, beta,
                       eps, residual, static_cast<int>(ldr), act, y, static_cast<int>(ldy));
    return launch_status("gn_finalize_apply_kernel");
  }
  {
    RDM_DUP_LOOP("gnfin")
    if (narrow)
      ::rdm::launch<gn_finalize_kernel_body<16>, gn_finalize_kernel<16>, 1024>(dim3(ceil_div<int64_t>(c, 16)), 0, st, use, nblk,
                         static_cast<int>(n), static_cast<int>(c), groups, gamma, beta, eps, ss, ss + c);
    else
    ::rdm::launch<gn_finalize_kernel_body<64>, gn_finalize_kernel<64>, 1024>(dim3(ceil_div<int64_t>(c, 64)), 0, st, use, nblk,
                       static_cast<int>(n), static_cast<int>(c), groups, gamma, beta, eps, ss, ss + c);
  }
  static const bool narrow_rows = ::rdm::dev_knob("RDM_GN_APPLY_ROWS") != nullptr;
  const int64_t c4 = c / 4;
  const bool flag_ok = c4 == 8 || c4 == 16 || c4 == 32;
  const bool wide = vec_ok && (narrow_rows ? (!positive && c >= 256) : (!positive || flag_ok));
  RDM_DUP_LOOP("gnapply")
  if (wide)
    ::rdm::launch<gn_apply_wide_kernel_body, gn_apply_wide_kernel, 256>(dim3(ceil_div<int64_t>(n * (c / 4), 256)), 0, st, x, static_cast<int>(n),
                       static_cast<int>(c / 4), static_cast<int>(ldx), ss, ss + c, residual, static_cast<int>(ldr), act, y,
                       static_cast<int>(ldy), positive);
  else
    ::rdm::launch<gn_apply_kernel_body, gn_apply_kernel, 256>(dim3(ceil_div<int64_t>(n, 4)), 0, st, x,
                       static_cast<int>(n), static_cast<int>(c), static_cast<int>(ldx), ss, ss + c, residual,
                       static_cast<int>(ldr), act, y, static_cast<int>(ldy), positive);
  return launch_status("group_norm kernels");
}

extern "C" int rdm_group_norm(const float* x, int64_t n, int64_t c, int64_t ldx, int groups,
                              const float* gamma, const float* beta, float eps, const float* residual,
                              int64_t ldr, int act, float* y, int64_t ldy, uint8_t* positive, void* ws,
                              size_t ws_bytes, void* stream) {
  using namespace rdm;
  RDM_REQUIRE(x && gamma && beta && y, "rdm_group_norm: null pointer");
  RDM_REQUIRE(n >= 0 && c > 0 && groups > 0 && c % groups == 0 && c <= 4096 && 64 % (c / groups) == 0,
              "rdm_group_norm: bad sizes (n=%lld c=%lld groups=%d)", (long long)n, (long long)c, groups);
  if (n == 0) return RDM_OK;
  return group_norm_finish(nullptr, 0, x, n, c, ldx, groups, gamma, beta, eps, residual, ldr, act, y, ldy, positive, ws,
                           ws_bytes, stream);
}

extern "C" int rdm_group_norm_form(const float* x, int64_t n, int64_t c, int64_t ldx, int groups, const float* gamma,
                                   const float* beta, float eps, const float* residual, int64_t ldr, int act, float* y, int64_t ldy,
                                   uint8_t* positive, void* ws, size_t ws_bytes, int form, void* stream) {
  RDM_REQUIRE(form >= 0 && form <= 1, "rdm_group_norm_form: form must be 0 (the library's choice) or 1 (statistics, finalize, apply as three launches)");
  using namespace rdm;
  RDM_REQUIRE(x && gamma && beta && y, "rdm_group_norm: null pointer");
  RDM_REQUIRE(n >= 0 && c > 0 && groups > 0 && c % groups == 0 && c <= 4096 && 64 % (c / groups) == 0,
              "rdm_group_norm: bad sizes (n=%lld c=%lld groups=%d)", (long long)n, (long long)c, groups);
  if (n == 0) return RDM_OK;
  return group_norm_finish(nullptr, 0, x, n, c, ldx, groups, gamma, beta, eps, residual, ldr, act, y, ldy, positive, ws, ws_bytes,
                           stream, form);
}

extern "C" int rdm_layer_norm(const float* x, int64_t n, int64_t c, int64_t ldx, const float* residual,
                              int64_t ldr, const float* gamma, const float* beta, float eps, int act,
                              float* y, int64_t ldy, void* stream) {
  using namespace rdm;
  RDM_REQUIRE(x && gamma && beta && y, "rdm_layer_norm: null pointer");
  RDM_REQUIRE(n >= 0 && c > 0 && c <= 2048, "rdm_layer_norm: bad sizes");
  if (n == 0) return RDM_OK;
  RDM_DUP_LOOP("ln")
  ::rdm::launch<layernorm_kernel_body, layernorm_kernel, 256>(dim3(ceil_div<int64_t>(n, 4)), 0, static_cast<hipStream_t>(stream), x, static_cast<int>(n), static_cast<int>(c),
                     static_cast<int>(ldx), residual, static_cast<int>(ldr), gamma, beta, eps, act, y,
                     static_cast<int>(ldy));
  return launch_status("layernorm_kernel");
}

int rdm::gather_max_ordered(const float* x, int64_t n_s, int64_t c, int64_t ldx, const int64_t* idx, int64_t m, int64_t h,
                            int64_t ldi, const int32_t* width, float* y, int64_t ldy, const float* order_records, int i32, void* stream) {
  RDM_REQUIRE(x && idx && y, "rdm_gather_max: null pointer");
  RDM_REQUIRE(c % 4 == 0 && ldx % 4 == 0 && ldy % 4 == 0 && h > 0, "rdm_gather_max: bad sizes");
  if (m == 0) return RDM_OK;
  static const bool no_order = ::rdm::dev_knob("RDM_NO_POOL_ORDER") != nullptr;
  if (no_order) order_records = nullptr;
  hipStream_t st = static_cast<hipStream_t>(stream);
  const float4* ord = reinterpret_cast<const float4*>(order_records);
  const int ns = static_cast<int>(n_s), ci = static_cast<int>(c), lx = static_cast<int>(ldx), mi = static_cast<int>(m), hi = static_cast<int>(h),
            li = static_cast<int>(ldi), ly = static_cast<int>(ldy);
  RDM_DUP_LOOP("pool") {
    if (c <= 64)
      ::rdm::launch<gather_max_kernel_body<16>, gather_max_kernel<16>, 256>(dim3(ceil_div<int64_t>(m, 16), 1), 0, st, x, ns, ci, lx, idx, mi, hi, li, width, y, ly, ord, i32);
    else if (c <= 128)
      ::rdm::launch<gather_max_kernel_body<32>, gather_max_kernel<32>, 256>(dim3(ceil_div<int64_t>(m, 8), 1), 0, st, x, ns, ci, lx, idx, mi, hi, li, width, y, ly, ord, i32);
    else if (m * ceil_div<int64_t>(c, 256) <= 4096)
      ::rdm::launch<gather_max_kernel_body<64, true>, gather_max_kernel<64, true>, 256>(dim3(static_cast<unsigned>(m), ceil_div<int64_t>(c, 256)), 0, st, x, ns, ci, lx,
                         idx, mi, hi, li, width, y, ly, ord, i32);
    else
      ::rdm::launch<gather_max_kernel_body<64>, gather_max_kernel<64>, 256>(dim3(ceil_div<int64_t>(m, 4), ceil_div<int64_t>(c, 256)), 0, st, x, ns, ci, lx, idx, mi,
                         hi, li, width, y, ly, ord, i32);
  }
  return launch_status("gather_max_kernel");
}

extern "C" int rdm_gather_max(const float* x, int64_t n_s, int64_t c, int64_t ldx, const int64_t* idx,
                              int64_t m, int64_t h, int64_t ldi, const int32_t* width, float* y,
                              int64_t ldy, void* stream) {
  return rdm::gather_max_ordered(x, n_s, c, ldx, idx, m, h, ldi, width, y, ldy, nullptr, 0, stream);
}

__device__ __forceinline__ void upsample_concat_vec_kernel_body(const dim3 blockIdx, const dim3 gridDim, const float* coarse, int n_coarse, int c1, int ld1,
                                                                  const int64_t* idx, int ldi, const float* skip, int c2, int ld2,
                                                                  int m_total, float* y, int ldy) {
  (void)blockIdx; (void)gridDim;
  const int m = blockIdx.x * 4 + (threadIdx.x >> 6);
// ... 45 lines not shown
```

Measured before the change: 599.7.

## Fold group-norm finalize into producer kernels via last-block atomic counters

Adds a 'last block done' tail to GEMM, split-K stat reduce, KPConv and GN partial kernels. Per-chunk atomic counters, kept in a reserved arena region and reset once per run, let the final block compute scale and shift. This removes the separate group-norm finalize launch and its reads of the partial statistics. The cost is extra LDS and an atomic per block, a rotating set of counters that must stay consistent across runs, and possible serialization on the last block.

```diff
diff --git a/rdmnet_amd/csrc/engine.hip b/rdmnet_amd/csrc/engine.hip
--- a/rdmnet_amd/csrc/engine.hip
+++ b/rdmnet_amd/csrc/engine.hip
@@ -13,6 +13,7 @@
 #include <ctime>
 
 #include "common.h"
+#include "gn_tail.h"
 #include "internal.h"
 #include "lockstep.h"
 
@@ -128,10 +129,16 @@
     int k = 0;
   } gt;
 
+  static constexpr size_t kGnCounterSets = 64, kGnCounterBytes = kGnCounterSets * kGnMaxChunks * sizeof(int);
+  unsigned gn_seq = 0;
+  bool gn_dirty = true;
+  size_t arena_limit() const { return arena_cap > kGnCounterBytes ? (arena_cap - kGnCounterBytes) & ~size_t(255) : 0; }
+  int* gn_counters() { return arena_limit() ? reinterpret_cast<int*>(arena + arena_limit()) + (gn_seq++ % kGnCounterSets) * kGnMaxChunks : nullptr; }
+
   template <typename T>
   T* alloc(size_t count) {
     size_t bytes = align_up(count * sizeof(T) + 16);
-    if (arena_off + bytes > arena_cap) return nullptr;
+    if (arena_off + bytes > arena_limit()) return nullptr;
     T* r = reinterpret_cast<T*>(arena + arena_off);
     arena_off += bytes;
     return r;
@@ -231,8 +238,9 @@
   ENG_ALLOC(y.p);
   float *g, *b;
   ENG_CHECK(norm_params(r, name + ".norm", &g, &b));
-  return rdm_group_norm(x.p, x.rows, x.cols, x.ld, r.groups, g, b, 1e-5f, res ? res->p : nullptr, res ? res->ld : 0, act,
-                        y.p, y.ld, positive, r.ws, r.ws_bytes, r.st);
+  if (x.rows == 0) return RDM_OK;
+  return group_norm_finish(nullptr, 0, x.p, x.rows, x.cols, x.ld, r.groups, g, b, 1e-5f, res ? res->p : nullptr, res ? res->ld : 0,
+                           act, y.p, y.ld, positive, r.ws, r.ws_bytes, r.st, 0, e->gn_counters());
 }
 
 int unary(Run& r, const std::string& name, const Mat& x, Mat& y, int act, const Mat* res, uint8_t* positive) {
@@ -246,9 +254,9 @@
   ENG_ALLOC(t.p); ENG_ALLOC(y.p);
   float *g, *b;
   ENG_CHECK(norm_params(r, name + ".norm.norm", &g, &b));
-  return rdm_linear_group_norm(x.p, x.ld, L.b, L.ldb, L.bias, nullptr, x.rows, L.out, L.kpad, r.groups, g, b, 1e-5f,
-                               res ? res->p : nullptr, res ? res->ld : 0, act, t.p, t.ld, y.p, y.ld, positive, r.ws,
-                               r.ws_bytes, r.st);
+  return linear_group_norm_impl(x.p, x.ld, L.b, L.ldb, L.bias, nullptr, x.rows, L.out, L.kpad, r.groups, g, b, 1e-5f,
+                                res ? res->p : nullptr, res ? res->ld : 0, act, t.p, t.ld, y.p, y.ld, positive, r.ws,
+                                r.ws_bytes, 0, e->gn_counters(), r.st);
 }
 
 int decoder_stage(Run& r, const std::string& lin_name, const std::string* norm_name, const Mat& coarse, const int64_t* up_idx,
@@ -277,9 +285,11 @@
     ENG_ALLOC(ws);
     ws_bytes = need;
   }
-  return rdm_decoder_stage(coarse.p, coarse.rows, coarse.cols, coarse.ld, up_idx, up_ld, skip.p, skip.cols, skip.ld, m, L.b, L.ldb,
-                           L.bias, L.out, r.groups, g, b, 1e-5f, 2, t.p, t.ld, norm_name ? y.p : nullptr, norm_name ? y.ld : 0, ws,
-                           ws_bytes, r.st);
+  RDM_REQUIRE(coarse.p && up_idx && skip.p && L.b && coarse.cols > 0 && skip.cols > 0 && L.out > 0 && m >= 0 && L.ldb % 4 == 0,
+              "rdm_engine: bad decoder stage %s", lin_name.c_str());
+  return decoder_stage_impl(coarse.p, coarse.rows, coarse.cols, coarse.ld, up_idx, up_ld, skip.p, skip.cols, skip.ld, m, L.b, L.ldb,
+                            L.bias, L.out, r.groups, g, b, 1e-5f, 2, t.p, t.ld, norm_name ? y.p : nullptr, norm_name ? y.ld : 0, ws,
+                            ws_bytes, 0, e->gn_counters(), r.st);
 }
 
 int layer_norm(Run& r, const std::string& name, const Mat& x, const Mat* res, int act, Mat& y, bool alloc_out = true) {
@@ -336,12 +346,15 @@
     const int nblk = static_cast<int>(rdm_kpconv_fused_partial_rows(q.n, cin));
     double* gn_partial = static_cast<double*>(r.ws);
     const size_t stat_bytes = align_up(static_cast<size_t>(nblk) * 2 * W.out * sizeof(double));
+    GnFinalizeSpec fin{e->gn_counters(), gam, bet,
+                       group_norm_scale_slot(static_cast<char*>(r.ws) + stat_bytes, r.ws_bytes - stat_bytes, q.n, W.out), r.groups, 1e-5f,
+                       false};
     ENG_CHECK(kpconv_fused_impl(q.pts, q.n, s.pts, s.n, x.p, cin, x.ld, x_pos, t.idx, t.width, t.stride(), t.flags,
                                 vecp(r, name + ".kernel_points"), sigma, W.packed, W.bias, W.out, conv.p, conv.ld, gn_partial, order, 0,
-                                i32, r.st));
+                                i32, r.st, &fin));
     if (prof) ENG_CHECK(layer_event(e, 3 * li + 1, r.st));
     ENG_CHECK(group_norm_finish(gn_partial, nblk, conv.p, q.n, W.out, conv.ld, r.groups, gam, bet, 1e-5f, nullptr, 0, 2, y.p, y.ld,
-                                nullptr, static_cast<char*>(r.ws) + stat_bytes, r.ws_bytes - stat_bytes, r.st));
+                                nullptr, static_cast<char*>(r.ws) + stat_bytes, r.ws_bytes - stat_bytes, r.st, 0, fin.counters, fin.done));
     if (pool_src) {
       *pool_out = e->mat(q.n, pool_src->cols);
       ENG_ALLOC(pool_out->p);
@@ -366,8 +379,13 @@
   RDM_REQUIRE(gemm_ws + stat_bytes + rdm_group_norm_workspace_bytes(q.n, W.out) <= r.ws_bytes, "rdm_engine: scratch too small");
   double* gn_partial = reinterpret_cast<double*>(static_cast<char*>(r.ws) + gemm_ws);
   int gn_blocks = 0;
+  float *gam, *bet;
+  ENG_CHECK(norm_params(r, norm_name + ".norm", &gam, &bet));
+  char* nws = static_cast<char*>(r.ws) + gemm_ws + stat_bytes;
+  const size_t nws_bytes = r.ws_bytes - gemm_ws - stat_bytes;
+  GnFinalizeSpec fin{e->gn_counters(), gam, bet, group_norm_scale_slot(nws, nws_bytes, q.n, W.out), r.groups, 1e-5f, false};
   ENG_CHECK(gemm_with_stats(wf.p, wf.ld, W.b, W.ldb, conv.p, conv.ld, q.n, W.out, W.kpad, W.bias, nn, r.ws, gemm_ws,
-                            gn_partial, &gn_blocks, r.st));
+                            gn_partial, &gn_blocks, r.st, 0, &fin));
   if (pool_src) {
     *pool_out = e->mat(q.n, pool_src->cols);
     ENG_ALLOC(pool_out->p);
@@ -377,11 +395,8 @@
   if (prof) ENG_CHECK(end_profile(0));
   y = e->mat(q.n, W.out);
   ENG_ALLOC(y.p);
-  float *gam, *bet;
-  ENG_CHECK(norm_params(r, norm_name + ".norm", &gam, &bet));
   return group_norm_finish(gn_partial, gn_blocks, conv.p, q.n, W.out, conv.ld, r.groups, gam, bet, 1e-5f, nullptr, 0, 2, y.p,
-                           y.ld, nullptr, static_cast<char*>(r.ws) + gemm_ws + stat_bytes, r.ws_bytes - gemm_ws - stat_bytes,
-                           r.st);
+                           y.ld, nullptr, nws, nws_bytes, r.st, 0, fin.counters, fin.done);
 }
 
 int linear_ln(Run& r, const std::string& lin, const std::string& norm, const Mat& x, const Mat& res, Mat& y, bool alloc_out) {
@@ -667,6 +682,7 @@
   e->arena_cap = cfg->arena_bytes ? cfg->arena_bytes : (size_t(3) << 30);
   e->arena_fixed = cfg->arena_bytes != 0;
   hipError_t err = hipMalloc(reinterpret_cast<void**>(&e->arena), e->arena_cap);
+  e->gn_dirty = true;
   if (err != hipSuccess) {
     set_error("rdm_engine_create: hipMalloc(%zu) failed: %s", e->arena_cap, hipGetErrorString(err));
     delete e;
@@ -869,6 +885,7 @@
   e->arena_cap = bytes;
   e->arena_fixed = false;
   const hipError_t err = hipMalloc(reinterpret_cast<void**>(&e->arena), e->arena_cap);
+  e->gn_dirty = true;
   if (err != hipSuccess) {
     e->arena_cap = 0;
     set_error("rdm_engine_reserve: hipMalloc(%zu) failed: %s", bytes, hipGetErrorString(err));
@@ -1068,6 +1085,7 @@
   e->arena = nullptr;
   e->arena_cap *= 2;
   const hipError_t err = hipMalloc(reinterpret_cast<void**>(&e->arena), e->arena_cap);
+  e->gn_dirty = true;
   if (err != hipSuccess) {
     e->arena_cap = 0;
     set_error("%s: growing the activation arena failed: %s", who, hipGetErrorString(err));
@@ -1890,7 +1908,20 @@
 
 }
 
+static int engine_run_body(rdm_engine* e, const float* ref_points, int64_t n_ref, const float* src_points, int64_t n_src,
+                           const rdm_data_dict* dd, rdm_engine_result* res, void* stream, const PairPyramid* pre);
 static int engine_run_once(rdm_engine* e, const float* ref_points, int64_t n_ref, const float* src_points, int64_t n_src,
+                           const rdm_data_dict* dd, rdm_engine_result* res, void* stream, const PairPyramid* pre) {
+  if (e->gn_dirty && e->arena_limit()) {
+    fill_words<int>(reinterpret_cast<int*>(e->arena + e->arena_limit()), rdm_engine::kGnCounterBytes / sizeof(int), 0,
+                    static_cast<hipStream_t>(stream));
+    e->gn_dirty = false;
+  }
+  const int rc = engine_run_body(e, ref_points, n_ref, src_points, n_src, dd, res, stream, pre);
+  if (rc != RDM_OK) e->gn_dirty = true;
+  return rc;
+}
+static int engine_run_body(rdm_engine* e, const float* ref_points, int64_t n_ref, const float* src_points, int64_t n_src,
                            const rdm_data_dict* dd, rdm_engine_result* res, void* stream, const PairPyramid* pre) {
   const rdm_engine_config& c = e->cfg;
   e->arena_off = pre ? e->arena_base : 0;
diff --git a/rdmnet_amd/csrc/gemm.hip b/rdmnet_amd/csrc/gemm.hip
--- a/rdmnet_amd/csrc/gemm.hip
+++ b/rdmnet_amd/csrc/gemm.hip
@@ -4,6 +4,7 @@
 #include <type_traits>
 
 #include "common.h"
+#include "gn_tail.h"
 #include "internal.h"
 #include "lockstep.h"
 
@@ -33,6 +34,7 @@
   const int64_t* bidx;
   int n_b;
   int xcd_tiles;
+  GnTail tail;
 #ifdef RDM_GEMM_TIMING
   unsigned long long* clk;
 #endif
@@ -65,8 +67,9 @@
   constexpr int TPR = BN / 4;
   constexpr int RPI = 256 / TPR;
   constexpr int kBytesAB = (2 * BK * LDA_S + 2 * BK * LDB_S) * 4, kBytesC = CR * LDC_S * 4, kBytesStat = RPI * BN * 2 * 8;
-  constexpr int kBytes = kBytesAB > kBytesC ? (kBytesAB > kBytesStat ? kBytesAB : kBytesStat) : (kBytesC > kBytesStat ? kBytesC : kBytesStat);
-  static_assert((2 * BK * LDA_S * 4) % 16 == 0 && CR % RPI == 0, "tile layout");
+  constexpr int kBytes3 = kBytesAB > kBytesC ? (kBytesAB > kBytesStat ? kBytesAB : kBytesStat) : (kBytesC > kBytesStat ? kBytesC : kBytesStat);
+  constexpr int kBytes = kBytes3 > kGnTailLdsBytes ? kBytes3 : kGnTailLdsBytes;
+  static_assert((2 * BK * LDA_S * 4) % 16 == 0 && CR % RPI == 0 && kGnChunkCols % BN == 0, "tile layout");
   __shared__ __attribute__((aligned(16))) char smem[kBytes];
   float (*As)[BK][LDA_S] = reinterpret_cast<float (*)[BK][LDA_S]>(smem);
   float (*Bs)[BK][LDB_S] = reinterpret_cast<float (*)[BK][LDB_S]>(smem + 2 * BK * LDA_S * 4);
@@ -370,6 +373,12 @@
       }
       g.stats[(static_cast<long long>(tile_y) * 2 + 0) * g.N + col] = a;
       g.stats[(static_cast<long long>(tile_y) * 2 + 1) * g.N + col] = b;
+    }
+    if (g.tail.counter) {
+      constexpr int TPC = kGnChunkCols / BN;
+      const int chunk = tile_x / TPC;
+      const int col_tiles = min(static_cast<int>(gridDim.x), (chunk + 1) * TPC) - chunk * TPC;
+      gn_tail<256>(smem, g.tail, g.stats, g.M, g.N, chunk, col_tiles * static_cast<int>(gridDim.y));
     }
   }
   GEMM_STAMP(3);
@@ -682,6 +691,11 @@
       }
       lds_barrier();
     }
+  }
+  if (stats && g.tail.counter) {
+    const int chunk = blockIdx.x / 2;
+    const int col_tiles = min(static_cast<int>(gridDim.x), (chunk + 1) * 2) - chunk * 2;
+    gn_tail<256>(smem, g.tail, g.stats, g.M, g.N, chunk, col_tiles * static_cast<int>(gridDim.y));
   }
   GEMM_WIDE_STAMP(3);
 }
@@ -1019,7 +1033,8 @@
 inline int stat_rows_per_block(long long n) { return kStatRowsPerLane * (256 / static_cast<int>(n < 256 ? n : 256)); }
 __device__ __forceinline__ void splitk_reduce_stats_kernel_body(const dim3 blockIdx, const dim3 gridDim, GemmArgs g, double* stats) {
   (void)blockIdx; (void)gridDim;
-  __shared__ double red[2][256];
+  __shared__ __attribute__((aligned(16))) char lds[kGnTailLdsBytes];
+  double (*red)[256] = reinterpret_cast<double (*)[256]>(lds);
   const int cw = g.N < 256 ? g.N : 256;
   const int lanes = 256 / cw;
   const int r0 = blockIdx.x * (kStatRowsPerLane * lanes);
@@ -1067,6 +1082,7 @@
     stats[(static_cast<long long>(blockIdx.x) * 2 + 0) * g.N + col] = a;
     stats[(static_cast<long long>(blockIdx.x) * 2 + 1) * g.N + col] = b;
   }
+  if (g.tail.counter) gn_tail<256>(lds, g.tail, stats, g.M, g.N, blockIdx.y, gridDim.x);
 }
 __global__ __launch_bounds__(256) void splitk_reduce_stats_kernel(GemmArgs g, double* stats) { splitk_reduce_stats_kernel_body(blockIdx, gridDim, g, stats); }
 
@@ -1120,7 +1136,8 @@
 
 thread_local int g_last_plan[4] = {0, 0, 0, 0};
 
-int gemm_dispatch(GemmArgs g, int batches, bool trans_b, void* ws, size_t ws_bytes, int* stat_blocks, hipStream_t st, int form = 0) {
+int gemm_dispatch(GemmArgs g, int batches, bool trans_b, void* ws, size_t ws_bytes, int* stat_blocks, hipStream_t st, int form = 0,
+                  GnFinalizeSpec* fin = nullptr) {
   const long long m = g.M, n = g.N, k = g.K;
   const char* tune_env = ::rdm::dev_knob("RDM_GEMM_TUNE");
   if (batches == 1 && !trans_b && !g.rowdiv && !g.stats && !g.aidx && m <= 1536 && k % 16 == 0 && k >= 64 && k <= 1024 &&
@@ -1225,6 +1242,12 @@
   if (stat_blocks)
     *stat_blocks = g.stats ? static_cast<int>(ceil_div<long long>(m, wide ? 64 : bm))
                            : (reduce_stats ? static_cast<int>(ceil_div<long long>(m, stat_rows_per_block(n))) : 0);
+  if (fin) fin->done = false;
+  if (fin && fin->counters && fin->scale && (g.stats || reduce_stats) && n <= kGnChunkCols * kGnMaxChunks) {
+    const int nblk = g.stats ? static_cast<int>(ceil_div<long long>(m, wide ? 64 : bm)) : static_cast<int>(ceil_div<long long>(m, stat_rows_per_block(n)));
+    g.tail = GnTail{fin->counters, fin->gamma, fin->beta, fin->scale, nblk, fin->groups, gn_finalize_cols(nblk, n, fin->groups), fin->eps};
+    fin->done = true;
+  }
   g_last_plan[0] = bm; g_last_plan[1] = bn; g_last_plan[3] = g.splits;
   g_last_plan[2] = wide ? 32 : (tile == T128 ? 16 : ((tile == T64 ? (k >= 48 || g.aidx) : k >= 32) ? 32 : 16));
   RDM_DUP_LOOP("gemm") {
@@ -1269,7 +1292,7 @@
 
 int rdm::gemm_with_stats(const float* a, int64_t lda, const float* b, int64_t ldb, float* c, int64_t ldc, int64_t m,
                          int64_t n, int64_t k, const float* bias, const float* rowdiv, void* ws, size_t ws_bytes,
-                         double* gn_partial, int* gn_blocks, void* stream, int form) {
+                         double* gn_partial, int* gn_blocks, void* stream, int form, GnFinalizeSpec* fin) {
   GemmArgs g;
   g.A = a; g.B = b; g.C = c; g.bias = bias; g.rowdiv = rowdiv;
   g.M = static_cast<int>(m); g.N = static_cast<int>(n); g.K = static_cast<int>(k);
@@ -1277,13 +1300,13 @@
   g.sa = g.sb = g.sc = 0;
   g.act = 0; g.splits = 1; g.part = nullptr; g.stats = gn_partial;
   g.A2 = nullptr; g.aidx = nullptr; g.lda2 = g.ldi = g.c1 = g.n_coarse = 0; g.bidx = nullptr; g.n_b = 0;
-  return gemm_dispatch(g, 1, false, ws, ws_bytes, gn_blocks, static_cast<hipStream_t>(stream), form);
+  return gemm_dispatch(g, 1, false, ws, ws_bytes, gn_blocks, static_cast<hipStream_t>(stream), form, fin);
 }
 
 int rdm::gemm_concat_with_stats(const float* coarse, int64_t ld1, int64_t c1, int64_t n_coarse, const int64_t* idx, int64_t ldi,
                                 const float* skip, int64_t ld2, int64_t c2, const float* b, int64_t ldb, float* c, int64_t ldc,
                                 int64_t m, int64_t n, const float* bias, int act, void* ws, size_t ws_bytes, double* gn_partial,
-                                int* gn_blocks, void* stream, int form) {
+                                int* gn_blocks, void* stream, int form, GnFinalizeSpec* fin) {
   if (c1 % 32 != 0 || c2 % 4 != 0 || c2 < 4 || ld1 % 4 != 0 || ld2 % 4 != 0 || ldb % 4 != 0 || m <= 0 ||
       ((reinterpret_cast<uintptr_t>(coarse) | reinterpret_cast<uintptr_t>(skip) | reinterpret_cast<uintptr_t>(b)) & 15) != 0)
     return 1;
@@ -1296,7 +1319,7 @@
   g.A2 = skip; g.aidx = idx; g.lda2 = static_cast<int>(ld2); g.ldi = static_cast<int>(ldi); g.c1 = static_cast<int>(c1);
   g.n_coarse = static_cast<int>(n_coarse);
   g.bidx = nullptr; g.n_b = 0;
-  return gemm_dispatch(g, 1, false, ws, ws_bytes, gn_blocks, static_cast<hipStream_t>(stream), form);
+  return gemm_dispatch(g, 1, false, ws, ws_bytes, gn_blocks, static_cast<hipStream_t>(stream), form, fin);
 }
 
 namespace {
@@ -1389,6 +1412,15 @@
                                           int64_t ldr, int act, float* lin_out, int64_t ld_lin, float* y, int64_t ldy,
                                           uint8_t* positive, void* ws, size_t ws_bytes, int form, void* stream) {
   using namespace rdm;
+  return rdm::linear_group_norm_impl(x, ldx, w, ldw, bias, rowdiv, m, n, k, groups, gamma, beta, eps, residual, ldr, act, lin_out, ld_lin, y,
+                                     ldy, positive, ws, ws_bytes, form, nullptr, stream);
+}
+
+int rdm::linear_group_norm_impl(const float* x, int64_t ldx, const float* w, int64_t ldw, const float* bias,
+                                const float* rowdiv, int64_t m, int64_t n, int64_t k, int groups,
+                                const float* gamma, const float* beta, float eps, const float* residual,
+                                int64_t ldr, int act, float* lin_out, int64_t ld_lin, float* y, int64_t ldy,
+                                uint8_t* positive, void* ws, size_t ws_bytes, int form, int* counters, void* stream) {
   RDM_REQUIRE(form >= 0 && form <= 2, "rdm_linear_group_norm_form: unknown form %d", form);
   RDM_REQUIRE(x && w && gamma && beta && lin_out && y, "rdm_linear_group_norm: null pointer");
   RDM_REQUIRE(k % 4 == 0 && ldx % 4 == 0 && ldw % 4 == 0, "rdm_linear_group_norm: K, ldx, ldw must be multiples of 4");
@@ -1404,10 +1436,12 @@
     return RDM_ERR_WORKSPACE;
   }
   int nblk = 0;
-  if (int e = gemm_with_stats(x, ldx, w, ldw, lin_out, ld_lin, m, n, k, bias, rowdiv, gws, gemm_ws, partial, &nblk, stream, form))
+  GnFinalizeSpec fin{counters, gamma, beta, nullptr, groups, eps, false};
+  fin.scale = group_norm_scale_slot(nws, gn_ws, m, n, counters ? nullptr : &fin.counters, stream);
+  if (int e = gemm_with_stats(x, ldx, w, ldw, lin_out, ld_lin, m, n, k, bias, rowdiv, gws, gemm_ws, partial, &nblk, stream, form, &fin))
     return e;
   return group_norm_finish(partial, nblk, lin_out, m, n, ld_lin, groups, gamma, beta, eps, residual, ldr, act, y, ldy,
-                           positive, nws, gn_ws, stream);
+                           positive, nws, gn_ws, stream, 0, fin.counters, fin.done);
 }
 
 extern "C" int rdm_patch_scores(const float* ref_feats, int64_t ld_ref, int64_t n_ref, const int64_t* ref_idx,
@@ -1449,7 +1483,15 @@
                                       const float* bias, int64_t n, int groups, const float* gamma, const float* beta, float eps,
                                       int act, float* lin_out, int64_t ld_lin, float* y, int64_t ldy, void* ws, size_t ws_bytes,
                                       int form, void* stream) {
-  using namespace rdm;
+  return rdm::decoder_stage_impl(coarse, n_coarse, c1, ld1, idx, ldi, skip, c2, ld2, m, w, ldw, bias, n, groups, gamma, beta, eps, act, lin_out,
+                                 ld_lin, y, ldy, ws, ws_bytes, form, nullptr, stream);
+}
+
+int rdm::decoder_stage_impl(const float* coarse, int64_t n_coarse, int64_t c1, int64_t ld1, const int64_t* idx, int64_t ldi,
+                            const float* skip, int64_t c2, int64_t ld2, int64_t m, const float* w, int64_t ldw,
+                            const float* bias, int64_t n, int groups, const float* gamma, const float* beta, float eps,
+                            int act, float* lin_out, int64_t ld_lin, float* y, int64_t ldy, void* ws, size_t ws_bytes,
+                            int form, int* counters, void* stream) {
   RDM_REQUIRE(form >= 0 && form <= 2, "rdm_decoder_stage_form: unknown form %d", form);
   RDM_REQUIRE(coarse && idx && skip && w && lin_out && (!gamma || (beta && y)), "rdm_decoder_stage: null pointer");
   RDM_REQUIRE(c1 > 0 && c2 > 0 && n > 0 && m >= 0 && ldw % 4 == 0, "rdm_decoder_stage: bad sizes");
@@ -1469,17 +1511,19 @@
   }
   int nblk = 0;
   int rc = 1;
+  GnFinalizeSpec fin{counters, gamma, beta, nullptr, groups, eps, false};
+  if (gamma) fin.scale = group_norm_scale_slot(nws, gn_ws, m, n, counters ? nullptr : &fin.counters, stream);
   if (!no_virtual && k == kpad)
     rc = gemm_concat_with_stats(coarse, ld1, c1, n_coarse, idx, ldi, skip, ld2, c2, w, ldw, lin_out, ld_lin, m, n, bias, 0, gws,
-                                gemm_ws, gamma ? partial : nullptr, &nblk, stream, form);
+                                gemm_ws, gamma ? partial : nullptr, &nblk, stream, form, gamma ? &fin : nullptr);
   if (rc == 1) {
     if (int e = rdm_upsample_concat(coarse, n_coarse, c1, ld1, idx, ldi, skip, c2, ld2, m, cat, kpad, stream)) return e;
     rc = gemm_with_stats(cat, kpad, w, ldw, lin_out, ld_lin, m, n, kpad, bias, nullptr, gws, gemm_ws, gamma ? partial : nullptr,
-                         &nblk, stream, form);
+                         &nblk, stream, form, gamma ? &fin : nullptr);
   }
   if (rc != 0 || !gamma) return rc;
   return group_norm_finish(partial, nblk, lin_out, m, n, ld_lin, groups, gamma, beta, eps, nullptr, 0, act, y, ldy, nullptr, nws,
-                           gn_ws, stream);
+                           gn_ws, stream, 0, fin.counters, fin.done);
 }
 
 extern "C" int rdm_linear_layer_norm(const float* x, int64_t ldx, const float* w, int64_t ldw, const float* bias, int64_t m,
diff --git a/rdmnet_amd/csrc/gn_tail.h b/rdmnet_amd/csrc/gn_tail.h
--- /dev/null
+++ b/rdmnet_amd/csrc/gn_tail.h
@@ -0,0 +1,138 @@
+#pragma once
+#include <hip/hip_runtime.h>
+
+#include <cstdint>
+
+#include "common.h"
+
+namespace rdm {
+
+constexpr int kGnChunkCols = 256;
+constexpr int kGnMaxChunks = 16;
+constexpr int kGnTailLdsBytes = 2 * 1024 * 8 + 16;
+
+struct GnTail {
+  int* counter = nullptr;
+  const float* gamma = nullptr;
+  const float* beta = nullptr;
+  float* scale = nullptr;
+  int nblk = 0;
+  int groups = 1;
+  int cols = 64;
+  float eps = 0.f;
+};
+inline GnTail gn_tail_none() { return GnTail{}; }
+
+inline int gn_finalize_cols(int nblk, int64_t c, int groups) {
+  static const bool fin64 = dev_knob("RDM_GN_FINALIZE_64") != nullptr;
+  return (!fin64 && nblk >= 128 && c / groups <= 16 && 16 % (c / groups) == 0) ? 16 : 64;
+}
+
+#ifdef __HIPCC__
+template <int COLS>
+struct GnFinalizeLds {
+  double sh[2][1024 / COLS][COLS];
+};
+template <int COLS, int THREADS>
+__device__ __forceinline__ float2 gn_scale_shift(GnFinalizeLds<COLS>& L, int col0, const double* partial, int nblk, int n, int c,
+                                                 int groups, const float* gamma, const float* beta, float eps) {
+  constexpr int LANES = 1024 / COLS;
+  static_assert(THREADS % 64 == 0 && 1024 % THREADS == 0 && THREADS >= COLS, "gn_scale_shift: workgroup size");
+  for (int vt = threadIdx.x; vt < 1024; vt += THREADS) {
+    const int ci = vt % COLS, lane = vt / COLS;
+    const int col = col0 + ci;
+    double s = 0.0, ss = 0.0;
+    if (col < c)
+      for (int b0 = lane; b0 < nblk; b0 += 4 * LANES) {
+        double p0[4], p1[4];
+#pragma unroll
+        for (int u = 0; u < 4; ++u) {
+          const int b = b0 + LANES * u;
+          p0[u] = b < nblk ? partial[(static_cast<int64_t>(b) * 2 + 0) * c + col] : 0.0;
+          p1[u] = b < nblk ? partial[(static_cast<int64_t>(b) * 2 + 1) * c + col] : 0.0;
+        }
+#pragma unroll
+        for (int u = 0; u < 4; ++u) {
+          s += p0[u];
+          ss += p1[u];
+        }
+      }
+    L.sh[0][lane][ci] = s;
+    L.sh[1][lane][ci] = ss;
+  }
+  __syncthreads();
+  const int ci = threadIdx.x % COLS;
+  const bool first = threadIdx.x < COLS;
+  const int col = col0 + ci;
+  if (first) {
+    double a = 0.0, b = 0.0;
+    for (int k = 0; k < LANES; ++k) {
+      a += L.sh[0][k][ci];
+      b += L.sh[1][k][ci];
+    }
+    L.sh[0][0][ci] = a;
+    L.sh[1][0][ci] = b;
+  }
+  __syncthreads();
+  float2 out = make_float2(0.f, 0.f);
+  if (first && col < c) {
+    const int cpg = c / groups;
+    const int g0 = (ci / cpg) * cpg;
+    double gs = 0.0, gss = 0.0;
+    for (int k = 0; k < cpg; ++k) {
+      gs += L.sh[0][0][g0 + k];
+      gss += L.sh[1][0][g0 + k];
+    }
+    const double cnt = static_cast<double>(n) * cpg;
+    const double mean = gs / cnt;
+    double var = gss / cnt - mean * mean;
+    if (var < 0.0) var = 0.0;
+    const double rstd = 1.0 / sqrt(var + static_cast<double>(eps));
+    const double gsc = rstd * static_cast<double>(gamma[col]);
+    out.x = static_cast<float>(gsc);
+    out.y = static_cast<float>(static_cast<double>(beta[col]) - mean * gsc);
+  }
+  return out;
+}
+
+template <int COLS, int THREADS>
+__device__ __forceinline__ void gn_tail_chunk(void* lds, const GnTail& t, const double* partial, int n, int c, int chunk) {
+  GnFinalizeLds<COLS>& L = *reinterpret_cast<GnFinalizeLds<COLS>*>(lds);
+  const int c_end = min(c, (chunk + 1) * kGnChunkCols);
+  for (int col0 = chunk * kGnChunkCols; col0 < c_end; col0 += COLS) {
+    const float2 v = gn_scale_shift<COLS, THREADS>(L, col0, partial, t.nblk, n, c, t.groups, t.gamma, t.beta, t.eps);
+    const int col = col0 + static_cast<int>(threadIdx.x);
+    if (threadIdx.x < COLS && col < c) {
+      t.scale[col] = v.x;
+      t.scale[c + col] = v.y;
+    }
+    __syncthreads();
+  }
+}
+
+template <int THREADS>
+__device__ __forceinline__ void gn_tail(void* lds, const GnTail& t, const double* partial, int n, int c, int chunk, int target) {
+  int* last = reinterpret_cast<int*>(static_cast<char*>(lds) + 2 * 1024 * 8);
+  asm volatile("s_waitcnt vmcnt(0)" ::: "memory");
+  __syncthreads();
+  if (threadIdx.x == 0) {
+    __builtin_amdgcn_fence(__ATOMIC_RELEASE, "agent");
+    asm volatile("s_waitcnt vmcnt(0)" ::: "memory");
+    const int ticket = __hip_atomic_fetch_add(t.counter + chunk, 1, __ATOMIC_RELAXED, __HIP_MEMORY_SCOPE_AGENT);
+    const int is_last = ticket == target - 1 ? 1 : 0;
+    if (is_last) {
+      __hip_atomic_store(t.counter + chunk, 0, __ATOMIC_RELAXED, __HIP_MEMORY_SCOPE_AGENT);
+      __builtin_amdgcn_fence(__ATOMIC_ACQUIRE, "agent");
+      asm volatile("s_waitcnt vmcnt(0)" ::: "memory");
+    }
+    *last = is_last;
+  }
+  __syncthreads();
+  if (*last == 0) return;
+  __syncthreads();
+  if (t.cols == 16) gn_tail_chunk<16, THREADS>(lds, t, partial, n, c, chunk);
+  else gn_tail_chunk<64, THREADS>(lds, t, partial, n, c, chunk);
+}
+#endif
+
+}
diff --git a/rdmnet_amd/csrc/internal.h b/rdmnet_amd/csrc/internal.h
--- a/rdmnet_amd/csrc/internal.h
+++ b/rdmnet_amd/csrc/internal.h
@@ -4,15 +4,26 @@
 
 namespace rdm {
 
+struct GnFinalizeSpec;
+
 int gemm_with_stats(const float* a, int64_t lda, const float* b, int64_t ldb, float* c, int64_t ldc, int64_t m,
                     int64_t n, int64_t k, const float* bias, const float* rowdiv, void* ws, size_t ws_bytes,
-                    double* gn_partial, int* gn_blocks, void* stream, int form = 0);
+                    double* gn_partial, int* gn_blocks, void* stream, int form = 0, GnFinalizeSpec* fin = nullptr);
 
 void gemm_set_lds_pad(unsigned bytes);
 int gemm_concat_with_stats(const float* coarse, int64_t ld1, int64_t c1, int64_t n_coarse, const int64_t* idx, int64_t ldi,
                            const float* skip, int64_t ld2, int64_t c2, const float* b, int64_t ldb, float* c, int64_t ldc,
                            int64_t m, int64_t n, const float* bias, int act, void* ws, size_t ws_bytes, double* gn_partial,
-                           int* gn_blocks, void* stream, int form = 0);
+                           int* gn_blocks, void* stream, int form = 0, GnFinalizeSpec* fin = nullptr);
+
+int linear_group_norm_impl(const float* x, int64_t ldx, const float* w, int64_t ldw, const float* bias, const float* rowdiv,
+                           int64_t m, int64_t n, int64_t k, int groups, const float* gamma, const float* beta, float eps,
+                           const float* residual, int64_t ldr, int act, float* lin_out, int64_t ld_lin, float* y, int64_t ldy,
+                           uint8_t* positive, void* ws, size_t ws_bytes, int form, int* counters, void* stream);
+int decoder_stage_impl(const float* coarse, int64_t n_coarse, int64_t c1, int64_t ld1, const int64_t* idx, int64_t ldi,
+                       const float* skip, int64_t c2, int64_t ld2, int64_t m, const float* w, int64_t ldw, const float* bias,
+                       int64_t n, int groups, const float* gamma, const float* beta, float eps, int act, float* lin_out,
+                       int64_t ld_lin, float* y, int64_t ldy, void* ws, size_t ws_bytes, int form, int* counters, void* stream);
 
 int gemm_pair(const float* a0, int64_t lda0, const float* b0, int64_t ldb0, float* c0, int64_t ldc0, int64_t m0, int64_t n0,
               int64_t k0, const float* bias0, const float* a1, int64_t lda1, const float* b1, int64_t ldb1, float* c1,
@@ -25,7 +36,19 @@
 
 int group_norm_finish(const double* partial, int nblk, const float* x, int64_t n, int64_t c, int64_t ldx, int groups,
                       const float* gamma, const float* beta, float eps, const float* residual, int64_t ldr, int act,
-                      float* y, int64_t ldy, uint8_t* positive, void* ws, size_t ws_bytes, void* stream, int form = 0);
+                      float* y, int64_t ldy, uint8_t* positive, void* ws, size_t ws_bytes, void* stream, int form = 0,
+                      int* counters = nullptr, bool finalized = false);
+float* group_norm_scale_slot(void* ws, size_t ws_bytes, int64_t n, int64_t c, int** own_counters = nullptr, void* stream = nullptr);
+
+struct GnFinalizeSpec {
+  int* counters;
+  const float* gamma;
+  const float* beta;
+  float* scale;
+  int groups;
+  float eps;
+  bool done;
+};
 
 int gather_rows_multi(int n, const void* const* x, const int64_t* n_src, const int64_t* words, const int64_t* ldx,
                       const int64_t* const* idx, const int64_t* m, void* const* y, const int64_t* ldy, void* stream);
@@ -53,7 +76,8 @@
 int kpconv_fused_impl(const float* q_points, int64_t m, const float* s_points, int64_t n_s, const float* s_feats, int64_t c,
                       int64_t ldf, const uint8_t* s_positive, const int64_t* idx, int64_t h, int64_t ldi, const int32_t* width,
                       const float* kernel_points, float sigma, const float* w_packed, const float* bias, int64_t c_out, float* out,
-                      int64_t ldo, double* gn_partial, const float* order_records, int form, int i32, void* stream);
+                      int64_t ldo, double* gn_partial, const float* order_records, int form, int i32, void* stream,
+                      GnFinalizeSpec* fin = nullptr);
 
 size_t radius_redo_queue_bytes();
 void radius_redo_queue_reset(void* queue);
diff --git a/rdmnet_amd/csrc/kpconv_fused.hip b/rdmnet_amd/csrc/kpconv_fused.hip
--- a/rdmnet_amd/csrc/kpconv_fused.hip
+++ b/rdmnet_amd/csrc/kpconv_fused.hip
@@ -3,6 +3,7 @@
 
 #include "../../include/rdmnet_hip.h"
 #include "common.h"
+#include "gn_tail.h"
 #include "internal.h"
 #include "lockstep.h"
 
@@ -40,6 +41,7 @@
   float sigma;
   int ctot;
   float* nn;
+  rdm::GnTail tail;
 };
 
 typedef float f32x2 __attribute__((ext_vector_type(2)));
@@ -222,6 +224,7 @@
       a.stats[(static_cast<int64_t>(blockIdx.x) * 2 + 0) * C + c] = s;
       a.stats[(static_cast<int64_t>(blockIdx.x) * 2 + 1) * C + c] = ss;
     }
+    if (a.tail.counter) rdm::gn_tail<64 * NW>(smem, a.tail, a.stats, a.M, C, 0, gridDim.x);
   }
 }
 template <int C, int QB, int NW, int ITERS>
@@ -636,6 +639,7 @@
       a.stats[(static_cast<int64_t>(blk) * 2 + 0) * C + 16 * ct + j] = st_s;
       a.stats[(static_cast<int64_t>(blk) * 2 + 1) * C + 16 * ct + j] = st_ss;
     }
+    if (a.tail.counter) rdm::gn_tail<64 * TileCfg<C>::NW>(smem_raw, a.tail, a.stats, a.M, C, 0, gridDim.x);
   }
   TILE_PHASE();
 #ifdef RDM_TILE_TIMING
@@ -726,6 +730,8 @@
       a.stats[(static_cast<int64_t>(blockIdx.x) * 2 + 0) * kC1Out + lane] = s;
       a.stats[(static_cast<int64_t>(blockIdx.x) * 2 + 1) * kC1Out + lane] = ss;
     }
+    static_assert(sizeof(nb_all) >= rdm::kGnTailLdsBytes, "the staging rows hold the finalize");
+    if (a.tail.counter) rdm::gn_tail<64 * kC1Waves>(nb_all, a.tail, a.stats, a.M, kC1Out, 0, gridDim.x);
   }
 }
 __global__ __launch_bounds__(64 * kC1Waves) void kpconv_fused_c1_kernel(FusedArgs a) { kpconv_fused_c1_kernel_body(blockIdx, gridDim, a); }
@@ -840,7 +846,8 @@
 int rdm::kpconv_fused_impl(const float* q_points, int64_t m, const float* s_points, int64_t n_s, const float* s_feats, int64_t c,
                            int64_t ldf, const uint8_t* s_positive, const int64_t* idx, int64_t h, int64_t ldi, const int32_t* width,
                            const float* kernel_points, float sigma, const float* w_packed, const float* bias, int64_t c_out,
-                           float* out, int64_t ldo, double* gn_partial, const float* order_records, int form, int i32, void* stream) {
+                           float* out, int64_t ldo, double* gn_partial, const float* order_records, int form, int i32, void* stream,
+                           GnFinalizeSpec* fin) {
   using namespace rdm;
   RDM_REQUIRE(form >= 0 && form <= 3, "rdm_kpconv_fused_form: form must be 0, 1 or 2 (3: lab variant of 2 without the XCD ranges)");
   RDM_REQUIRE(q_points && s_points && s_feats && s_positive && idx && kernel_points && w_packed && bias && out,
@@ -860,6 +867,12 @@
   a.ldf = static_cast<int>(ldf); a.ldi = static_cast<int>(ldi); a.ldo = static_cast<int>(ldo); a.sigma = sigma;
   hipStream_t st = static_cast<hipStream_t>(stream);
   const unsigned blocks = static_cast<unsigned>(rdm_kpconv_fused_partial_rows(m, c));
+  if (fin) fin->done = false;
+  if (fin && fin->counters && fin->scale && gn_partial) {
+    a.tail = GnTail{fin->counters, fin->gamma, fin->beta, fin->scale, static_cast<int>(blocks), fin->groups,
+                    gn_finalize_cols(static_cast<int>(blocks), c_out, fin->groups), fin->eps};
+    fin->done = true;
+  }
   RDM_DUP_LOOP("fused") {
   if (c == 1) {
     ::rdm::launch<kpconv_fused_c1_kernel_body, kpconv_fused_c1_kernel, 64 * kC1Waves>(dim3(blocks), 0, st, a);
@@ -916,11 +929,13 @@
     set_error("rdm_kpconv_fused_group_norm: workspace too small (%zu < %zu)", ws_bytes, ar.off);
     return RDM_ERR_WORKSPACE;
   }
-  if (int e = rdm_kpconv_fused(q_points, m, s_points, n_s, s_feats, c, ldf, s_positive, idx, h, ldi, width, kernel_points, sigma,
-                               w_packed, bias, c_out, conv_out, ld_conv, partial, order_records, stream))
+  GnFinalizeSpec fin{nullptr, gamma, beta, nullptr, groups, eps, false};
+  fin.scale = group_norm_scale_slot(nws, gn_ws, m, c_out, &fin.counters, stream);
+  if (int e = kpconv_fused_impl(q_points, m, s_points, n_s, s_feats, c, ldf, s_positive, idx, h, ldi, width, kernel_points, sigma,
+                                w_packed, bias, c_out, conv_out, ld_conv, partial, order_records, 0, 0, stream, &fin))
     return e;
   return group_norm_finish(partial, nblk, conv_out, m, c_out, ld_conv, groups, gamma, beta, eps, nullptr, 0, act, y, ldy, nullptr,
-                           nws, gn_ws, stream);
+                           nws, gn_ws, stream, 0, fin.counters, fin.done);
 }
 
 #ifdef RDM_TILE_TIMING
diff --git a/rdmnet_amd/csrc/norm.hip b/rdmnet_amd/csrc/norm.hip
--- a/rdmnet_amd/csrc/norm.hip
+++ b/rdmnet_amd/csrc/norm.hip
@@ -1,5 +1,6 @@
 #include "../../include/rdmnet_hip.h"
 #include "common.h"
+#include "gn_tail.h"
 #include "internal.h"
 #include "lockstep.h"
 
@@ -10,9 +11,10 @@
 constexpr int kGnRowsPerBlock = 64;
 
 __device__ __forceinline__ void gn_partial_kernel_body(const dim3 blockIdx, const dim3 gridDim, const float* x, int n, int c, int ld,
-                                                         double* partial) {
-  (void)blockIdx; (void)gridDim;
-  __shared__ double red[2][256];
+                                                         double* partial, GnTail tail) {
+  (void)blockIdx; (void)gridDim;
+  __shared__ __attribute__((aligned(16))) char lds[kGnTailLdsBytes];
+  double (*red)[256] = reinterpret_cast<double (*)[256]>(lds);
   const int r0 = blockIdx.x * kGnRowsPerBlock;
   const int r1 = min(n, r0 + kGnRowsPerBlock);
   const int cw = c < 256 ? c : 256;
@@ -38,70 +40,12 @@
     partial[(static_cast<int64_t>(blockIdx.x) * 2 + 0) * c + col] = a;
     partial[(static_cast<int64_t>(blockIdx.x) * 2 + 1) * c + col] = b;
   }
+  if (tail.counter) gn_tail<256>(lds, tail, partial, n, c, blockIdx.y, gridDim.x);
 }
 __global__ __launch_bounds__(256) void gn_partial_kernel(const float* x, int n, int c, int ld,
-                                                         double* partial) { gn_partial_kernel_body(blockIdx, gridDim, x, n, c, ld, partial); }
-
-
-template <int COLS>
-struct GnFinalizeLds {
-  double sh[2][1024 / COLS][COLS];
-};
-template <int COLS>
-__device__ __forceinline__ float2 gn_scale_shift(GnFinalizeLds<COLS>& L, int col0, const double* partial, int nblk, int n, int c,
-                                                 int groups, const float* gamma, const float* beta, float eps) {
-  constexpr int LANES = 1024 / COLS;
-  const int ci = threadIdx.x % COLS, lane = threadIdx.x / COLS;
-  const int col = col0 + ci;
-  double s = 0.0, ss = 0.0;
-  if (col < c)
-    for (int b0 = lane; b0 < nblk; b0 += 4 * LANES) {
-      double p0[4], p1[4];
-#pragma unroll
-      for (int u = 0; u < 4; ++u) {
-        const int b = b0 + LANES * u;
-        p0[u] = b < nblk ? partial[(static_cast<int64_t>(b) * 2 + 0) * c + col] : 0.0;
-        p1[u] = b < nblk ? partial[(static_cast<int64_t>(b) * 2 + 1) * c + col] : 0.0;
-      }
-#pragma unroll
-      for (int u = 0; u < 4; ++u) {
-        s += p0[u];
-        ss += p1[u];
-      }
-    }
-  L.sh[0][lane][ci] = s;
-  L.sh[1][lane][ci] = ss;
-  __syncthreads();
-  if (lane == 0) {
-    double a = 0.0, b = 0.0;
-    for (int k = 0; k < LANES; ++k) {
-      a += L.sh[0][k][ci];
-      b += L.sh[1][k][ci];
-    }
-    L.sh[0][0][ci] = a;
-    L.sh[1][0][ci] = b;
-  }
-  __syncthreads();
-  float2 out = make_float2(0.f, 0.f);
-  if (lane == 0 && col < c) {
-    const int cpg = c / groups;
-    const int g0 = (ci / cpg) * cpg;
-    double gs = 0.0, gss = 0.0;
-    for (int k = 0; k < cpg; ++k) {
-      gs += L.sh[0][0][g0 + k];
-      gss += L.sh[1][0][g0 + k];
-    }
-    const double cnt = static_cast<double>(n) * cpg;
-    const double mean = gs / cnt;
-    double var = gss / cnt - mean * mean;
-    if (var < 0.0) var = 0.0;
-    const double rstd = 1.0 / sqrt(var + static_cast<double>(eps));
-    const double gsc = rstd * static_cast<double>(gamma[col]);
-    out.x = static_cast<float>(gsc);
-    out.y = static_cast<float>(static_cast<double>(beta[col]) - mean * gsc);
-  }
-  return out;
-}
+                                                         double* partial, GnTail tail) { gn_partial_kernel_body(blockIdx, gridDim, x, n, c, ld, partial, tail); }
+
+
 template <int COLS>
 __device__ __forceinline__ void gn_finalize_kernel_body(const dim3 blockIdx, const dim3 gridDim, const double* partial, int nblk, int n,
                                                             int c, int groups, const float* gamma,
@@ -109,7 +53,7 @@
                                                             float* shift) {
   (void)blockIdx; (void)gridDim;
   __shared__ GnFinalizeLds<COLS> L;
-  const float2 v = gn_scale_shift<COLS>(L, blockIdx.x * COLS, partial, nblk, n, c, groups, gamma, beta, eps);
+  const float2 v = gn_scale_shift<COLS, 1024>(L, blockIdx.x * COLS, partial, nblk, n, c, groups, gamma, beta, eps);
   const int col = blockIdx.x * COLS + threadIdx.x % COLS;
   if (threadIdx.x / COLS == 0 && col < c) {
     scale[col] = v.x;
@@ -131,7 +75,7 @@
   __shared__ GnFinalizeLds<64> L;
   __shared__ float sc_l[64], sh_l[64];
   const int col0 = blockIdx.x * 64;
-  const float2 v = gn_scale_shift<64>(L, col0, partial, nblk, n, c, groups, gamma, beta, eps);
+  const float2 v = gn_scale_shift<64, 1024>(L, col0, partial, nblk, n, c, groups, gamma, beta, eps);
   if (threadIdx.x < 64) {
     sc_l[threadIdx.x] = v.x;
     sh_l[threadIdx.x] = v.y;
@@ -462,13 +406,25 @@
 
 extern "C" size_t rdm_group_norm_workspace_bytes(int64_t n, int64_t c) {
   const size_t nblk = static_cast<size_t>(rdm::ceil_div<int64_t>(n > 0 ? n : 1, kGnRowsPerBlock));
-  return rdm::align_up(nblk * 2 * c * sizeof(double)) + rdm::align_up(2 * c * sizeof(float));
+  return rdm::align_up(nblk * 2 * c * sizeof(double)) + rdm::align_up(2 * c * sizeof(float)) +
+         rdm::align_up(rdm::kGnMaxChunks * sizeof(int));
+}
+
+float* rdm::group_norm_scale_slot(void* ws, size_t ws_bytes, int64_t n, int64_t c, int** own_counters, void* stream) {
+  Arena ar(ws, ws_bytes);
+  ar.take<double>(static_cast<size_t>(ceil_div<int64_t>(n, kGnRowsPerBlock)) * 2 * c);
+  float* ss = ar.take<float>(2 * c);
+  if (own_counters) {
+    *own_counters = ar.take<int>(kGnMaxChunks);
+    if (*own_counters) fill_words<int>(*own_counters, kGnMaxChunks, 0, static_cast<hipStream_t>(stream));
+  }
+  return ss;
 }
 
 int rdm::group_norm_finish(const double* partial_in, int nblk, const float* x, int64_t n, int64_t c, int64_t ldx,
                            int groups, const float* gamma, const float* beta, float eps, const float* residual,
                            int64_t ldr, int act, float* y, int64_t ldy, uint8_t* positive, void* ws, size_t ws_bytes,
-                           void* stream, int form) {
+                           void* stream, int form, int* counters, bool finalized) {
   Arena ar(ws, ws_bytes);
   const int own_blk = static_cast<int>(ceil_div<int64_t>(n, kGnRowsPerBlock));
   double* partial = ar.take<double>(static_cast<size_t>(own_blk) * 2 * c);
@@ -480,23 +436,27 @@
   hipStream_t st = static_cast<hipStream_t>(stream);
   const double* use = partial_in;
   if (nblk <= 0) {
+    GnTail tail = gn_tail_none();
+    if (counters && form != 1 && c <= kGnChunkCols * kGnMaxChunks) {
+      tail = GnTail{counters, gamma, beta, ss, own_blk, groups, gn_finalize_cols(own_blk, c, groups), eps};
+      finalized = true;
+    }
     ::rdm::launch<gn_partial_kernel_body, gn_partial_kernel, 256>(dim3(own_blk, ceil_div<int64_t>(c, 256)), 0, st, x,
-                       static_cast<int>(n), static_cast<int>(c), static_cast<int>(ldx), partial);
+                       static_cast<int>(n), static_cast<int>(c), static_cast<int>(ldx), partial, tail);
     use = partial;
     nblk = own_blk;
   }
   const bool vec_ok = c % 4 == 0 && ldx % 4 == 0 && ldy % 4 == 0 && (!residual || ldr % 4 == 0) &&
                       (reinterpret_cast<uintptr_t>(x) & 15) == 0 && (reinterpret_cast<uintptr_t>(y) & 15) == 0 &&
                       (!residual || (reinterpret_cast<uintptr_t>(residual) & 15) == 0);
-  static const bool fin64 = ::rdm::dev_knob("RDM_GN_FINALIZE_64") != nullptr;
-  const bool narrow = !fin64 && nblk >= 128 && c / groups <= 16 && 16 % (c / groups) == 0;
-  if (form != 1 && !narrow && !positive && vec_ok && c % 64 == 0 && n <= 4096) {
+  const bool narrow = gn_finalize_cols(nblk, c, groups) == 16;
+  if (!finalized && form != 1 && !narrow && !positive && vec_ok && c % 64 == 0 && n <= 4096) {
     RDM_DUP_LOOP("gnfin")
     ::rdm::launch<gn_finalize_apply_kernel_body, gn_finalize_apply_kernel, 1024>(dim3(static_cast<unsigned>(c / 64), static_cast<unsigned>(ceil_div<int64_t>(n, kGnFusedRows))), 0, st, use, nblk, x, static_cast<int>(n), static_cast<int>(c), static_cast<int>(ldx), groups, gamma, beta,
                        eps, residual, static_cast<int>(ldr), act, y, static_cast<int>(ldy));
     return launch_status("gn_finalize_apply_kernel");
   }
-  {
+  if (!finalized) {
     RDM_DUP_LOOP("gnfin")
     if (narrow)
       ::rdm::launch<gn_finalize_kernel_body<16>, gn_finalize_kernel<16>, 1024>(dim3(ceil_div<int64_t>(c, 16)), 0, st, use, nblk,
@@ -530,8 +490,10 @@
   RDM_REQUIRE(n >= 0 && c > 0 && groups > 0 && c % groups == 0 && c <= 4096 && 64 % (c / groups) == 0,
               "rdm_group_norm: bad sizes (n=%lld c=%lld groups=%d)", (long long)n, (long long)c, groups);
   if (n == 0) return RDM_OK;
+  int* counters = nullptr;
+  (void)group_norm_scale_slot(ws, ws_bytes, n, c, &counters, stream);
   return group_norm_finish(nullptr, 0, x, n, c, ldx, groups, gamma, beta, eps, residual, ldr, act, y, ldy, positive, ws,
-                           ws_bytes, stream);
+                           ws_bytes, stream, 0, counters);
 }
 
 extern "C" int rdm_group_norm_form(const float* x, int64_t n, int64_t c, int64_t ldx, int groups, const float* gamma,
@@ -543,8 +505,10 @@
   RDM_REQUIRE(n >= 0 && c > 0 && groups > 0 && c % groups == 0 && c <= 4096 && 64 % (c / groups) == 0,
               "rdm_group_norm: bad sizes (n=%lld c=%lld groups=%d)", (long long)n, (long long)c, groups);
   if (n == 0) return RDM_OK;
+  int* counters = nullptr;
+  if (form != 1) (void)group_norm_scale_slot(ws, ws_bytes, n, c, &counters, stream);
   return group_norm_finish(nullptr, 0, x, n, c, ldx, groups, gamma, beta, eps, residual, ldr, act, y, ldy, positive, ws, ws_bytes,
-                           stream, form);
+                           stream, form, counters);
 }
 
 extern "C" int rdm_layer_norm(const float* x, int64_t n, int64_t c, int64_t ldx, const float* residual,
```

Measured after the change: 415.9. 30.6% lower.
